# Tele-AI/MMPL

Hardware: AMD Instinct MI355X
Metric: video_latent_frames_per_sec (higher is better)
Workload: dtype bf16

## Files before the change

### include/mmpl_hip.h

```cpp
#ifndef MMPL_HIP_H
#define MMPL_HIP_H
#include <stddef.h>
#include <stdint.h>
#ifdef __cplusplus
extern "C" {
#endif

typedef void* mmpl_stream_t;

typedef struct MmplDitConfig {
  int dim, ffn_dim, num_heads, num_layers;
  int text_dim, freq_dim, in_dim, out_dim, text_len;
  float eps;
  int lat_h, lat_w;
  int max_frames;
} MmplDitConfig;

typedef struct MmplDit MmplDit;

int mmpl_dit_num_weights(const MmplDitConfig* cfg);
const char* mmpl_dit_weight_name(int slot_in_layer_or_global, int per_layer);

int mmpl_dit_create(const MmplDitConfig* cfg, MmplDit** out);
void mmpl_dit_destroy(MmplDit* h);
int mmpl_dit_bind_weights(MmplDit* h, const void* const* dev_ptrs, int n);

size_t mmpl_dit_workspace_bytes(const MmplDit* h, int n_frames);
size_t mmpl_dit_context_workspace_bytes(const MmplDit* h);

int mmpl_dit_precompute_context(MmplDit* h, const void* context, void* cross_k, void* cross_v, void* workspace,
                                size_t workspace_bytes, int* distinct_rows, mmpl_stream_t stream);

int mmpl_dit_set_image_kv(MmplDit* h, const void* img_k, const void* img_v, int n_img_tokens);

int mmpl_dit_set_attn_stats(MmplDit* h, void* stats_dev);

int mmpl_dit_forward(MmplDit* h, const void* x_in, const float* t_dev, int n_frames, const int* frame_ids,
                     const int* write_slots, const int* visible_slots, int n_visible, void* k_cache, void* v_cache,
                     int n_slots, const void* cross_k, const void* cross_v, int cross_rows, void* share_out, const void* share_in,
                     void* attn_history, void* out, void* workspace, size_t workspace_bytes, mmpl_stream_t stream);
size_t mmpl_dit_attn_history_bytes(const MmplDit* h, int n_frames);
int mmpl_dit_share_check_failures(MmplDit* h, long long* count, mmpl_stream_t stream);

int mmpl_attn_fwd(const void* q, int ldq, void* o, int ldo, const void* const* k_pages, const void* const* v_pages,
                  int ldk, int ldv, int n_pages, int page_rows, int Lq, int num_heads, float softmax_scale,
                  mmpl_stream_t stream);
size_t mmpl_attn_workspace_bytes(void);
int mmpl_attn_fwd_ws(const void* q, int ldq, void* o, int ldo, const void* const* k_pages, const void* const* v_pages,
                     int ldk, int ldv, int n_pages, int page_rows, int Lq, int num_heads, float softmax_scale,
                     void* workspace, size_t workspace_bytes, mmpl_stream_t stream);

int mmpl_attn_fwd_variant(const void* q, int ldq, void* o, int ldo, const void* const* k_pages, const void* const* v_pages,
                          int ldk, int ldv, int n_pages, int page_rows, int Lq, int num_heads, float softmax_scale,
                          void* workspace, size_t workspace_bytes, int variant, int cross, mmpl_stream_t stream);

size_t mmpl_attn_history_bytes(int Lq, int num_heads);
int mmpl_attn_fwd_history(const void* q, int ldq, void* o, int ldo, const void* const* k_pages, const void* const* v_pages,
                          int ldk, int ldv, int n_pages, int page_rows, int Lq, int num_heads, float softmax_scale,
                          void* workspace, size_t workspace_bytes, void* history, void* stats_dev, mmpl_stream_t stream);

int mmpl_gemm(const void* A, int lda, const void* W, int ldw, const void* bias, void* C, int ldc, int M, int N, int K,
              int epi, const void* res, int ldres, const void* gate, int gate_frame_stride, int rows_per_frame,
              mmpl_stream_t stream);
int mmpl_gemm_tickets(const void* A, int lda, const void* W, int ldw, const void* bias, void* C, int ldc, int M, int N, int K,
                      int epi, const void* res, int ldres, const void* gate, int gate_frame_stride, int rows_per_frame,
                      void* tile_counter, mmpl_stream_t stream);
size_t mmpl_gemm_scratch_bytes(void);
int mmpl_device_xcd_round_robin(void);
int mmpl_probe_mfma_tflops(int shape, double seconds, double* tflops);
int mmpl_gemm_scratch(const void* A, int lda, const void* W, int ldw, const void* bias, void* C, int ldc, int M, int N, int K,
                      int epi, const void* res, int ldres, const void* gate, int gate_frame_stride, int rows_per_frame,
                      void* scratch, size_t scratch_bytes, mmpl_stream_t stream);

int mmpl_layernorm(const void* x, int ldx, void* y, int ldy, int rows, int d, float eps, const void* scale,
                   const void* shift, int mod_frame_stride, int rows_per_frame, const void* w, const void* b,
                   mmpl_stream_t stream);

int mmpl_qknorm_rope(MmplDit* h, void* q, int ldq, const void* k, int ldk, const void* v, int ldv, const void* wq,
                     const void* wk, int n_frames, const int* frame_ids, void* const* k_dst, void* const* v_dst,
                     mmpl_stream_t stream);

typedef struct MmplUniPCStep {
  float guidance, sigma_cur;
  int use_corrector, corr_order;
  float c_c1, c_c2, c_c3, c_inv_rk, c_rho0, c_rho_last;
  int pred_order;
  float p_c1, p_c2, p_c3, p_inv_rk;
} MmplUniPCStep;
int mmpl_cfg_unipc_step(const void* flow_cond, const void* flow_uncond, void* x, void* m0, void* m1, void* last_sample,
                        size_t n, const MmplUniPCStep* s, mmpl_stream_t stream);
int mmpl_cfg_unipc_step_table(const void* flow_cond, const void* flow_uncond, void* x, void* m0, void* m1, void* last_sample,
                              size_t n, const MmplUniPCStep* table_dev, int* step_dev, float* timestep_dev,
                              const float* timestep_table_dev, int n_timestep, int n_steps, mmpl_stream_t stream);

int mmpl_fewstep_update(const void* flow, void* x, const void* noise, void* x0_out, size_t n, double sigma_t, float sigma_next,
                        mmpl_stream_t stream);

typedef struct MmplVae MmplVae;
int mmpl_vae_num_weights(void);
const char* mmpl_vae_weight_name(int i);
int mmpl_vae_create(int lat_h, int lat_w, MmplVae** out);
void mmpl_vae_destroy(MmplVae* v);
int mmpl_vae_bind_weights(MmplVae* v, const void* const* dev_ptrs, int n);
size_t mmpl_vae_workspace_bytes(MmplVae* v, int mode);
int mmpl_vae_decode(MmplVae* v, const void* z, int n_frames, const float* mean, const float* inv_std, void* out, void* workspace,
                    size_t workspace_bytes, mmpl_stream_t stream);
int mmpl_vae_encode(MmplVae* v, const void* px, int n_px_frames, const float* mean, const float* inv_std, void* out, void* workspace,
                    size_t workspace_bytes, mmpl_stream_t stream);

typedef struct MmplVaeStream MmplVaeStream;
int mmpl_vae_stream_create(MmplVae* v, MmplVaeStream** out);
void mmpl_vae_stream_destroy(MmplVaeStream* s);
int mmpl_vae_stream_reset(MmplVaeStream* s);
int mmpl_vae_stream_decode(MmplVaeStream* s, const void* z, int n_frames, const float* mean, const float* inv_std, void* out,
                           int out_format, int* n_px_frames_out, void* workspace, size_t workspace_bytes, mmpl_stream_t stream);

typedef struct MmplTaehv MmplTaehv;
int mmpl_taehv_num_weights(void);
const char* mmpl_taehv_weight_name(int i);
int mmpl_taehv_create(int lat_h, int lat_w, MmplTaehv** out);
void mmpl_taehv_destroy(MmplTaehv* v);
int mmpl_taehv_bind_weights(MmplTaehv* v, const void* const* dev_ptrs, int n);
size_t mmpl_taehv_workspace_bytes(MmplTaehv* v);
int mmpl_taehv_reset(MmplTaehv* v);
int mmpl_taehv_decode(MmplTaehv* v, const void* z, int n_frames, void* out, int out_format, int* n_px_frames_out, void* workspace,
                      size_t workspace_bytes, mmpl_stream_t stream);

typedef struct MmplT5Config {
  int vocab, dim, dim_attn, dim_ffn, num_heads, num_layers, num_buckets, text_len;
  float eps;
} MmplT5Config;
typedef struct MmplT5 MmplT5;
int mmpl_t5_num_weights(const MmplT5Config* cfg);
int mmpl_t5_create(const MmplT5Config* cfg, MmplT5** out);
void mmpl_t5_destroy(MmplT5* h);
int mmpl_t5_bind_weights(MmplT5* h, const void* const* dev_ptrs, int n);
size_t mmpl_t5_workspace_bytes(const MmplT5* h);
int mmpl_t5_encode(MmplT5* h, const int* ids, const int* mask, const int* bucket, void* out, void* workspace,
                   size_t workspace_bytes, mmpl_stream_t stream);

size_t mmpl_i2v_img_proj_workspace_bytes(int n_tok, int clip_dim, int dim);
int mmpl_i2v_img_proj(const void* clip_fea, int n_tok, int clip_dim, int dim, const void* const* w, void* out, void* workspace,
                      size_t workspace_bytes, mmpl_stream_t stream);
int mmpl_i2v_img_kv(const void* ctx_img, int n_tok, int dim, const void* wk, const void* bk, const void* wv, const void* bv,
                    const void* norm_k_img_w, float eps, void* k_out, void* v_out, mmpl_stream_t stream);
size_t mmpl_i2v_cross_attn_workspace_bytes(int Lq, int dim);
int mmpl_i2v_cross_attn(const void* x, int Lq, int dim, const void* wq, const void* bq, const void* norm_q_w, float eps,
                        const void* k_txt, const void* v_txt, int n_txt, const void* k_img, const void* v_img, int n_img,
                        const void* wo, const void* bo, void* out, void* workspace, size_t workspace_bytes, mmpl_stream_t stream);

size_t mmpl_clip_visual_workspace_bytes(int n_tok, int dim, int mlp_dim, int heads);
int mmpl_clip_visual(const void* patches, int n_patch, int pk, int dim, int mlp_dim, int heads, int head_dim, int n_blocks,
                     const void* const* gw, const void* const* lw, float eps, void* out, void* workspace, size_t workspace_bytes,
                     mmpl_stream_t stream);

int mmpl_profile_enable(int on);
int mmpl_profile_read(int n_kinds, double* ms, double* flops, long long* launches);

const char* mmpl_last_error(void);
const char* mmpl_version(void);

#ifdef __cplusplus
}
#endif
#endif
```

### mmpl_amd/_lib.py

```python
from __future__ import annotations

import ctypes as C
import os

_HERE = os.path.dirname(os.path.abspath(__file__))
LIB_PATH = os.path.join(_HERE, "lib", "libmmpl_hip.so")

SYMBOLS = [
    "mmpl_dit_num_weights", "mmpl_dit_weight_name", "mmpl_dit_create", "mmpl_dit_destroy", "mmpl_dit_bind_weights",
    "mmpl_dit_workspace_bytes", "mmpl_dit_context_workspace_bytes", "mmpl_dit_precompute_context", "mmpl_dit_forward", "mmpl_dit_attn_history_bytes", "mmpl_dit_share_check_failures", "mmpl_dit_set_attn_stats", "mmpl_dit_set_image_kv", "mmpl_clip_visual", "mmpl_clip_visual_workspace_bytes",
    "mmpl_attn_fwd", "mmpl_attn_fwd_ws", "mmpl_attn_fwd_variant", "mmpl_attn_fwd_history", "mmpl_attn_history_bytes", "mmpl_attn_workspace_bytes", "mmpl_gemm", "mmpl_gemm_tickets", "mmpl_gemm_scratch", "mmpl_gemm_scratch_bytes", "mmpl_device_xcd_round_robin", "mmpl_probe_mfma_tflops", "mmpl_layernorm", "mmpl_qknorm_rope", "mmpl_cfg_unipc_step", "mmpl_cfg_unipc_step_table", "mmpl_fewstep_update",
    "mmpl_vae_num_weights", "mmpl_vae_weight_name", "mmpl_vae_create", "mmpl_vae_destroy", "mmpl_vae_bind_weights",
    "mmpl_vae_workspace_bytes", "mmpl_vae_decode", "mmpl_vae_encode",
    "mmpl_vae_stream_create", "mmpl_vae_stream_destroy", "mmpl_vae_stream_reset", "mmpl_vae_stream_decode",
    "mmpl_taehv_num_weights", "mmpl_taehv_weight_name", "mmpl_taehv_create", "mmpl_taehv_destroy", "mmpl_taehv_bind_weights",
    "mmpl_taehv_workspace_bytes", "mmpl_taehv_reset", "mmpl_taehv_decode",
    "mmpl_t5_num_weights", "mmpl_t5_create", "mmpl_t5_destroy", "mmpl_t5_bind_weights", "mmpl_t5_workspace_bytes", "mmpl_t5_encode",
    "mmpl_i2v_img_proj_workspace_bytes", "mmpl_i2v_img_proj", "mmpl_i2v_img_kv", "mmpl_i2v_cross_attn_workspace_bytes", "mmpl_i2v_cross_attn",
    "mmpl_profile_enable", "mmpl_profile_read", "mmpl_last_error", "mmpl_version",
]


class MmplDitConfig(C.Structure):
    _fields_ = [(n, C.c_int) for n in ("dim", "ffn_dim", "num_heads", "num_layers", "text_dim", "freq_dim", "in_dim",
                                       "out_dim", "text_len")] + [("eps", C.c_float)] + \
               [(n, C.c_int) for n in ("lat_h", "lat_w", "max_frames")]


class MmplT5Config(C.Structure):
    _fields_ = [(n, C.c_int) for n in ("vocab", "dim", "dim_attn", "dim_ffn", "num_heads", "num_layers", "num_buckets", "text_len")] + \
               [("eps", C.c_float)]


class MmplUniPCStep(C.Structure):
    _fields_ = [("guidance", C.c_float), ("sigma_cur", C.c_float), ("use_corrector", C.c_int), ("corr_order", C.c_int),
                ("c_c1", C.c_float), ("c_c2", C.c_float), ("c_c3", C.c_float), ("c_inv_rk", C.c_float),
                ("c_rho0", C.c_float), ("c_rho_last", C.c_float), ("pred_order", C.c_int), ("p_c1", C.c_float),
                ("p_c2", C.c_float), ("p_c3", C.c_float), ("p_inv_rk", C.c_float)]


_lib = None


def load() -> C.CDLL:
    global _lib
    if _lib is not None:
        return _lib
    if not os.path.exists(LIB_PATH):
        raise RuntimeError(
            f"{LIB_PATH} not found: the MI355X HIP extension is not built. Run `python -m mmpl_amd.build` "
            "(or __graft_entry__.build()). mmpl_amd has no CPU/PyTorch fallback by design.")
    import torch
    lib = C.CDLL(LIB_PATH)
    vp, ci, cf, sz = C.c_void_p, C.c_int, C.c_float, C.c_size_t
    lib.mmpl_last_error.restype = C.c_char_p
    lib.mmpl_version.restype = C.c_char_p
    lib.mmpl_dit_num_weights.argtypes = [C.POINTER(MmplDitConfig)]
    lib.mmpl_dit_weight_name.argtypes = [ci, ci]
    lib.mmpl_dit_weight_name.restype = C.c_char_p
    lib.mmpl_dit_create.argtypes = [C.POINTER(MmplDitConfig), C.POINTER(vp)]
    lib.mmpl_dit_destroy.argtypes = [vp]
    lib.mmpl_dit_destroy.restype = None
    lib.mmpl_dit_bind_weights.argtypes = [vp, C.POINTER(vp), ci]
    lib.mmpl_dit_workspace_bytes.argtypes = [vp, ci]
    lib.mmpl_dit_workspace_bytes.restype = sz
    lib.mmpl_dit_context_workspace_bytes.argtypes = [vp]
    lib.mmpl_dit_context_workspace_bytes.restype = sz
    lib.mmpl_dit_precompute_context.argtypes = [vp, vp, vp, vp, vp, sz, C.POINTER(ci), vp]
    lib.mmpl_dit_forward.argtypes = [vp, vp, vp, ci, C.POINTER(ci), C.POINTER(ci), C.POINTER(ci), ci, vp, vp, ci, vp, vp,
                                     ci, vp, vp, vp, vp, vp, sz, vp]
    lib.mmpl_dit_attn_history_bytes.argtypes = [vp, ci]
    lib.mmpl_dit_attn_history_bytes.restype = sz
    lib.mmpl_dit_share_check_failures.argtypes = [vp, C.POINTER(C.c_longlong), vp]
    lib.mmpl_attn_history_bytes.argtypes = [ci, ci]
    lib.mmpl_attn_history_bytes.restype = sz
    lib.mmpl_attn_fwd_history.argtypes = [vp, ci, vp, ci, C.POINTER(vp), C.POINTER(vp), ci, ci, ci, ci, ci, ci, cf, vp, sz, vp, vp, vp]
    lib.mmpl_attn_fwd.argtypes = [vp, ci, vp, ci, C.POINTER(vp), C.POINTER(vp), ci, ci, ci, ci, ci, ci, cf, vp]
    lib.mmpl_attn_fwd_ws.argtypes = [vp, ci, vp, ci, C.POINTER(vp), C.POINTER(vp), ci, ci, ci, ci, ci, ci, cf, vp, sz, vp]
    lib.mmpl_attn_fwd_variant.argtypes = [vp, ci, vp, ci, C.POINTER(vp), C.POINTER(vp), ci, ci, ci, ci, ci, ci, cf, vp, sz, ci, ci, vp]
    lib.mmpl_cfg_unipc_step_table.argtypes = [vp, vp, vp, vp, vp, vp, sz, vp, vp, vp, vp, ci, ci, vp]
    lib.mmpl_attn_workspace_bytes.argtypes = []
    lib.mmpl_attn_workspace_bytes.restype = sz
    lib.mmpl_gemm.argtypes = [vp, ci, vp, ci, vp, vp, ci, ci, ci, ci, ci, vp, ci, vp, ci, ci, vp]
    lib.mmpl_gemm_tickets.argtypes = [vp, ci, vp, ci, vp, vp, ci, ci, ci, ci, ci, vp, ci, vp, ci, ci, vp, vp]
    lib.mmpl_gemm_scratch.argtypes = [vp, ci, vp, ci, vp, vp, ci, ci, ci, ci, ci, vp, ci, vp, ci, ci, vp, sz, vp]
    lib.mmpl_gemm_scratch_bytes.argtypes = []
    lib.mmpl_device_xcd_round_robin.argtypes = []
    lib.mmpl_probe_mfma_tflops.argtypes = [ci, C.c_double, C.POINTER(C.c_double)]
    lib.mmpl_gemm_scratch_bytes.restype = sz
    lib.mmpl_layernorm.argtypes = [vp, ci, vp, ci, ci, ci, cf, vp, vp, ci, ci, vp, vp, vp]
    lib.mmpl_qknorm_rope.argtypes = [vp, vp, ci, vp, ci, vp, ci, vp, vp, ci, C.POINTER(ci), C.POINTER(vp), C.POINTER(vp), vp]
    lib.mmpl_cfg_unipc_step.argtypes = [vp, vp, vp, vp, vp, vp, sz, C.POINTER(MmplUniPCStep), vp]
    lib.mmpl_fewstep_update.argtypes = [vp, vp, vp, vp, sz, C.c_double, cf, vp]
    lib.mmpl_profile_enable.argtypes = [ci]
    lib.mmpl_profile_read.argtypes = [ci, C.POINTER(C.c_double), C.POINTER(C.c_double), C.POINTER(C.c_longlong)]
    lib.mmpl_t5_num_weights.argtypes = [C.POINTER(MmplT5Config)]
    lib.mmpl_t5_create.argtypes = [C.POINTER(MmplT5Config), C.POINTER(vp)]
    lib.mmpl_t5_destroy.argtypes = [vp]
    lib.mmpl_t5_destroy.restype = None
    lib.mmpl_t5_bind_weights.argtypes = [vp, C.POINTER(vp), ci]
    lib.mmpl_t5_workspace_bytes.argtypes = [vp]
    lib.mmpl_t5_workspace_bytes.restype = sz
    lib.mmpl_t5_encode.argtypes = [vp, vp, vp, vp, vp, vp, sz, vp]
    cf = C.c_float
    lib.mmpl_i2v_img_proj_workspace_bytes.argtypes = [ci, ci, ci]
    lib.mmpl_i2v_img_proj_workspace_bytes.restype = sz
    lib.mmpl_dit_set_image_kv.argtypes = [vp, vp, vp, ci]
    lib.mmpl_dit_set_attn_stats.argtypes = [vp, vp]
    lib.mmpl_clip_visual_workspace_bytes.argtypes = [ci, ci, ci, ci]
    lib.mmpl_clip_visual_workspace_bytes.restype = sz
    lib.mmpl_clip_visual.argtypes = [vp, ci, ci, ci, ci, ci, ci, ci, C.POINTER(vp), C.POINTER(vp), cf, vp, vp, sz, vp]
    lib.mmpl_i2v_img_proj.argtypes = [vp, ci, ci, ci, C.POINTER(vp), vp, vp, sz, vp]
    lib.mmpl_i2v_img_kv.argtypes = [vp, ci, ci, vp, vp, vp, vp, vp, cf, vp, vp, vp]
    lib.mmpl_i2v_cross_attn_workspace_bytes.argtypes = [ci, ci]
    lib.mmpl_i2v_cross_attn_workspace_bytes.restype = sz
    lib.mmpl_i2v_cross_attn.argtypes = [vp, ci, ci, vp, vp, vp, cf, vp, vp, ci, vp, vp, ci, vp, vp, vp, vp, sz, vp]
    if hasattr(lib, "mmpl_vae_create"):
        _bind_vae(lib)
    _lib = lib
    return lib


def _bind_vae(lib):
    vp, ci, sz = C.c_void_p, C.c_int, C.c_size_t
    fp = C.POINTER(C.c_float)
    lib.mmpl_vae_weight_name.argtypes = [ci]
    lib.mmpl_vae_weight_name.restype = C.c_char_p
    lib.mmpl_vae_create.argtypes = [ci, ci, C.POINTER(vp)]
    lib.mmpl_vae_destroy.argtypes = [vp]
    lib.mmpl_vae_destroy.restype = None
    lib.mmpl_vae_bind_weights.argtypes = [vp, C.POINTER(vp), ci]
    lib.mmpl_vae_workspace_bytes.argtypes = [vp, ci]
    lib.mmpl_vae_workspace_bytes.restype = sz
    lib.mmpl_vae_decode.argtypes = [vp, vp, ci, fp, fp, vp, vp, sz, vp]
    lib.mmpl_vae_encode.argtypes = [vp, vp, ci, fp, fp, vp, vp, sz, vp]
    lib.mmpl_vae_stream_create.argtypes = [vp, C.POINTER(vp)]
    lib.mmpl_vae_stream_destroy.argtypes = [vp]
    lib.mmpl_vae_stream_destroy.restype = None
    lib.mmpl_vae_stream_reset.argtypes = [vp]
    lib.mmpl_vae_stream_decode.argtypes = [vp, vp, ci, fp, fp, vp, ci, C.POINTER(ci), vp, sz, vp]
    lib.mmpl_taehv_weight_name.argtypes = [ci]
    lib.mmpl_taehv_weight_name.restype = C.c_char_p
    lib.mmpl_taehv_create.argtypes = [ci, ci, C.POINTER(vp)]
    lib.mmpl_taehv_destroy.argtypes = [vp]
    lib.mmpl_taehv_destroy.restype = None
    lib.mmpl_taehv_bind_weights.argtypes = [vp, C.POINTER(vp), ci]
    lib.mmpl_taehv_workspace_bytes.argtypes = [vp]
    lib.mmpl_taehv_workspace_bytes.restype = sz
    lib.mmpl_taehv_reset.argtypes = [vp]
    lib.mmpl_taehv_decode.argtypes = [vp, vp, ci, vp, ci, C.POINTER(ci), vp, sz, vp]


def check(rc: int, what: str = "") -> None:
    if rc != 0:
        raise RuntimeError(f"libmmpl_hip {what}: {load().mmpl_last_error().decode()}")


def ptr(t) -> C.c_void_p:
    return C.c_void_p(0 if t is None else t.data_ptr())


def stream_ptr() -> C.c_void_p:
    import torch
    return C.c_void_p(torch.cuda.current_stream().cuda_stream)
```

### mmpl_amd/csrc/api.hip

```cpp
#include <math.h>
#include <stdio.h>
#include <stdlib.h>
#include <string.h>

#include <string>
#include <utility>
#include <vector>

#include "../../include/mmpl_hip.h"
#include "kernels.h"
#include "mmpl_config.h"

static thread_local std::string g_err;
static int fail(const char* where, const char* what) {
  g_err = std::string(where) + ": " + what;
  return 1;
}
int mmpl_set_error(const char* where, const char* what) { return fail(where, what); }
#define HIP_TRY(expr, where)                                     \
  do {                                                           \
    hipError_t e__ = (expr);                                     \
    if (e__ != hipSuccess) return fail(where, hipGetErrorString(e__)); \
  } while (0)

// ... 125 lines not shown
  for (int pos = 0; pos < 1024; ++pos) {
    int p = 0;
    for (int part = 0; part < 3; ++part)
      for (int j = 0; j < dims[part] / 2; ++j, ++p) {
        const double freq = 1.0 / pow(10000.0, (double)(2 * j) / (double)dims[part]);
        const double ang = (double)pos * freq;
        c[pos * 64 + p] = (float)cos(ang);
        s[pos * 64 + p] = (float)sin(ang);
      }
  }
  if (hipMalloc(&h->cos_tab, c.size() * 4) != hipSuccess || hipMalloc(&h->sin_tab, s.size() * 4) != hipSuccess) {
    delete h;
    return fail("mmpl_dit_create", "hipMalloc of RoPE tables failed (is a GPU present?)");
  }
  hipMemcpy(h->cos_tab, c.data(), c.size() * 4, hipMemcpyHostToDevice);
  hipMemcpy(h->sin_tab, s.data(), s.size() * 4, hipMemcpyHostToDevice);
  if (mmpl_config().check_share) {
    if (hipMalloc(&h->share_chk, 8 * sizeof(unsigned long long)) != hipSuccess || hipMemset(h->share_chk, 0, 8 * sizeof(unsigned long long)) != hipSuccess) {
      mmpl_dit_destroy(h);
      return fail("mmpl_dit_create", "hipMalloc of the share-check state failed");
    }
  }
  *out = h;
  return 0;
}

void mmpl_dit_destroy(MmplDit* h) {
  if (!h) return;
  if (h->cos_tab) hipFree(h->cos_tab);
  if (h->sin_tab) hipFree(h->sin_tab);
  if (h->share_chk) hipFree(h->share_chk);
  delete h;
}

int mmpl_dit_bind_weights(MmplDit* h, const void* const* ptrs, int n) {
  if (!h || !ptrs) return fail("mmpl_dit_bind_weights", "null argument");
  if (n != NG + h->cfg.num_layers * NL) return fail("mmpl_dit_bind_weights", "wrong pointer count");
  h->w.resize(n);
  for (int i = 0; i < n; ++i) {
    if (!ptrs[i]) return fail("mmpl_dit_bind_weights", "null weight pointer");
    h->w[i] = (const bf16_t*)ptrs[i];
  }
  return 0;
}

}

namespace {
struct Carver {
  char* base;
  size_t off = 0;
  explicit Carver(void* b) : base((char*)b) {}
  bf16_t* take(size_t elems) {
    bf16_t* p = (bf16_t*)(base + off);
    off += (elems * 2 + 255) & ~(size_t)255;
    return p;
  }
};
constexpr int kTicketInts = 64 + 256;
struct FwdWs {
  bf16_t *x, *xn, *big, *attn, *ksc, *vsc, *patch, *sinu, *t1, *e, *se, *e0, *emod, *emod_head, *yh;
  int* tile_counter;
  float* splitk;
  size_t bytes;
};
FwdWs carve_fwd(const MmplDit* h, int nF, void* base) {
  const MmplDitConfig& c = h->cfg;
  const size_t Lq = (size_t)nF * h->S, d = c.dim;
  const size_t bigw = (size_t)(3 * c.dim > c.ffn_dim ? 3 * c.dim : c.ffn_dim);
  Carver k(base);
  FwdWs w;
  static_assert(kTicketInts * sizeof(int) % sizeof(bf16_t) == 0, "ticket area");
  w.tile_counter = (int*)k.take(kTicketInts * sizeof(int) / sizeof(bf16_t));
  w.x = k.take(Lq * d);
  w.xn = k.take(Lq * d);
  w.big = k.take(Lq * bigw);
  w.attn = k.take(Lq * d);
  w.ksc = k.take(Lq * d);
  w.vsc = k.take(Lq * d);
  w.patch = k.take(Lq * (size_t)h->pe_k);
  w.sinu = k.take((size_t)nF * c.freq_dim);
  w.t1 = k.take((size_t)nF * d);
  w.e = k.take((size_t)nF * d);
  w.se = k.take((size_t)nF * d);
  w.e0 = k.take((size_t)nF * 6 * d);
  w.emod = k.take((size_t)c.num_layers * nF * 6 * d);
  w.emod_head = k.take((size_t)nF * 2 * d);
  w.yh = k.take(Lq * 64);
  w.splitk = (float*)k.take(mmpl_gemm_splitk_ws_bytes() / sizeof(bf16_t));
  w.bytes = k.off;
  return w;
}

int gemm(const bf16_t* A, int lda, const bf16_t* W, int ldw, const bf16_t* bias, bf16_t* C, int ldc, int M, int N, int K,
         int epi, const bf16_t* res, int ldres, const bf16_t* gate, int gfs, int rpf, hipStream_t s, int* tile_counter = nullptr,
         float* splitk_ws = nullptr) {
  GemmArgs g{A, lda, W, ldw, bias, C, ldc, M, N, K, epi, res, ldres, gate, gfs, rpf > 0 ? rpf : 1, 1.0f, 0, 0, 0, 0, 0};
  g.tile_counter = tile_counter;
  g.splitk_ws = splitk_ws;
  g.splitk_cnt = splitk_ws ? tile_counter + 64 : nullptr;
  ProfScope ps(K_GEMM, 2.0 * M * (double)N * K, s);
  hipError_t e = mmpl_launch_gemm(g, s);
  if (e != hipSuccess) return fail("gemm", hipGetErrorString(e));
  return 0;
}
#define TRY(x) do { if ((x) != 0) return 1; } while (0)
}

extern "C" {

size_t mmpl_dit_workspace_bytes(const MmplDit* h, int n_frames) { return carve_fwd(h, n_frames, nullptr).bytes; }
size_t mmpl_dit_context_workspace_bytes(const MmplDit* h) {
  return 2 * (((size_t)h->cfg.text_len * h->cfg.dim * 2 + 255) & ~(size_t)255) + (((size_t)h->cfg.text_len * sizeof(int) + 255) & ~(size_t)255);
}

int mmpl_dit_precompute_context(MmplDit* h, const void* context, void* cross_k, void* cross_v, void* workspace,
                                size_t workspace_bytes, int* distinct_rows, mmpl_stream_t stream) {
  if (!h || h->w.empty()) return fail("mmpl_dit_precompute_context", "weights not bound");
  if (workspace_bytes < mmpl_dit_context_workspace_bytes(h)) return fail("mmpl_dit_precompute_context", "workspace too small");
  const MmplDitConfig& c = h->cfg;
  hipStream_t s = (hipStream_t)stream;
  Carver k(workspace);
  bf16_t* t0 = k.take((size_t)c.text_len * c.dim);
  bf16_t* ctx = k.take((size_t)c.text_len * c.dim);
  const int T = c.text_len, d = c.dim;
  TRY(gemm((const bf16_t*)context, c.text_dim, h->G(G_TXT0_W), c.text_dim, h->G(G_TXT0_B), t0, d, T, d, c.text_dim,
           EPI_BIAS_GELU, nullptr, 0, nullptr, 0, 1, s));
  TRY(gemm(t0, d, h->G(G_TXT2_W), d, h->G(G_TXT2_B), ctx, d, T, d, d, EPI_BIAS, nullptr, 0, nullptr, 0, 1, s));
  if (distinct_rows) {
    *distinct_rows = T;
    hipStreamCaptureStatus cs = hipStreamCaptureStatusNone;
    (void)hipStreamIsCapturing(s, &cs);
    if (cs == hipStreamCaptureStatusNone && T >= 2) {
      int* flags = (int*)k.take(((size_t)T * sizeof(int) + 1) / sizeof(bf16_t));
      std::vector<int> hf(T);
      HIP_TRY(mmpl_launch_rows_equal_last(ctx, d, T, d, flags, s), "rows_equal_last");
      HIP_TRY(hipMemcpyAsync(hf.data(), flags, (size_t)T * sizeof(int), hipMemcpyDeviceToHost, s), "context flags");
      HIP_TRY(hipStreamSynchronize(s), "context flags");
      int n = T - 1;
      while (n > 0 && hf[n - 1]) --n;
      if (T - n >= 2) *distinct_rows = n;
    }
  }
  for (int l = 0; l < c.num_layers; ++l) {
    bf16_t* kl = (bf16_t*)cross_k + (size_t)l * T * d;
    bf16_t* vl = (bf16_t*)cross_v + (size_t)l * T * d;
    TRY(gemm(ctx, d, h->Lw(l, L_CK_W), d, h->Lw(l, L_CK_B), kl, d, T, d, d, EPI_BIAS, nullptr, 0, nullptr, 0, 1, s));
    HIP_TRY(mmpl_launch_rmsnorm(kl, d, h->Lw(l, L_CNK), T, d, c.eps, s), "rmsnorm(ctx k)");
    TRY(gemm(ctx, d, h->Lw(l, L_CV_W), d, h->Lw(l, L_CV_B), vl, d, T, d, d, EPI_BIAS, nullptr, 0, nullptr, 0, 1, s));
  }
  return 0;
}

int mmpl_dit_set_image_kv(MmplDit* h, const void* img_k, const void* img_v, int n_img_tokens) {
  if (!h) return fail("mmpl_dit_set_image_kv", "null handle");
  if ((img_k == nullptr) != (img_v == nullptr)) return fail("mmpl_dit_set_image_kv", "need both of img_k / img_v, or neither");
  if (img_k && (n_img_tokens < 1 || n_img_tokens > 4096)) return fail("mmpl_dit_set_image_kv", "n_img_tokens out of range");
  h->img_k = (const bf16_t*)img_k;
  h->img_v = (const bf16_t*)img_v;
  h->n_img = img_k ? n_img_tokens : 0;
  return 0;
}

int mmpl_dit_set_attn_stats(MmplDit* h, void* stats_dev) {
  if (!h) return fail("mmpl_dit_set_attn_stats", "null handle");
  if (reinterpret_cast<uintptr_t>(stats_dev) % 8) return fail("mmpl_dit_set_attn_stats", "stats must be 8-byte aligned");
  h->attn_stats = (unsigned long long*)stats_dev;
  return 0;
}

int mmpl_dit_forward(MmplDit* h, const void* x_in, const float* t_dev, int nF, const int* frame_ids,
                     const int* write_slots, const int* visible_slots, int n_visible, void* k_cache, void* v_cache,
                     int n_slots, const void* cross_k, const void* cross_v, int cross_rows, void* share_out, const void* share_in,
                     void* attn_history, void* out, void* workspace, size_t workspace_bytes, mmpl_stream_t stream) {
  if (!h || h->w.empty()) return fail("mmpl_dit_forward", "weights not bound");
  const MmplDitConfig& c = h->cfg;
  if (nF < 1 || nF > c.max_frames) return fail("mmpl_dit_forward", "n_frames out of range");
  int n_write = 0;
  for (int i = 0; i < nF; ++i) {
    if (write_slots[i] >= n_slots) return fail("mmpl_dit_forward", "write slot out of range");
    if (write_slots[i] >= 0) ++n_write;
  }
  if (n_write != 0 && n_write != nF) return fail("mmpl_dit_forward", "write_slots must be all >= 0 or all -1");
  if (share_out && share_in) return fail("mmpl_dit_forward", "share_out and share_in are exclusive (producer or consumer of block 0's self-attention)");
  const bool persist = n_write == nF;
  const int n_pages = n_visible + (persist ? 0 : nF);
  if (n_pages < 1 || n_pages > MMPL_MAX_PAGES) return fail("mmpl_dit_forward", "too many / no visible KV pages");
  for (int i = 0; i < n_visible; ++i)
    if (visible_slots[i] < 0 || visible_slots[i] >= n_slots) return fail("mmpl_dit_forward", "visible slot out of range");
  FwdWs w = carve_fwd(h, nF, workspace);
  if (workspace_bytes < w.bytes) return fail("mmpl_dit_forward", "workspace too small");
  hipStream_t s = (hipStream_t)stream;
  const int S = h->S, d = c.dim, f = c.ffn_dim, Lq = nF * S, H = c.num_heads, T = c.text_len;

  HIP_TRY(mmpl_launch_zero_ints(w.tile_counter, kTicketInts, s), "tile counter");
  int* const tc = w.tile_counter;
  HIP_TRY(mmpl_launch_patchify((const bf16_t*)x_in, w.patch, h->pe_k, nF, c.in_dim, c.lat_h, c.lat_w, s), "patchify");
  TRY(gemm(w.patch, h->pe_k, h->G(G_PE_W), h->pe_k, h->G(G_PE_B), w.x, d, Lq, d, h->pe_k, EPI_BIAS, nullptr, 0, nullptr, 0, 1, s));
  HIP_TRY(mmpl_launch_sinusoid(t_dev, w.sinu, nF, c.freq_dim, s), "sinusoid");
  TRY(gemm(w.sinu, c.freq_dim, h->G(G_TE0_W), c.freq_dim, h->G(G_TE0_B), w.t1, d, nF, d, c.freq_dim, EPI_BIAS_SILU, nullptr,
           0, nullptr, 0, 1, s));
  TRY(gemm(w.t1, d, h->G(G_TE2_W), d, h->G(G_TE2_B), w.e, d, nF, d, d, EPI_BIAS, nullptr, 0, nullptr, 0, 1, s));
  HIP_TRY(mmpl_launch_silu(w.e, w.se, (size_t)nF * d, s), "silu");
  TRY(gemm(w.se, d, h->G(G_TP_W), d, h->G(G_TP_B), w.e0, 6 * d, nF, 6 * d, d, EPI_BIAS, nullptr, 0, nullptr, 0, 1, s));
  HIP_TRY(mmpl_launch_modulation(h->G(G_BLOCK_MOD), (size_t)6 * d, w.e0, 6 * d, 0, w.emod, c.num_layers, nF, 6, d, s), "modulation");
  HIP_TRY(mmpl_launch_modulation(h->G(G_HEAD_MOD), 0, w.e, d, 1, w.emod_head, 1, nF, 2, d, s), "head modulation");

  const float scale = 1.0f / sqrtf(128.0f);
  const int self_variant = mmpl_attention_self_variant();
  const bool prescale_q = self_variant == ATTN_W64;
  const bool cross_w64_env = mmpl_config().cross_w64;
  const bool cross_w64 = cross_w64_env && prescale_q;
  const size_t layer_stride = (size_t)n_slots * S * d;
  const int ctx_n = (cross_rows >= 0 && cross_rows <= T - 2) ? cross_rows : -1;
  const size_t hist_layer = mmpl_attn_history_bytes(Lq, H);
  const bool check_share = h->share_chk != nullptr && (share_out || share_in);
  auto fingerprint_layer0 = [&](int which) -> int {
    PageList pk{}, pv{};
    for (int i = 0; i < n_visible; ++i) {
      pk.p[i] = (const bf16_t*)k_cache + (size_t)visible_slots[i] * S * d;
      pv.p[i] = (const bf16_t*)v_cache + (size_t)visible_slots[i] * S * d;
    }
    pk.n = pv.n = n_visible;
    if (n_visible < 1) return 0;
    HIP_TRY(mmpl_launch_share_check_zero(h->share_chk, which, s), "share check");
    HIP_TRY(mmpl_launch_pages_fingerprint(pk, (size_t)S * d * sizeof(bf16_t), h->share_chk, which, s), "share check (K)");
    HIP_TRY(mmpl_launch_pages_fingerprint(pv, (size_t)S * d * sizeof(bf16_t), h->share_chk, which, s), "share check (V)");
    if (which == 1) HIP_TRY(mmpl_launch_share_check_compare(h->share_chk, s), "share check (compare)");
    return 0;
  };
  for (int l = 0; l < c.num_layers; ++l) {
    const bf16_t* em = w.emod + (size_t)l * nF * 6 * d;
    bf16_t* kc = (bf16_t*)k_cache + (size_t)l * layer_stride;
    bf16_t* vc = (bf16_t*)v_cache + (size_t)l * layer_stride;
    const bool take_shared = l == 0 && share_in != nullptr;
    if (!take_shared || persist) {
      {
        LnArgs a{w.x, d, w.xn, d, Lq, d, c.eps, em + 1 * d, em + 0 * d, 6 * d, S, nullptr, nullptr};
        ProfScope ps(K_LAYERNORM, 0, s);
        HIP_TRY(mmpl_launch_layernorm(a, s), "norm1");
      }
      {
        GemmArgs g{w.xn, d, h->Lw(l, L_QKV_W), d, h->Lw(l, L_QKV_B), w.big, 3 * d, Lq, 3 * d, d, EPI_BIAS_VPAGES, nullptr, 0, nullptr, 0, S,
                   1.0f, 0, 0, 0, 0, 0};
        for (int i = 0; i < nF; ++i) g.v_dst[i] = persist ? vc + (size_t)write_slots[i] * S * d : w.vsc + (size_t)i * S * d;
        g.v_col0 = 2 * d;
        g.v_ld = d;
        g.tile_counter = tc;
        g.splitk_ws = w.splitk; g.splitk_cnt = tc + 64;
        ProfScope ps(K_GEMM, 2.0 * Lq * 3.0 * d * d, s);
        HIP_TRY(mmpl_launch_gemm(g, s), "qkv gemm");
      }
      {
        QkNormArgs a = {};
        a.q = w.big; a.ldq = 3 * d; a.k = w.big + d; a.ldk = 3 * d; a.v = nullptr; a.ldv = 3 * d;
        a.wq = h->Lw(l, L_NQ); a.wk = h->Lw(l, L_NK); a.rows = Lq; a.d = d; a.eps = c.eps; a.rope = 1;
        a.q_scale = prescale_q ? scale * 1.4426950408889634f : 0.f;
        a.cos_tab = h->cos_tab; a.sin_tab = h->sin_tab; a.rows_per_frame = S; a.grid_w = h->gw;
        for (int i = 0; i < nF; ++i) {
          a.frame_ids[i] = frame_ids[i];
          a.k_dst[i] = persist ? kc + (size_t)write_slots[i] * S * d : w.ksc + (size_t)i * S * d;
          a.v_dst[i] = persist ? vc + (size_t)write_slots[i] * S * d : w.vsc + (size_t)i * S * d;
        }
        ProfScope ps(K_QKNORM, 0, s);
        HIP_TRY(mmpl_launch_qknorm(a, s), "qk norm + rope + kv write");
      }
    }
    if (l == 0 && check_share) TRY(fingerprint_layer0(share_in ? 1 : 0));
    if (take_shared) {
      HIP_TRY(hipMemcpyAsync(w.x, share_in, (size_t)Lq * d * sizeof(bf16_t), hipMemcpyDeviceToDevice, s), "shared block-0 x");
    } else {
    {
        AttnArgs a = {};
        a.q = w.big; a.ldq = 3 * d; a.o = w.attn; a.ldo = d; a.ldk = d; a.ldv = d; a.page_rows = S; a.Lq = Lq; a.H = H; a.scale = scale;
        int np = 0;
        for (int i = 0; i < n_visible; ++i, ++np) {
          a.k_pages[np] = kc + (size_t)visible_slots[i] * S * d;
          a.v_pages[np] = vc + (size_t)visible_slots[i] * S * d;
        }
        if (!persist)
          for (int i = 0; i < nF; ++i, ++np) {
            a.k_pages[np] = w.ksc + (size_t)i * S * d;
            a.v_pages[np] = w.vsc + (size_t)i * S * d;
            a.page_group[np] = 1;
          }
        a.n_pages = np;
        a.variant = self_variant;
        a.q_prescaled = prescale_q;
        a.split_ws = (float*)w.xn;
        a.split_ws_bytes = (size_t)Lq * d * sizeof(bf16_t);
        a.redo_stats = h->attn_stats;
        a.history = attn_history ? (unsigned char*)attn_history + (size_t)l * hist_layer : nullptr;
        ProfScope ps(K_ATTN_SELF, 4.0 * Lq * (double)np * S * d, s);
        HIP_TRY(mmpl_launch_attention(a, s), "self attention");
      }
      TRY(gemm(w.attn, d, h->Lw(l, L_O_W), d, h->Lw(l, L_O_B), w.x, d, Lq, d, d, EPI_GATE_RES, w.x, d, em + 2 * d, 6 * d, S, s, tc, w.splitk));
      if (l == 0 && share_out) HIP_TRY(hipMemcpyAsync(share_out, w.x, (size_t)Lq * d * sizeof(bf16_t), hipMemcpyDeviceToDevice, s), "share block-0 x");
    }
    {
      LnArgs a{w.x, d, w.xn, d, Lq, d, c.eps, nullptr, nullptr, 0, S, h->Lw(l, L_N3_W), h->Lw(l, L_N3_B)};
      ProfScope ps(K_LAYERNORM, 0, s);
      HIP_TRY(mmpl_launch_layernorm(a, s), "norm3");
    }
    TRY(gemm(w.xn, d, h->Lw(l, L_CQ_W), d, h->Lw(l, L_CQ_B), w.big, d, Lq, d, d, EPI_BIAS, nullptr, 0, nullptr, 0, 1, s, tc, w.splitk));
    {
      ProfScope ps(K_QKNORM, 0, s);
      HIP_TRY(mmpl_launch_rmsnorm(w.big, d, h->Lw(l, L_CNQ), Lq, d, c.eps, s, cross_w64 ? scale * 1.4426950408889634f : 0.f), "cross q norm");
    }
    {
      AttnArgs a = {};
      a.q = w.big; a.ldq = d; a.o = w.attn; a.ldo = d; a.ldk = d; a.ldv = d; a.page_rows = T; a.Lq = Lq; a.H = H; a.scale = scale;
      a.n_pages = 1;
      a.cross = 1;
      if (cross_w64) { a.variant = ATTN_W64; a.q_prescaled = true; }
      else if (ctx_n >= 0) { a.page_rows = ctx_n + 1; a.last_row_copies = T - ctx_n; }
      a.k_pages[0] = (const bf16_t*)cross_k + (size_t)l * T * d;
      a.v_pages[0] = (const bf16_t*)cross_v + (size_t)l * T * d;
      ProfScope ps(K_ATTN_CROSS, 4.0 * Lq * (double)T * d, s);
      HIP_TRY(mmpl_launch_attention(a, s), "cross attention");
      if (h->img_k) {
        a.o = w.ksc;
        a.page_rows = h->n_img;
        a.last_row_copies = 0;
        a.k_pages[0] = h->img_k + (size_t)l * h->n_img * d;
        a.v_pages[0] = h->img_v + (size_t)l * h->n_img * d;
        ProfScope ps2(K_ATTN_CROSS, 4.0 * Lq * (double)h->n_img * d, s);
        HIP_TRY(mmpl_launch_attention(a, s), "image cross attention");
        HIP_TRY(mmpl_launch_add(w.attn, w.ksc, (size_t)Lq * d, s), "x + img_x");
      }
    }
    TRY(gemm(w.attn, d, h->Lw(l, L_CO_W), d, h->Lw(l, L_CO_B), w.x, d, Lq, d, d, EPI_RES, w.x, d, nullptr, 0, 1, s, tc, w.splitk));
    {
      LnArgs a{w.x, d, w.xn, d, Lq, d, c.eps, em + 4 * d, em + 3 * d, 6 * d, S, nullptr, nullptr};
      ProfScope ps(K_LAYERNORM, 0, s);
      HIP_TRY(mmpl_launch_layernorm(a, s), "norm2");
    }
    TRY(gemm(w.xn, d, h->Lw(l, L_F0_W), d, h->Lw(l, L_F0_B), w.big, f, Lq, f, d, EPI_BIAS_GELU, nullptr, 0, nullptr, 0, 1, s, tc, w.splitk));
    TRY(gemm(w.big, f, h->Lw(l, L_F2_W), f, h->Lw(l, L_F2_B), w.x, d, Lq, d, f, EPI_GATE_RES, w.x, d, em + 5 * d, 6 * d, S, s, tc, w.splitk));
  }
  {
    LnArgs a{w.x, d, w.xn, d, Lq, d, c.eps, w.emod_head + d, w.emod_head, 2 * d, S, nullptr, nullptr};
    HIP_TRY(mmpl_launch_layernorm(a, s), "head norm");
  }
  TRY(gemm(w.xn, d, h->G(G_HEAD_W), d, h->G(G_HEAD_B), w.yh, 64, Lq, 64, d, EPI_BIAS, nullptr, 0, nullptr, 0, 1, s));
  HIP_TRY(mmpl_launch_unpatchify(w.yh, 64, (bf16_t*)out, nF, c.out_dim, c.lat_h, c.lat_w, s), "unpatchify");
  if (check_share && share_in) {
    hipStreamCaptureStatus cs = hipStreamCaptureStatusNone;
    (void)hipStreamIsCapturing(s, &cs);
    if (cs == hipStreamCaptureStatusNone) {
      long long n = 0;
      TRY(mmpl_dit_share_check_failures(h, &n, stream));
      if (n) return fail("mmpl_dit_forward", "MMPL_CHECK_SHARE: share_in was given but the layer-0 K / V this forward attends to differ from "
                                             "the share_out forward's (the two CFG caches are out of step)");
    }
  }
  return 0;
}

int mmpl_dit_share_check_failures(MmplDit* h, long long* count, mmpl_stream_t stream) {
  if (!h || !count) return fail("mmpl_dit_share_check_failures", "null argument");
  *count = 0;
  if (!h->share_chk) return 0;
  unsigned long long n = 0;
  hipStream_t s = (hipStream_t)stream;
  HIP_TRY(hipMemcpyAsync(&n, h->share_chk + 4, sizeof(n), hipMemcpyDeviceToHost, s), "share check read");
  HIP_TRY(hipStreamSynchronize(s), "share check read");
  if (n) HIP_TRY(hipMemsetAsync(h->share_chk + 4, 0, sizeof(n), s), "share check reset");
  *count = (long long)n;
  return 0;
}

size_t mmpl_dit_attn_history_bytes(const MmplDit* h, int n_frames) {
  return h ? (size_t)h->cfg.num_layers * mmpl_attn_history_bytes(n_frames * h->S, h->cfg.num_heads) : 0;
}
size_t mmpl_attn_history_bytes(int Lq, int num_heads) { return mmpl_attention_history_bytes(Lq, num_heads); }

int mmpl_attn_fwd_history(const void* q, int ldq, void* o, int ldo, const void* const* k_pages, const void* const* v_pages,
                          int ldk, int ldv, int n_pages, int page_rows, int Lq, int num_heads, float softmax_scale,
                          void* workspace, size_t workspace_bytes, void* history, void* stats_dev, mmpl_stream_t stream) {
  if (n_pages < 1 || n_pages > MMPL_MAX_PAGES) return fail("mmpl_attn_fwd_history", "n_pages out of range");
  if (reinterpret_cast<uintptr_t>(stats_dev) % 8) return fail("mmpl_attn_fwd_history", "stats must be 8-byte aligned");
  AttnArgs a = {};
  a.variant = ATTN_W64;
  a.q_prescaled = 1;
  a.q = (const bf16_t*)q; a.ldq = ldq; a.o = (bf16_t*)o; a.ldo = ldo; a.ldk = ldk; a.ldv = ldv; a.n_pages = n_pages;
  a.page_rows = page_rows; a.Lq = Lq; a.H = num_heads; a.scale = softmax_scale;
  a.split_ws = (float*)workspace; a.split_ws_bytes = workspace ? workspace_bytes : 0;
  a.history = (unsigned char*)history;
  a.redo_stats = (unsigned long long*)stats_dev;
  for (int i = 0; i < n_pages; ++i) { a.k_pages[i] = (const bf16_t*)k_pages[i]; a.v_pages[i] = (const bf16_t*)v_pages[i]; }
  HIP_TRY(mmpl_launch_attention(a, (hipStream_t)stream), "mmpl_attn_fwd_history");
  return 0;
}

size_t mmpl_attn_workspace_bytes(void) { return mmpl_attention_split_ws_bytes(); }

int mmpl_attn_fwd_variant(const void* q, int ldq, void* o, int ldo, const void* const* k_pages, const void* const* v_pages,
                          int ldk, int ldv, int n_pages, int page_rows, int Lq, int num_heads, float softmax_scale,
                          void* workspace, size_t workspace_bytes, int variant, int cross, mmpl_stream_t stream) {
  if (n_pages < 1 || n_pages > MMPL_MAX_PAGES) return fail("mmpl_attn_fwd", "n_pages out of range");
  if (variant != ATTN_AUTO && variant != ATTN_LOCKSTEP && variant != ATTN_W64 && variant != ATTN_W64 + 1)
    return fail("mmpl_attn_fwd", "unknown kernel variant");
  AttnArgs a = {};
  a.variant = variant > ATTN_W64 ? ATTN_W64 : variant;
  a.q_prescaled = variant == ATTN_W64 + 1;
  a.cross = cross != 0;
  a.q = (const bf16_t*)q; a.ldq = ldq; a.o = (bf16_t*)o; a.ldo = ldo; a.ldk = ldk; a.ldv = ldv; a.n_pages = n_pages;
  a.page_rows = page_rows; a.Lq = Lq; a.H = num_heads; a.scale = softmax_scale;
  a.split_ws = (float*)workspace; a.split_ws_bytes = workspace ? workspace_bytes : 0;
  for (int i = 0; i < n_pages; ++i) { a.k_pages[i] = (const bf16_t*)k_pages[i]; a.v_pages[i] = (const bf16_t*)v_pages[i]; }
  HIP_TRY(mmpl_launch_attention(a, (hipStream_t)stream), "mmpl_attn_fwd");
  return 0;
}

int mmpl_attn_fwd_ws(const void* q, int ldq, void* o, int ldo, const void* const* k_pages, const void* const* v_pages,
                     int ldk, int ldv, int n_pages, int page_rows, int Lq, int num_heads, float softmax_scale,
                     void* workspace, size_t workspace_bytes, mmpl_stream_t stream) {
  return mmpl_attn_fwd_variant(q, ldq, o, ldo, k_pages, v_pages, ldk, ldv, n_pages, page_rows, Lq, num_heads, softmax_scale, workspace,
                               workspace_bytes, ATTN_AUTO, 0, stream);
}

int mmpl_attn_fwd(const void* q, int ldq, void* o, int ldo, const void* const* k_pages, const void* const* v_pages,
                  int ldk, int ldv, int n_pages, int page_rows, int Lq, int num_heads, float softmax_scale,
                  mmpl_stream_t stream) {
  return mmpl_attn_fwd_ws(q, ldq, o, ldo, k_pages, v_pages, ldk, ldv, n_pages, page_rows, Lq, num_heads, softmax_scale, nullptr, 0,
                          stream);
}

int mmpl_gemm(const void* A, int lda, const void* W, int ldw, const void* bias, void* C, int ldc, int M, int N, int K,
              int epi, const void* res, int ldres, const void* gate, int gate_frame_stride, int rows_per_frame,
              mmpl_stream_t stream) {
  if (epi < EPI_BIAS || epi > EPI_F32_SCALE) return fail("mmpl_gemm", "unknown epilogue");
  if ((epi == EPI_GATE_RES && (!res || !gate)) || (epi == EPI_RES && !res)) return fail("mmpl_gemm", "missing epilogue operand");
  return gemm((const bf16_t*)A, lda, (const bf16_t*)W, ldw, (const bf16_t*)bias, (bf16_t*)C, ldc, M, N, K, epi,
              (const bf16_t*)res, ldres, (const bf16_t*)gate, gate_frame_stride, rows_per_frame, (hipStream_t)stream);
}

int mmpl_gemm_tickets(const void* A, int lda, const void* W, int ldw, const void* bias, void* C, int ldc, int M, int N, int K,
                      int epi, const void* res, int ldres, const void* gate, int gate_frame_stride, int rows_per_frame,
                      void* tile_counter, mmpl_stream_t stream) {
  if (epi < EPI_BIAS || epi > EPI_F32_SCALE) return fail("mmpl_gemm", "unknown epilogue");
  if ((epi == EPI_GATE_RES && (!res || !gate)) || (epi == EPI_RES && !res)) return fail("mmpl_gemm", "missing epilogue operand");
  return gemm((const bf16_t*)A, lda, (const bf16_t*)W, ldw, (const bf16_t*)bias, (bf16_t*)C, ldc, M, N, K, epi,
              (const bf16_t*)res, ldres, (const bf16_t*)gate, gate_frame_stride, rows_per_frame, (hipStream_t)stream, (int*)tile_counter);
}

size_t mmpl_gemm_scratch_bytes(void) { return 2048 + mmpl_gemm_splitk_ws_bytes(); }
int mmpl_device_xcd_round_robin(void) { return mmpl_xcd_dispatch_ok(true) ? 1 : 0; }

int mmpl_gemm_scratch(const void* A, int lda, const void* W, int ldw, const void* bias, void* C, int ldc, int M, int N, int K,
                      int epi, const void* res, int ldres, const void* gate, int gate_frame_stride, int rows_per_frame,
                      void* scratch, size_t scratch_bytes, mmpl_stream_t stream) {
  if (epi < EPI_BIAS || epi > EPI_F32_SCALE) return fail("mmpl_gemm", "unknown epilogue");
  if ((epi == EPI_GATE_RES && (!res || !gate)) || (epi == EPI_RES && !res)) return fail("mmpl_gemm", "missing epilogue operand");
  if (!scratch || scratch_bytes < mmpl_gemm_scratch_bytes()) return fail("mmpl_gemm_scratch", "scratch missing or smaller than mmpl_gemm_scratch_bytes()");
  if (reinterpret_cast<uintptr_t>(scratch) % 256) return fail("mmpl_gemm_scratch", "scratch must be 256-byte aligned");
  return gemm((const bf16_t*)A, lda, (const bf16_t*)W, ldw, (const bf16_t*)bias, (bf16_t*)C, ldc, M, N, K, epi,
              (const bf16_t*)res, ldres, (const bf16_t*)gate, gate_frame_stride, rows_per_frame, (hipStream_t)stream, (int*)scratch,
              (float*)((char*)scratch + 2048));
}

int mmpl_layernorm(const void* x, int ldx, void* y, int ldy, int rows, int d, float eps, const void* scale,
                   const void* shift, int mod_frame_stride, int rows_per_frame, const void* w, const void* b,
                   mmpl_stream_t stream) {
  if (!w && (!scale || !shift)) return fail("mmpl_layernorm", "need (scale, shift) or (w, b)");
  LnArgs a{(const bf16_t*)x, ldx, (bf16_t*)y, ldy, rows, d, eps, (const bf16_t*)scale, (const bf16_t*)shift, mod_frame_stride,
           rows_per_frame > 0 ? rows_per_frame : 1, (const bf16_t*)w, (const bf16_t*)b};
  HIP_TRY(mmpl_launch_layernorm(a, (hipStream_t)stream), "mmpl_layernorm");
  return 0;
}

int mmpl_qknorm_rope(MmplDit* h, void* q, int ldq, const void* k, int ldk, const void* v, int ldv, const void* wq,
                     const void* wk, int n_frames, const int* frame_ids, void* const* k_dst, void* const* v_dst,
                     mmpl_stream_t stream) {
  if (!h) return fail("mmpl_qknorm_rope", "null handle");
  if (n_frames < 1 || n_frames > 8) return fail("mmpl_qknorm_rope", "n_frames out of range");
  QkNormArgs a = {};
  a.q = (bf16_t*)q; a.ldq = ldq; a.k = (const bf16_t*)k; a.ldk = ldk; a.v = (const bf16_t*)v; a.ldv = ldv;
  a.wq = (const bf16_t*)wq; a.wk = (const bf16_t*)wk; a.rows = n_frames * h->S; a.d = h->cfg.dim; a.eps = h->cfg.eps; a.rope = 1;
  a.cos_tab = h->cos_tab; a.sin_tab = h->sin_tab; a.rows_per_frame = h->S; a.grid_w = h->gw;
  for (int i = 0; i < n_frames; ++i) { a.frame_ids[i] = frame_ids[i]; a.k_dst[i] = (bf16_t*)k_dst[i]; a.v_dst[i] = (bf16_t*)v_dst[i]; }
  HIP_TRY(mmpl_launch_qknorm(a, (hipStream_t)stream), "mmpl_qknorm_rope");
  return 0;
}

int mmpl_cfg_unipc_step(const void* flow_cond, const void* flow_uncond, void* x, void* m0, void* m1, void* last_sample,
                        size_t n, const MmplUniPCStep* st, mmpl_stream_t stream) {
  if (!st) return fail("mmpl_cfg_unipc_step", "null step");
  UniPCArgs a = {};
  a.flow_c = (const bf16_t*)flow_cond; a.flow_u = (const bf16_t*)flow_uncond; a.guidance = st->guidance; a.x = (bf16_t*)x;
  a.m0 = (bf16_t*)m0; a.m1 = (bf16_t*)m1; a.last_sample = (bf16_t*)last_sample; a.n = n; a.sigma_cur = st->sigma_cur;
  a.use_corrector = st->use_corrector; a.corr_order = st->corr_order; a.c_c1 = st->c_c1; a.c_c2 = st->c_c2; a.c_c3 = st->c_c3;
  a.c_inv_rk = st->c_inv_rk; a.c_rho0 = st->c_rho0; a.c_rho_last = st->c_rho_last; a.pred_order = st->pred_order;
  a.p_c1 = st->p_c1; a.p_c2 = st->p_c2; a.p_c3 = st->p_c3; a.p_inv_rk = st->p_inv_rk;
  ProfScope ps(K_UNIPC, 0, (hipStream_t)stream);
  HIP_TRY(mmpl_launch_unipc(a, (hipStream_t)stream), "mmpl_cfg_unipc_step");
  return 0;
}

int mmpl_cfg_unipc_step_table(const void* flow_cond, const void* flow_uncond, void* x, void* m0, void* m1, void* last_sample,
                              size_t n, const MmplUniPCStep* table_dev, int* step_dev, float* timestep_dev,
                              const float* timestep_table_dev, int n_timestep, int n_steps, mmpl_stream_t stream) {
  if (!table_dev || !step_dev || !timestep_dev || !timestep_table_dev || n_steps < 1 || n_timestep < 1)
    return fail("mmpl_cfg_unipc_step_table", "bad arguments");
  static_assert(sizeof(MmplUniPCStep) == sizeof(UniPCStepDev), "table layout");
  UniPCArgs a = {};
  a.flow_c = (const bf16_t*)flow_cond; a.flow_u = (const bf16_t*)flow_uncond; a.x = (bf16_t*)x;
  a.m0 = (bf16_t*)m0; a.m1 = (bf16_t*)m1; a.last_sample = (bf16_t*)last_sample; a.n = n;
  HIP_TRY(mmpl_launch_unipc_table(a, (const UniPCStepDev*)table_dev, step_dev, timestep_dev, timestep_table_dev, n_timestep, n_steps,
                                  (hipStream_t)stream), "mmpl_cfg_unipc_step_table");
  return 0;
}

}
```

### mmpl_amd/csrc/attention.hip

```cpp
#include <stdlib.h>

#include <type_traits>

#include "common.h"
#include "kernels.h"
#include "mmpl_config.h"

namespace {

constexpr int NW = 8, QW = 32, QB = NW * QW, KVB = 64;
constexpr int K_STRIDE = 272;
constexpr int V_STRIDE = 320;
constexpr int K_TILE = KVB * K_STRIDE;
constexpr int V_TILE = KVB * V_STRIDE;
constexpr int BUF = K_TILE + V_TILE;
constexpr int SMEM = 2 * BUF;

typedef __attribute__((ext_vector_type(4))) short s16x4;

MMPL_DEV bf16x8 tr_pair(const char* p0, const char* p1) {
  s16x4 a = __builtin_amdgcn_ds_read_tr16_b64_v4i16((__attribute__((address_space(3))) s16x4*)(p0));
  s16x4 b = __builtin_amdgcn_ds_read_tr16_b64_v4i16((__attribute__((address_space(3))) s16x4*)(p1));
  return bf16x8{a[0], a[1], a[2], a[3], b[0], b[1], b[2], b[3]};
}

struct AttnState { f32x16 o[4]; float m_run, l_run; };
MMPL_DEV void attn_tile(const char* kb, const char* vb, const bf16x8 (&qf)[8], int valid, float last_bias, float c, int k_off, int v_off,
                        int hi, AttnState& st) {
#pragma clang fp contract(off)
  f32x16 (&o)[4] = st.o;
  float& m_run = st.m_run;
  float& l_run = st.l_run;
  f32x16 s0, s1;
#pragma unroll
  for (int r = 0; r < 16; ++r) { s0[r] = 0.f; s1[r] = 0.f; }
  {
    auto kfrag = [&](int i) {
      return *reinterpret_cast<const bf16x8*>(kb + k_off + (i >> 3) * (32 * K_STRIDE) + 32 * (i & 7));
    };
    bf16x8 w0 = kfrag(0), w1 = kfrag(1), w2 = kfrag(2), w3 = kfrag(3);
    __builtin_amdgcn_sched_barrier(0);
    __builtin_amdgcn_s_setprio(1);
#pragma unroll
    for (int i = 0; i < 16; i += 4) {
      if (i < 8) s0 = __builtin_amdgcn_mfma_f32_32x32x16_bf16(w0, qf[i & 7], s0, 0, 0, 0);
      else s1 = __builtin_amdgcn_mfma_f32_32x32x16_bf16(w0, qf[i & 7], s1, 0, 0, 0);
      if (i + 4 < 16) w0 = kfrag(i + 4);
      __builtin_amdgcn_sched_barrier(0);
      if (i < 8) s0 = __builtin_amdgcn_mfma_f32_32x32x16_bf16(w1, qf[(i + 1) & 7], s0, 0, 0, 0);
      else s1 = __builtin_amdgcn_mfma_f32_32x32x16_bf16(w1, qf[(i + 1) & 7], s1, 0, 0, 0);
      if (i + 5 < 16) w1 = kfrag(i + 5);
      __builtin_amdgcn_sched_barrier(0);
      if (i < 8) s0 = __builtin_amdgcn_mfma_f32_32x32x16_bf16(w2, qf[(i + 2) & 7], s0, 0, 0, 0);
      else s1 = __builtin_amdgcn_mfma_f32_32x32x16_bf16(w2, qf[(i + 2) & 7], s1, 0, 0, 0);
      if (i + 6 < 16) w2 = kfrag(i + 6);
      __builtin_amdgcn_sched_barrier(0);
      if (i < 8) s0 = __builtin_amdgcn_mfma_f32_32x32x16_bf16(w3, qf[(i + 3) & 7], s0, 0, 0, 0);
      else s1 = __builtin_amdgcn_mfma_f32_32x32x16_bf16(w3, qf[(i + 3) & 7], s1, 0, 0, 0);
      if (i + 7 < 16) w3 = kfrag(i + 7);
      __builtin_amdgcn_sched_barrier(0);
    }
    __builtin_amdgcn_s_setprio(0);
  }
  if (valid < KVB) {
#pragma unroll
    for (int r = 0; r < 16; ++r) {
      const int kv = 8 * (r >> 2) + 4 * hi + (r & 3);
      if (kv >= valid) s0[r] = -INFINITY;
      if (kv + 32 >= valid) s1[r] = -INFINITY;
    }
  }
  if (last_bias != 0.f && valid <= KVB) {
#pragma unroll
    for (int r = 0; r < 16; ++r) {
      const int kv = 8 * (r >> 2) + 4 * hi + (r & 3);
      if (kv == valid - 1) s0[r] += last_bias;
      if (kv + 32 == valid - 1) s1[r] += last_bias;
    }
  }
  float mx = s0[0];
#pragma unroll
  for (int r = 1; r < 16; ++r) mx = fmaxf(mx, s0[r]);
#pragma unroll
  for (int r = 0; r < 16; ++r) mx = fmaxf(mx, s1[r]);
  mx = fmaxf(mx, __shfl_xor(mx, 32, 64));
  const float m_new = fmaxf(m_run, mx);
  if (__any(m_new > m_run)) {
    const float alpha = __builtin_amdgcn_exp2f((m_run - m_new) * c);
    l_run *= alpha;
#pragma unroll
    for (int nb = 0; nb < 4; ++nb)
#pragma unroll
      for (int r = 0; r < 16; ++r) o[nb][r] *= alpha;
    m_run = m_new;
  }
  const float mc = m_run * c;
  float ls0 = 0.f, ls1 = 0.f;
  bf16x8 pb[2][2];
#pragma unroll
  for (int r = 0; r < 16; ++r) { s0[r] = __builtin_amdgcn_exp2f(__builtin_fmaf(s0[r], c, -mc)); ls0 += s0[r]; }
#pragma unroll
  for (int cc = 0; cc < 2; ++cc) {
    union { uint32_t u[4]; bf16x8 v; } x0;
#pragma unroll
    for (int j = 0; j < 4; ++j) x0.u[j] = pack2bf(s0[8 * cc + 2 * j], s0[8 * cc + 2 * j + 1]);
    pb[0][cc] = x0.v;
  }
#pragma unroll
  for (int cc = 0; cc < 2; ++cc)
#pragma unroll
    for (int nb = 0; nb < 4; ++nb) {
      const char* vp = vb + v_off + (16 * cc) * V_STRIDE + 64 * nb;
      const bf16x8 vf = tr_pair(vp, vp + 8 * V_STRIDE);
      o[nb] = __builtin_amdgcn_mfma_f32_32x32x16_bf16(vf, pb[0][cc], o[nb], 0, 0, 0);
    }
#pragma unroll
  for (int r = 0; r < 16; ++r) { s1[r] = __builtin_amdgcn_exp2f(__builtin_fmaf(s1[r], c, -mc)); ls1 += s1[r]; }
  l_run += ls0 + ls1;
#pragma unroll
  for (int cc = 0; cc < 2; ++cc) {
    union { uint32_t u[4]; bf16x8 v; } x1;
#pragma unroll
    for (int j = 0; j < 4; ++j) x1.u[j] = pack2bf(s1[8 * cc + 2 * j], s1[8 * cc + 2 * j + 1]);
    pb[1][cc] = x1.v;
  }
  __builtin_amdgcn_s_setprio(1);
#pragma unroll
  for (int cc = 0; cc < 2; ++cc)
#pragma unroll
    for (int nb = 0; nb < 4; ++nb) {
      const char* vp = vb + v_off + (32 + 16 * cc) * V_STRIDE + 64 * nb;
      const bf16x8 vf = tr_pair(vp, vp + 8 * V_STRIDE);
      o[nb] = __builtin_amdgcn_mfma_f32_32x32x16_bf16(vf, pb[1][cc], o[nb], 0, 0, 0);
    }
  __builtin_amdgcn_s_setprio(0);

}

template <int CROSS>
__global__ __launch_bounds__(512, 2) void attn_fwd_kernel(AttnArgs a) {
  extern __shared__ __attribute__((aligned(16))) char smem[];
  const int tid = threadIdx.x, lane = tid & 63, wave = tid >> 6;
  const int hi = lane >> 5, l31 = lane & 31;

  const int n_qb = (a.Lq + QB - 1) / QB;
  int head, qb;
  if ((a.H & 7) == 0) {
    const int xcd = blockIdx.x & 7, local = blockIdx.x >> 3;
    head = xcd + 8 * (local / n_qb);
    qb = local % n_qb;
  } else {
    head = blockIdx.x / n_qb;
    qb = blockIdx.x % n_qb;
  }

  const int qrow = min(qb * QB + wave * QW + l31, a.Lq - 1);
  bf16x8 qf[8];
  {
    const bf16_t* qp = a.q + (size_t)qrow * a.ldq + head * 128 + 8 * hi;
#pragma unroll
    for (int c = 0; c < 8; ++c) qf[c] = *reinterpret_cast<const bf16x8*>(qp + 16 * c);
  }

  const int tiles_pp = (a.page_rows + KVB - 1) / KVB;
  const int total = a.n_pages * tiles_pp;

  const int srow = tid >> 4, schunk = tid & 15;
  u32x4 rk[2], rv[2];
  auto stage_load = [&](int t) {
    const int p = t / tiles_pp, row0 = (t - p * tiles_pp) * KVB;
    const bf16_t* kp = a.k_pages[p] + head * 128 + schunk * 8;
    const bf16_t* vp = a.v_pages[p] + head * 128 + schunk * 8;
#pragma unroll
    for (int j = 0; j < 2; ++j) {
      const int r = min(row0 + srow + 32 * j, a.page_rows - 1);
      rk[j] = *reinterpret_cast<const u32x4*>(kp + (size_t)r * a.ldk);
      rv[j] = *reinterpret_cast<const u32x4*>(vp + (size_t)r * a.ldv);
    }
  };
  auto stage_write = [&](int buf) {
    char* kb = smem + buf * BUF;
    char* vb = kb + K_TILE;
#pragma unroll
    for (int j = 0; j < 2; ++j) {
      *reinterpret_cast<u32x4*>(kb + (srow + 32 * j) * K_STRIDE + schunk * 16) = rk[j];
      *reinterpret_cast<u32x4*>(vb + (srow + 32 * j) * V_STRIDE + schunk * 16) = rv[j];
    }
  };

  AttnState st;
#pragma unroll
  for (int nb = 0; nb < 4; ++nb)
#pragma unroll
    for (int r = 0; r < 16; ++r) st.o[nb][r] = 0.f;
  st.m_run = -INFINITY;
  st.l_run = 0.f;
  const float c = a.scale * 1.4426950408889634f;
  const float last_bias = a.last_row_copies > 1 ? __logf((float)a.last_row_copies) / a.scale : 0.f;

  const int k_off = l31 * K_STRIDE + 16 * hi;
  const int i16 = lane & 15, g16 = (lane >> 4) & 1;
  const int v_off = (4 * hi + (i16 >> 2)) * V_STRIDE + (16 * g16 + 4 * (i16 & 3)) * 2;

  stage_load(0);
  stage_write(0);
  __syncthreads();

  for (int t = 0; t < total; ++t) {
    const int cur = t & 1;
    if (t + 1 < total) stage_load(t + 1);
    const char* kb = smem + cur * BUF;
    const char* vb = kb + K_TILE;

    const int pg = t / tiles_pp, row0 = (t - pg * tiles_pp) * KVB;
    attn_tile(kb, vb, qf, a.page_rows - row0, last_bias, c, k_off, v_off, hi, st);

    if (t + 1 < total) stage_write(cur ^ 1);
    __syncthreads();
  }

  const float l_tot = st.l_run + __shfl_xor(st.l_run, 32, 64);
  const float inv = 1.0f / l_tot;
  constexpr int O_PITCH = 264;
  static_assert(NW * QW * O_PITCH <= SMEM, "output staging fits the K/V buffers");
  char* ob = smem + wave * (QW * O_PITCH);
#pragma unroll
  for (int nb = 0; nb < 4; ++nb)
#pragma unroll
    for (int g = 0; g < 4; ++g) {
      uint2 w;
      w.x = pack2bf(st.o[nb][4 * g] * inv, st.o[nb][4 * g + 1] * inv);
      w.y = pack2bf(st.o[nb][4 * g + 2] * inv, st.o[nb][4 * g + 3] * inv);
      *reinterpret_cast<uint2*>(ob + l31 * O_PITCH + (32 * nb + 8 * g + 4 * hi) * 2) = w;
    }
  const int orow = lane >> 4, ochunk = lane & 15;
#pragma unroll
  for (int k = 0; k < 8; ++k) {
    const int r = orow + 4 * k, q_out = qb * QB + wave * QW + r;
    const uint2 lo = *reinterpret_cast<const uint2*>(ob + r * O_PITCH + ochunk * 16);
    const uint2 hi2 = *reinterpret_cast<const uint2*>(ob + r * O_PITCH + ochunk * 16 + 8);
    if (q_out < a.Lq) *reinterpret_cast<uint4*>(a.o + (size_t)q_out * a.ldo + head * 128 + ochunk * 8) = uint4{lo.x, lo.y, hi2.x, hi2.y};
  }
}


constexpr int O_PITCH_X = 264;
constexpr int SMEM_X = 2 * BUF + NW * QW * O_PITCH_X;

template <int NT>
__global__ __launch_bounds__(512, 2) void attn_cross_kernel(AttnArgs a, int qb_per_block, int blocks_per_head) {
  extern __shared__ __attribute__((aligned(16))) char smem[];
  const int tid = threadIdx.x, lane = tid & 63, wave = __builtin_amdgcn_readfirstlane(tid >> 6);
  const int hi = lane >> 5, l31 = lane & 31;
  const int n_qb = (a.Lq + QB - 1) / QB;
  int head, part;
  if ((a.H & 7) == 0) {
    const int xcd = blockIdx.x & 7, local = blockIdx.x >> 3;
    head = xcd + 8 * (local / blocks_per_head);
    part = local % blocks_per_head;
  } else {
    head = blockIdx.x / blocks_per_head;
    part = blockIdx.x % blocks_per_head;
  }
  int qb = part * qb_per_block;
  const int qb_end = min(qb + qb_per_block, n_qb);
  if (qb >= qb_end) return;

  auto load_q = [&](bf16x8 (&f)[8], int qblock) {
    const int qrow = min(qblock * QB + wave * QW + l31, a.Lq - 1);
    const bf16_t* qp = a.q + (size_t)qrow * a.ldq + head * 128 + 8 * hi;
#pragma unroll
    for (int c = 0; c < 8; ++c) f[c] = *reinterpret_cast<const bf16x8*>(qp + 16 * c);
  };
  bf16x8 qf[8], qn[8];
  load_q(qf, qb);
  {
    const int srow = tid >> 4, schunk = tid & 15;
    const bf16_t* kp = a.k_pages[0] + head * 128 + schunk * 8;
    const bf16_t* vp = a.v_pages[0] + head * 128 + schunk * 8;
#pragma unroll
    for (int t = 0; t < NT; ++t)
#pragma unroll
      for (int j = 0; j < 2; ++j) {
        const int r = min(t * KVB + srow + 32 * j, a.page_rows - 1);
        const u32x4 rk = *reinterpret_cast<const u32x4*>(kp + (size_t)r * a.ldk);
        const u32x4 rv = *reinterpret_cast<const u32x4*>(vp + (size_t)r * a.ldv);
        *reinterpret_cast<u32x4*>(smem + t * BUF + (srow + 32 * j) * K_STRIDE + schunk * 16) = rk;
        *reinterpret_cast<u32x4*>(smem + t * BUF + K_TILE + (srow + 32 * j) * V_STRIDE + schunk * 16) = rv;
      }
  }
  __syncthreads();
  const float c = a.scale * 1.4426950408889634f;
  const float last_bias = a.last_row_copies > 1 ? __logf((float)a.last_row_copies) / a.scale : 0.f;
  const int k_off = l31 * K_STRIDE + 16 * hi;
  const int i16 = lane & 15, g16 = (lane >> 4) & 1;
  const int v_off = (4 * hi + (i16 >> 2)) * V_STRIDE + (16 * g16 + 4 * (i16 & 3)) * 2;
  char* ob = smem + 2 * BUF + wave * (QW * O_PITCH_X);
  const int orow = lane >> 4, ochunk = lane & 15;

  for (;; ++qb) {
    const bool more = qb + 1 < qb_end;
    if (more) load_q(qn, qb + 1);
    asm volatile("" ::: "memory");
    AttnState st;
#pragma unroll
    for (int nb = 0; nb < 4; ++nb)
#pragma unroll
      for (int r = 0; r < 16; ++r) st.o[nb][r] = 0.f;
    st.m_run = -INFINITY;
    st.l_run = 0.f;
#pragma unroll
    for (int t = 0; t < NT; ++t)
      attn_tile(smem + t * BUF, smem + t * BUF + K_TILE, qf, a.page_rows - t * KVB, last_bias, c, k_off, v_off, hi, st);
    const float l_tot = st.l_run + __shfl_xor(st.l_run, 32, 64);
    const float inv = 1.0f / l_tot;
#pragma unroll
    for (int nb = 0; nb < 4; ++nb)
#pragma unroll
      for (int g = 0; g < 4; ++g) {
        uint2 w;
        w.x = pack2bf(st.o[nb][4 * g] * inv, st.o[nb][4 * g + 1] * inv);
        w.y = pack2bf(st.o[nb][4 * g + 2] * inv, st.o[nb][4 * g + 3] * inv);
        *reinterpret_cast<uint2*>(ob + l31 * O_PITCH_X + (32 * nb + 8 * g + 4 * hi) * 2) = w;
      }
#pragma unroll
    for (int k = 0; k < 8; ++k) {
      const int r = orow + 4 * k, q_out = qb * QB + wave * QW + r;
      const uint2 lo = *reinterpret_cast<const uint2*>(ob + r * O_PITCH_X + ochunk * 16);
      const uint2 hi2 = *reinterpret_cast<const uint2*>(ob + r * O_PITCH_X + ochunk * 16 + 8);
      if (q_out < a.Lq) *reinterpret_cast<uint4*>(a.o + (size_t)q_out * a.ldo + head * 128 + ochunk * 8) = uint4{lo.x, lo.y, hi2.x, hi2.y};
    }
    if (!more) break;
#pragma unroll
    for (int i = 0; i < 8; ++i) {
      qf[i] = qn[i];
      asm volatile("" : "+v"(qf[i]));
    }
  }
}


__global__ __launch_bounds__(256) void attn_merge_kernel(AttnArgs a, int local_base, int sp, int tb) {
  __shared__ float wgt[QB][4];
  const int xcd = blockIdx.x & 7, k = blockIdx.x >> 3;
  const int n_qb = (a.Lq + QB - 1) / QB;
  int head, qb;
  if (!mmpl_attn_item(a.H, n_qb, xcd, local_base + k, head, qb)) return;
  const float* base = a.split_ws + (size_t)(xcd * tb + k) * sp * (QB * 130);
  const float c = a.scale * 1.4426950408889634f;
  {
    const int r = threadIdx.x;
    float m = -INFINITY;
    for (int p = 0; p < sp; ++p) m = fmaxf(m, base[(size_t)p * (QB * 130) + QB * 128 + r]);
    float l = 0.f, w[4] = {0.f, 0.f, 0.f, 0.f};
    for (int p = 0; p < sp; ++p) {
      w[p] = __builtin_amdgcn_exp2f((base[(size_t)p * (QB * 130) + QB * 128 + r] - m) * c);
      l += w[p] * base[(size_t)p * (QB * 130) + QB * 129 + r];
    }
    const float inv = 1.0f / l;
    for (int p = 0; p < 4; ++p) wgt[r][p] = w[p] * inv;
  }
  __syncthreads();
  for (int i = threadIdx.x; i < QB * 32; i += 256) {
    const int r = i >> 5, ch = i & 31, q_out = qb * QB + r;
    f32x4 acc = {0.f, 0.f, 0.f, 0.f};
    for (int p = 0; p < sp; ++p) {
      const f32x4 v = *reinterpret_cast<const f32x4*>(base + (size_t)p * (QB * 130) + (size_t)r * 128 + ch * 4);
      const float w = wgt[r][p];
      acc[0] += w * v[0]; acc[1] += w * v[1]; acc[2] += w * v[2]; acc[3] += w * v[3];
    }
    if (q_out < a.Lq) {
      uint2 o2;
      o2.x = pack2bf(acc[0], acc[1]);
      o2.y = pack2bf(acc[2], acc[3]);
      *reinterpret_cast<uint2*>(a.o + (size_t)q_out * a.ldo + head * 128 + ch * 4) = o2;
    }
  }
}

}

size_t mmpl_attention_split_ws_bytes() { return (size_t)256 * QB * 130 * sizeof(float); }

int mmpl_attention_self_variant() { return mmpl_config().attn_v1 ? ATTN_LOCKSTEP : ATTN_W64; }

namespace {
AttnArgs merge_contiguous_pages(const AttnArgs& a) {
  int order[MMPL_MAX_PAGES];
  for (int i = 0; i < a.n_pages; ++i) order[i] = i;
  auto before = [&a](int x, int y) {
    return a.page_group[x] != a.page_group[y] ? a.page_group[x] < a.page_group[y] : a.k_pages[x] < a.k_pages[y];
  };
  for (int i = 1; i < a.n_pages; ++i)
    for (int j = i; j > 0 && before(order[j], order[j - 1]); --j) { const int t = order[j]; order[j] = order[j - 1]; order[j - 1] = t; }
  const size_t kstride = (size_t)a.page_rows * a.ldk, vstride = (size_t)a.page_rows * a.ldv;
  const size_t per_page = 2 * (kstride > vstride ? kstride : vstride);
  const int max_run = per_page ? (int)(((1ull << 31) - 1) / per_page) : 1;
  AttnArgs m = a;
  m.n_pages = 0;
  for (int i = 0; i < a.n_pages;) {
    int r = 1;
    while (i + r < a.n_pages && r < max_run && a.page_group[order[i + r]] == a.page_group[order[i]] &&
           a.k_pages[order[i + r]] == a.k_pages[order[i + r - 1]] + kstride && a.v_pages[order[i + r]] == a.v_pages[order[i + r - 1]] + vstride)
      ++r;
    m.k_pages[m.n_pages] = a.k_pages[order[i]];
    m.v_pages[m.n_pages] = a.v_pages[order[i]];
    m.page_rows_each[m.n_pages++] = r * a.page_rows;
    i += r;
  }
  return m;
}
}

hipError_t mmpl_launch_attention(const AttnArgs& a_in, hipStream_t s) {
  if (a_in.Lq <= 0) return hipSuccess;
  if (a_in.n_pages <= 0 || a_in.n_pages > MMPL_MAX_PAGES) return hipErrorInvalidValue;
  const bool no_merge = mmpl_config().attn_no_merge;
  const bool w64_bound = a_in.variant == ATTN_W64 || (a_in.variant == ATTN_AUTO && !a_in.cross && a_in.q_prescaled && mmpl_attention_self_variant() == ATTN_W64);
  AttnArgs a = a_in;
  for (int p = 0; p < a.n_pages; ++p) a.page_rows_each[p] = a.page_rows;
  if (!no_merge && w64_bound && a.n_pages > 1) a = merge_contiguous_pages(a);
  if (a.n_pages <= 0 || a.n_pages > MMPL_MAX_PAGES || a.page_rows <= 0 || (a.ldq % 8) || (a.ldk % 8) || (a.ldv % 8) ||
      (a.ldo % 8) || ((uintptr_t)a.o & 15) || (a.variant != ATTN_AUTO && a.variant != ATTN_LOCKSTEP && a.variant != ATTN_W64))
    return hipErrorInvalidValue;
  const bool no_split = mmpl_config().attn_nosplit;
  int variant = a.variant;
  if (variant == ATTN_AUTO) {
    variant = a.cross ? ATTN_LOCKSTEP : mmpl_attention_self_variant();
    if (variant == ATTN_W64 && !a.q_prescaled) variant = ATTN_LOCKSTEP;
  }
  if (a.q_prescaled && variant != ATTN_W64) return hipErrorInvalidValue;
  if (a.last_row_copies > 1 && (variant != ATTN_LOCKSTEP || a.n_pages != 1)) return hipErrorInvalidValue;
  const int n_qb = (a.Lq + QB - 1) / QB;
  if (variant == ATTN_LOCKSTEP && a.cross && a.n_pages == 1 && a.page_rows <= 2 * KVB) {
    const int nt = (a.page_rows + KVB - 1) / KVB;
    const void* f = nt == 1 ? reinterpret_cast<const void*>(attn_cross_kernel<1>) : reinterpret_cast<const void*>(attn_cross_kernel<2>);
    if (hipError_t e = mmpl_dyn_smem_once(f, SMEM_X); e != hipSuccess) return e;
    const int cus = 8 * mmpl_cus_per_xcd();
    int bph = cus / a.H < 1 ? 1 : cus / a.H;
    if (bph > n_qb) bph = n_qb;
    const int qpb = (n_qb + bph - 1) / bph;
    bph = (n_qb + qpb - 1) / qpb;
    if (nt == 1) hipLaunchKernelGGL(attn_cross_kernel<1>, dim3(bph * a.H), dim3(512), SMEM_X, s, a, qpb, bph);
    else hipLaunchKernelGGL(attn_cross_kernel<2>, dim3(bph * a.H), dim3(512), SMEM_X, s, a, qpb, bph);
    return hipGetLastError();
  }
  if (variant == ATTN_LOCKSTEP) {
    const void* f = a.cross ? reinterpret_cast<const void*>(attn_fwd_kernel<1>) : reinterpret_cast<const void*>(attn_fwd_kernel<0>);
    if (hipError_t e = mmpl_dyn_smem_once(f, SMEM); e != hipSuccess) return e;
    if (a.cross) hipLaunchKernelGGL(attn_fwd_kernel<1>, dim3(n_qb * a.H), dim3(512), SMEM, s, a);
    else hipLaunchKernelGGL(attn_fwd_kernel<0>, dim3(n_qb * a.H), dim3(512), SMEM, s, a);
    return hipGetLastError();
  }
  if (a.history) a.history_mem = reinterpret_cast<short*>(a.history + mmpl_attention_history_state_bytes(a.Lq, a.H));
  if (hipError_t e = mmpl_dyn_smem_once(mmpl_attention_w64_symbol(0), mmpl_attention_w64_smem()); e != hipSuccess) return e;
  if (hipError_t e = mmpl_dyn_smem_once(mmpl_attention_w64_symbol(1), mmpl_attention_w64_smem()); e != hipSuccess) return e;
  auto run = [&](int blocks, int local_base, int sp, bool split) { mmpl_launch_attention_w64(a, blocks, local_base, sp, split, s); };
  const int per_xcd = mmpl_cus_per_xcd();
  int tiles = 0;
  for (int p = 0; p < a.n_pages; ++p) tiles += (a.page_rows_each[p] + KVB - 1) / KVB;
  const int total = n_qb * a.H;
  const int b = (a.H & 7) == 0 ? total / 8 : (total + 7) / 8, tb = b % per_xcd;
  int sp = 1;
  if (!no_split && a.split_ws && b > per_xcd && tb > 0 && per_xcd / tb >= 2) {
    sp = per_xcd / tb > 4 ? 4 : per_xcd / tb;
    if (tiles / sp < 8 || (size_t)8 * tb * sp * QB * 130 * sizeof(float) > a.split_ws_bytes) sp = 1;
  }
  if (sp == 1) {
    run(8 * b, 0, 1, false);
  } else {
    run(8 * (b - tb), 0, 1, false);
    run(8 * tb * sp, b - tb, sp, true);
    hipLaunchKernelGGL(attn_merge_kernel, dim3(8 * tb), dim3(256), 0, s, a, b - tb, sp, tb);
  }
  return hipGetLastError();
}
```

### mmpl_amd/csrc/device_state.hip

```cpp
#include <mutex>
#include <set>
#include <utility>

#include "kernels.h"

namespace {
std::mutex g_mu;
std::set<std::pair<int, const void*>> g_attr_done;
int g_per_xcd[64];
int g_xcd_dispatch[64];

__global__ void xcc_probe_kernel(int* out) {
  if (threadIdx.x == 0) {
    int x;
    asm volatile("s_getreg_b32 %0, hwreg(HW_REG_XCC_ID, 0, 4)" : "=s"(x));
    out[blockIdx.x] = x;
  }
}
}

bool mmpl_xcd_dispatch_ok(bool may_probe) {
  int dev = 0;
  if (hipGetDevice(&dev) != hipSuccess || dev < 0 || dev >= 64) return false;
  std::lock_guard<std::mutex> lk(g_mu);
  if (g_xcd_dispatch[dev] == 0 && may_probe) {
    constexpr int n = 2048;
    int* d = nullptr;
    int h[n];
    bool ok = hipMalloc(&d, n * sizeof(int)) == hipSuccess;
    if (ok) {
      ok = hipMemset(d, 0xff, n * sizeof(int)) == hipSuccess;
      hipLaunchKernelGGL(xcc_probe_kernel, dim3(n), dim3(64), 0, 0, d);
      ok = ok && hipGetLastError() == hipSuccess;
      ok = hipMemcpy(h, d, n * sizeof(int), hipMemcpyDeviceToHost) == hipSuccess && ok;
      (void)hipFree(d);
    }
    unsigned seen = 0;
    for (int x = 0; ok && x < 8; ++x) {
      ok = h[x] >= 0 && h[x] < 8 && !(seen & (1u << h[x]));
      if (ok) seen |= 1u << h[x];
    }
    for (int b = 8; ok && b < n; ++b) ok = h[b] == h[b & 7];
    g_xcd_dispatch[dev] = ok ? 1 : -1;
  }
  return g_xcd_dispatch[dev] == 1;
}

hipError_t mmpl_dyn_smem_once(const void* func, int bytes) {
  int dev = 0;
  hipError_t e = hipGetDevice(&dev);
  if (e != hipSuccess) return e;
  std::lock_guard<std::mutex> lk(g_mu);
  if (g_attr_done.count({dev, func})) return hipSuccess;
  e = hipFuncSetAttribute(func, hipFuncAttributeMaxDynamicSharedMemorySize, bytes);
  if (e == hipSuccess) g_attr_done.insert({dev, func});
  return e;
}

int mmpl_cus_per_xcd() {
  int dev = 0;
  if (hipGetDevice(&dev) != hipSuccess || dev < 0 || dev >= 64) return 32;
  std::lock_guard<std::mutex> lk(g_mu);
  if (!g_per_xcd[dev]) {
    hipDeviceProp_t prop;
    g_per_xcd[dev] = hipGetDeviceProperties(&prop, dev) == hipSuccess && prop.multiProcessorCount >= 8 ? prop.multiProcessorCount / 8 : 32;
  }
  return g_per_xcd[dev];
}


#include <stdlib.h>

#include "mmpl_config.h"
const MmplRuntimeConfig& mmpl_config() {
  static const MmplRuntimeConfig cfg = [] {
    auto flag = [](const char* n) { const char* v = getenv(n); return v != nullptr && atoi(v) != 0; };
    auto num = [](const char* n, int dflt) { const char* v = getenv(n); return v ? atoi(v) : dflt; };
    MmplRuntimeConfig c{};
    c.attn_v1 = flag("MMPL_ATTN_V1"); c.attn_nosplit = flag("MMPL_ATTN_NOSPLIT"); c.attn_no_merge = flag("MMPL_ATTN_NO_MERGE");
    c.cross_w64 = flag("MMPL_CROSS_W64");
    c.gemm_v1 = flag("MMPL_GEMM_V1"); c.gemm_v2 = flag("MMPL_GEMM_V2");
    c.gemm_no_splitk = flag("MMPL_GEMM_NO_SPLITK"); c.gemm_no_subtile = flag("MMPL_GEMM_NO_SUBTILE");
    c.gemm_group = num("MMPL_GEMM_GROUP", 0);
    c.gemm_pf = num("MMPL_GEMM_PF", 2);
    c.gemm_v8 = num("MMPL_GEMM_V8", -1);
    c.vae_no_fuse_norm = flag("MMPL_VAE_NO_FUSE_NORM");
    c.ln_pipeline_min_rows = num("MMPL_LN_PIPELINE_MIN_ROWS", 16384);
    c.check_share = flag("MMPL_CHECK_SHARE");
    return c;
  }();
  return cfg;
}
```

### mmpl_amd/csrc/elementwise.hip

```cpp
#include "common.h"
#include "kernels.h"
#include "mmpl_config.h"

namespace {

MMPL_DEV void unpack8(const uint4& u, float (&f)[8]) {
  f[0] = bf2f(u.x & 0xffff); f[1] = bf2f(u.x >> 16); f[2] = bf2f(u.y & 0xffff); f[3] = bf2f(u.y >> 16);
  f[4] = bf2f(u.z & 0xffff); f[5] = bf2f(u.z >> 16); f[6] = bf2f(u.w & 0xffff); f[7] = bf2f(u.w >> 16);
}
MMPL_DEV uint4 pack8(const float (&f)[8]) {
  uint4 u;
  u.x = pack2bf(f[0], f[1]); u.y = pack2bf(f[2], f[3]); u.z = pack2bf(f[4], f[5]); u.w = pack2bf(f[6], f[7]);
  return u;
}

template <int NIT>
__global__ __launch_bounds__(256) void layernorm_kernel(LnArgs a) {
#pragma clang fp contract(off)
  const int row = blockIdx.x * 4 + (threadIdx.x >> 6);
  if (row >= a.rows) return;
  const int lane = threadIdx.x & 63;
  const int nchunk = a.d >> 3;
  const bf16_t* xp = a.x + (size_t)row * a.ldx;
  float v[NIT][8];
// ... 138 lines not shown
      __syncthreads();
      const bf16_t* p0 = a.w ? a.w : a.scale + (size_t)gframe * a.mod_frame_stride;
      const bf16_t* p1 = a.w ? a.b : a.shift + (size_t)gframe * a.mod_frame_stride;
      for (int i = threadIdx.x; i < nchunk; i += 256) {
        sm[0][i] = *reinterpret_cast<const uint4*>(p0 + i * 8);
        sm[1][i] = *reinterpret_cast<const uint4*>(p1 + i * 8);
      }
      __syncthreads();
      staged = gframe;
    }
    if (more) load_row<NIT, FULL>(nxt, a.x + (size_t)(row + 4) * a.ldx, lane, nchunk, row + 4 < a.rows);
    asm volatile("" ::: "memory");
    if (FULL || row < a.rows) layernorm_row<NIT, FULL>(a, cur, sm, staged, row, lane, nchunk);
    if (!more) break;
#pragma unroll
    for (int it = 0; it < NIT; ++it) { cur[it] = nxt[it]; keep_packed(cur[it]); }
  }
}

struct RopeRow { float cs[4], sn[4]; int lf, tok; };
MMPL_DEV void rope_row(const QkNormArgs& a, int row, int lane, bool live, RopeRow& r) {
  r.lf = a.rope ? row / a.rows_per_frame : 0;
  r.tok = a.rope ? row - r.lf * a.rows_per_frame : row;
  if (a.rope && live) {
    const int gy = r.tok / a.grid_w, gx = r.tok - gy * a.grid_w, ft = a.frame_ids[r.lf];
#pragma unroll
    for (int j = 0; j < 4; ++j) {
      const int p = 4 * (lane & 15) + j;
      const int pos = p < 22 ? ft : (p < 43 ? gy : gx);
      r.cs[j] = a.cos_tab[pos * 64 + p];
      r.sn[j] = a.sin_tab[pos * 64 + p];
    }
  }
}

template <int NIT, bool FULL>
MMPL_DEV void qknorm_row(const QkNormArgs& a, uint4 (&cur)[NIT], const uint4* sg, const RopeRow& rc, bf16_t* dst, float qs, int lane, int nchunk) {
#pragma clang fp contract(off)
  float sq = 0.f;
#pragma unroll
  for (int it = 0; it < NIT; ++it) {
    float v[8];
    unpack8(cur[it], v);
#pragma unroll
    for (int j = 0; j < 8; ++j) sq += v[j] * v[j];
  }
  const float rr = rsqrtf(wave_sum(sq) / (float)a.d + a.eps);
#pragma unroll
  for (int it = 0; it < NIT; ++it) {
    const int ch = lane + 64 * it;
    if (!FULL && ch >= nchunk) continue;
    keep_packed(cur[it]);
    float v[8], w[8], o[8];
    unpack8(cur[it], v);
    unpack8(sg[ch], w);
#pragma unroll
    for (int j = 0; j < 8; ++j) o[j] = rbf(rbf(v[j] * rr) * w[j]);
    if (a.rope) {
#pragma unroll
      for (int j = 0; j < 4; ++j) {
        const float re = o[2 * j], im = o[2 * j + 1], cs = rc.cs[j], sn = rc.sn[j];
        o[2 * j] = j == 0 ? re * cs - im * sn : __builtin_fmaf(re, cs, -(im * sn));
        o[2 * j + 1] = j == 3 ? __builtin_fmaf(re, sn, im * cs) : __builtin_fmaf(im, cs, re * sn);
      }
    }
#pragma unroll
    for (int j = 0; j < 8; ++j) o[j] *= qs;
    *reinterpret_cast<uint4*>(dst + ch * 8) = pack8(o);
  }
}

template <int NIT, bool FULL>
__global__ __launch_bounds__(256) void qknorm_kernel(QkNormArgs a, int groups_per_block) {
  __shared__ uint4 sg[NIT * 64];
  const int wv = __builtin_amdgcn_readfirstlane(threadIdx.x >> 6), lane = threadIdx.x & 63;
  const int nchunk = a.d >> 3;
  const int which = blockIdx.y;
  const int ngroups = (a.rows + 3) >> 2;
  int g = blockIdx.x * groups_per_block;
  const int g_end = min(g + groups_per_block, ngroups);
  if (g >= g_end) return;
  if (which == 2) {
    for (; g < g_end; ++g) {
      const int row = 4 * g + wv;
      if (row >= a.rows) break;
      const int lf = a.rope ? row / a.rows_per_frame : 0, tok = a.rope ? row - lf * a.rows_per_frame : row;
      const bf16_t* src = a.v + (size_t)row * a.ldv;
      bf16_t* dst = a.v_dst[lf] + (size_t)tok * a.d;
      for (int ch = lane; ch < nchunk; ch += 64)
        *reinterpret_cast<uint4*>(dst + ch * 8) = *reinterpret_cast<const uint4*>(src + ch * 8);
    }
    return;
  }
  const bf16_t* gain = which == 0 ? a.wq : a.wk;
  for (int i = threadIdx.x; i < nchunk; i += 256) sg[i] = *reinterpret_cast<const uint4*>(gain + i * 8);
  const bf16_t* base = which == 0 ? a.q : a.k;
  const int ld = which == 0 ? a.ldq : a.ldk;
  const float qs = (which == 0 && a.q_scale != 0.f) ? a.q_scale : 1.0f;
  uint4 cur[NIT], nxt[NIT];
  RopeRow rc, rn;
  rope_row(a, 4 * g + wv, lane, FULL || 4 * g + wv < a.rows, rc);
  load_row<NIT, FULL>(cur, base + (size_t)(4 * g + wv) * ld, lane, nchunk, 4 * g + wv < a.rows);
  __syncthreads();
  for (;; ++g) {
    const int row = 4 * g + wv;
    const bool more = g + 1 < g_end;
    if (more) {
      rope_row(a, row + 4, lane, FULL || row + 4 < a.rows, rn);
      load_row<NIT, FULL>(nxt, base + (size_t)(row + 4) * ld, lane, nchunk, row + 4 < a.rows);
    }
    asm volatile("" ::: "memory");
    if (FULL || row < a.rows)
      qknorm_row<NIT, FULL>(a, cur, sg, rc, which == 0 ? a.q + (size_t)row * a.ldq : (a.k_dst[rc.lf] + (size_t)rc.tok * a.d), qs, lane, nchunk);
    if (!more) break;
#pragma unroll
    for (int it = 0; it < NIT; ++it) { cur[it] = nxt[it]; keep_packed(cur[it]); }
    rc = rn;
  }
}

__global__ void modulation_kernel(const bf16_t* mod, size_t mod_layer_stride, const bf16_t* e, int e_frame_stride, int bcast,
                                  bf16_t* emod, int n_layers, int n_frames, int nmod, int d) {
  const size_t per_frame = (size_t)nmod * d;
  const size_t total = (size_t)n_layers * n_frames * per_frame;
  for (size_t i = (size_t)blockIdx.x * blockDim.x + threadIdx.x; i < total; i += (size_t)gridDim.x * blockDim.x) {
    const size_t within = i % per_frame;
    const size_t lf = i / per_frame;
    const int f = (int)(lf % n_frames), l = (int)(lf / n_frames);
    const size_t ei = (size_t)f * e_frame_stride + (bcast ? within % d : within);
    emod[i] = f2bf(bf2f(mod[(size_t)l * mod_layer_stride + within]) + bf2f(e[ei]));
  }
}

__global__ void patchify_kernel(const bf16_t* x, bf16_t* a, int lda, int F, int C, int h, int w) {
  const int gh = h >> 1, gw = w >> 1;
  const size_t total = (size_t)F * gh * gw * lda;
  for (size_t i = (size_t)blockIdx.x * blockDim.x + threadIdx.x; i < total; i += (size_t)gridDim.x * blockDim.x) {
    const int col = (int)(i % lda);
    const size_t tokg = i / lda;
    const int c = col >> 2, ph = (col >> 1) & 1, pw = col & 1;
    const int gx = (int)(tokg % gw), gy = (int)((tokg / gw) % gh), f = (int)(tokg / ((size_t)gw * gh));
    a[i] = c < C ? x[(((size_t)f * C + c) * h + (2 * gy + ph)) * w + 2 * gx + pw] : (bf16_t)0;
  }
}

__global__ void unpatchify_kernel(const bf16_t* y, int ldy, bf16_t* out, int F, int C, int h, int w) {
  const int gh = h >> 1, gw = w >> 1;
  const size_t total = (size_t)F * C * h * w;
  for (size_t i = (size_t)blockIdx.x * blockDim.x + threadIdx.x; i < total; i += (size_t)gridDim.x * blockDim.x) {
    const int xx = (int)(i % w), yy = (int)((i / w) % h), c = (int)((i / ((size_t)w * h)) % C),
              f = (int)(i / ((size_t)w * h * C));
    const size_t tok = ((size_t)f * gh + (yy >> 1)) * gw + (xx >> 1);
    out[i] = y[tok * ldy + ((yy & 1) * 2 + (xx & 1)) * C + c];
  }
}

__global__ void sinusoid_kernel(const float* t, bf16_t* out, int F, int freq_dim) {
  const int half = freq_dim >> 1;
  const int i = blockIdx.x * blockDim.x + threadIdx.x;
  if (i >= F * half) return;
  const int f = i / half, k = i - f * half;
  const double ang = (double)t[f] * pow(10000.0, -(double)k / (double)half);
  out[(size_t)f * freq_dim + k] = f2bf((float)cos(ang));
  out[(size_t)f * freq_dim + half + k] = f2bf((float)sin(ang));
}

__global__ void silu_kernel(const bf16_t* x, bf16_t* y, size_t n) {
  for (size_t i = (size_t)blockIdx.x * blockDim.x + threadIdx.x; i < n; i += (size_t)gridDim.x * blockDim.x)
    y[i] = f2bf(silu(bf2f(x[i])));
}

MMPL_DEV void unipc_body(const UniPCArgs& a) {
  for (size_t i = (size_t)blockIdx.x * blockDim.x + threadIdx.x; i < a.n; i += (size_t)gridDim.x * blockDim.x) {
    float flow = bf2f(a.flow_c[i]);
    if (a.flow_u) {
      const float fu = bf2f(a.flow_u[i]);
      flow = rbf(fu + rbf(a.guidance * rbf(flow - fu)));
    }
    float x = bf2f(a.x[i]);
    const float m_conv = rbf(x - rbf(a.sigma_cur * flow));
    float m0 = bf2f(a.m0[i]), m1 = bf2f(a.m1[i]);
    if (a.use_corrector) {
      const float ls = bf2f(a.last_sample[i]);
      const float xt_ = rbf(rbf(a.c_c1 * ls) - rbf(a.c_c2 * m0));
      const float d1t = rbf(m_conv - m0);
      float acc = rbf(a.c_rho_last * d1t);
      if (a.corr_order == 2) {
        const float d1 = rbf(rbf(m1 - m0) * a.c_inv_rk);
        acc = rbf(rbf(a.c_rho0 * d1) + acc);
      }
      x = rbf(xt_ - rbf(a.c_c3 * acc));
    }
    m1 = m0;
    m0 = m_conv;
    a.m1[i] = f2bf(m1);
    a.m0[i] = f2bf(m0);
    a.last_sample[i] = f2bf(x);
    float xt = rbf(rbf(a.p_c1 * x) - rbf(a.p_c2 * m0));
    if (a.pred_order == 2) {
      const float d1 = rbf(rbf(m1 - m0) * a.p_inv_rk);
      xt = rbf(xt - rbf(a.p_c3 * rbf(0.5f * d1)));
    }
    a.x[i] = f2bf(xt);
  }
}
__global__ void unipc_kernel(UniPCArgs a) { unipc_body(a); }
__global__ void unipc_table_kernel(UniPCArgs a, const UniPCStepDev* table, const int* step, int n_steps) {
  if (*step >= n_steps) return;
  const UniPCStepDev st = table[*step];
  a.guidance = st.guidance; a.sigma_cur = st.sigma_cur; a.use_corrector = st.use_corrector; a.corr_order = st.corr_order;
  a.c_c1 = st.c_c1; a.c_c2 = st.c_c2; a.c_c3 = st.c_c3; a.c_inv_rk = st.c_inv_rk; a.c_rho0 = st.c_rho0; a.c_rho_last = st.c_rho_last;
  a.pred_order = st.pred_order; a.p_c1 = st.p_c1; a.p_c2 = st.p_c2; a.p_c3 = st.p_c3; a.p_inv_rk = st.p_inv_rk;
  unipc_body(a);
}
__global__ void unipc_advance_kernel(int* step, float* t_out, const float* t_tab, int n_t, int n_steps) {
  if (*step >= n_steps) return;
  const int nxt = *step + 1;
  __syncthreads();
  if (threadIdx.x == 0) *step = nxt;
  const float t = t_tab[nxt < n_steps ? nxt : n_steps - 1];
  for (int i = threadIdx.x; i < n_t; i += blockDim.x) t_out[i] = t;
}

inline int grid_for(size_t n, int block = 256) {
  size_t g = (n + block - 1) / block;
  return (int)(g > 2048 * 4 ? 2048 * 4 : (g == 0 ? 1 : g));
}

}

#define DISPATCH_NIT(NITV, KERNEL, ARGS, ROWS, STREAM)                                                     \
  switch (NITV) {                                                                                          \
    case 1: hipLaunchKernelGGL(KERNEL<1>, dim3(((ROWS) + 3) / 4), dim3(256), 0, STREAM, ARGS); break;      \
    case 2: hipLaunchKernelGGL(KERNEL<2>, dim3(((ROWS) + 3) / 4), dim3(256), 0, STREAM, ARGS); break;      \
    case 3: hipLaunchKernelGGL(KERNEL<3>, dim3(((ROWS) + 3) / 4), dim3(256), 0, STREAM, ARGS); break;      \
    case 4: hipLaunchKernelGGL(KERNEL<4>, dim3(((ROWS) + 3) / 4), dim3(256), 0, STREAM, ARGS); break;      \
    case 5: case 6: hipLaunchKernelGGL(KERNEL<6>, dim3(((ROWS) + 3) / 4), dim3(256), 0, STREAM, ARGS); break; \
    case 7: case 8: hipLaunchKernelGGL(KERNEL<8>, dim3(((ROWS) + 3) / 4), dim3(256), 0, STREAM, ARGS); break; \
    case 9: case 10: hipLaunchKernelGGL(KERNEL<10>, dim3(((ROWS) + 3) / 4), dim3(256), 0, STREAM, ARGS); break; \
    default: return hipErrorInvalidValue;                                                                  \
  }
template <typename K>
static int resident_blocks(K kernel, int* cache) {
  if (!*cache) {
    int per_cu = 0;
    if (hipOccupancyMaxActiveBlocksPerMultiprocessor(&per_cu, kernel, 256, 0) != hipSuccess || per_cu < 1) per_cu = 2;
    *cache = per_cu * 8 * mmpl_cus_per_xcd();
  }
  return *cache;
}
template <typename A>
static void launch_pipelined(void (*kernel)(A, int), int* cache, const A& a, int rows, int ny, hipStream_t s) {
  const int ngroups = (rows + 3) / 4, resident = resident_blocks(kernel, cache);
  int gpb = (ngroups + resident - 1) / resident;
  hipLaunchKernelGGL(kernel, dim3((ngroups + gpb - 1) / gpb, ny), dim3(256), 0, s, a, gpb);
}
#define PIPELINED_CASE(N, KERNEL, ARGS, ROWS, NY, STREAM, FULLV)                                           \
  { static int c0 = 0, c1 = 0;                                                                             \
    if (FULLV) launch_pipelined(KERNEL<N, true>, &c1, ARGS, ROWS, NY, STREAM);                             \
    else launch_pipelined(KERNEL<N, false>, &c0, ARGS, ROWS, NY, STREAM); }
#define DISPATCH_PIPELINED(NITV, KERNEL, ARGS, ROWS, NY, STREAM, FULLV)                                    \
  switch (NITV) {                                                                                          \
    case 1: PIPELINED_CASE(1, KERNEL, ARGS, ROWS, NY, STREAM, FULLV) break;                                \
    case 2: PIPELINED_CASE(2, KERNEL, ARGS, ROWS, NY, STREAM, FULLV) break;                                \
    case 3: PIPELINED_CASE(3, KERNEL, ARGS, ROWS, NY, STREAM, FULLV) break;                                \
    case 4: PIPELINED_CASE(4, KERNEL, ARGS, ROWS, NY, STREAM, FULLV) break;                                \
    case 5: case 6: PIPELINED_CASE(6, KERNEL, ARGS, ROWS, NY, STREAM, (FULLV) && (NITV) == 6) break;       \
    case 7: case 8: PIPELINED_CASE(8, KERNEL, ARGS, ROWS, NY, STREAM, (FULLV) && (NITV) == 8) break;       \
    case 9: case 10: PIPELINED_CASE(10, KERNEL, ARGS, ROWS, NY, STREAM, (FULLV) && (NITV) == 10) break;    \
    default: return hipErrorInvalidValue;                                                                  \
  }

hipError_t mmpl_launch_layernorm(const LnArgs& a, hipStream_t s) {
  if (a.rows <= 0) return hipSuccess;
  if (a.d % 8 || a.d > 5120 || a.ldx % 8 || a.ldy % 8) return hipErrorInvalidValue;
  const int nit = (a.d / 8 + 63) / 64;
  if (nit >= 6 && a.rows >= mmpl_config().ln_pipeline_min_rows) {
    const bool full = a.d == 512 * nit && a.rows % 4 == 0 && (a.w || a.rows_per_frame % 4 == 0);
    DISPATCH_PIPELINED(nit, layernorm_pipelined_kernel, a, a.rows, 1, s, full);
  } else {
    DISPATCH_NIT(nit, layernorm_kernel, a, a.rows, s);
  }
  return hipGetLastError();
}

hipError_t mmpl_launch_qknorm(const QkNormArgs& a, hipStream_t s) {
  if (a.rows <= 0) return hipSuccess;
  if (a.d % 128 || a.d > 5120 || a.ldq % 8 || a.ldk % 8 || a.ldv % 8) return hipErrorInvalidValue;
  if (a.v && !a.k) return hipErrorInvalidValue;
  const int nit = (a.d / 8 + 63) / 64;
  const bool full = a.d == 512 * nit && a.rows % 4 == 0;
  DISPATCH_PIPELINED(nit, qknorm_kernel, a, a.rows, 1 + (a.k ? 1 : 0) + (a.v ? 1 : 0), s, full);
  return hipGetLastError();
}

hipError_t mmpl_launch_rmsnorm(bf16_t* x, int ldx, const bf16_t* w, int rows, int d, float eps, hipStream_t s, float out_scale) {
  QkNormArgs a = {};
  a.q = x; a.ldq = ldx; a.wq = w; a.rows = rows; a.d = d; a.eps = eps; a.rope = 0; a.rows_per_frame = rows > 0 ? rows : 1;
  a.q_scale = out_scale;
  a.grid_w = 1;
  return mmpl_launch_qknorm(a, s);
}

hipError_t mmpl_launch_modulation(const bf16_t* mod, size_t mod_layer_stride, const bf16_t* e, int e_frame_stride, int bcast,
                                  bf16_t* emod, int n_layers, int n_frames, int nmod, int d, hipStream_t s) {
  const size_t n = (size_t)n_layers * n_frames * nmod * d;
  hipLaunchKernelGGL(modulation_kernel, dim3(grid_for(n)), dim3(256), 0, s, mod, mod_layer_stride, e, e_frame_stride, bcast, emod,
                     n_layers, n_frames, nmod, d);
  return hipGetLastError();
}
hipError_t mmpl_launch_patchify(const bf16_t* x, bf16_t* a, int lda, int F, int C, int h, int w, hipStream_t s) {
  const size_t n = (size_t)F * (h / 2) * (w / 2) * lda;
  hipLaunchKernelGGL(patchify_kernel, dim3(grid_for(n)), dim3(256), 0, s, x, a, lda, F, C, h, w);
  return hipGetLastError();
}
hipError_t mmpl_launch_unpatchify(const bf16_t* y, int ldy, bf16_t* out, int F, int C, int h, int w, hipStream_t s) {
  const size_t n = (size_t)F * C * h * w;
  hipLaunchKernelGGL(unpatchify_kernel, dim3(grid_for(n)), dim3(256), 0, s, y, ldy, out, F, C, h, w);
  return hipGetLastError();
}
__global__ __launch_bounds__(64) void rows_equal_last_kernel(const bf16_t* x, int ld, int rows, int d, int* flags) {
  const int r = blockIdx.x;
  const u32x4* a = reinterpret_cast<const u32x4*>(x + (size_t)r * ld);
  const u32x4* b = reinterpret_cast<const u32x4*>(x + (size_t)(rows - 1) * ld);
  bool same = true;
  for (int i = threadIdx.x; i < d / 8; i += 64) {
    const u32x4 u = a[i], v = b[i];
    same = same && u[0] == v[0] && u[1] == v[1] && u[2] == v[2] && u[3] == v[3];
  }
  const bool all = __all(same);
  if (threadIdx.x == 0) flags[r] = all ? 1 : 0;
}
hipError_t mmpl_launch_rows_equal_last(const bf16_t* x, int ld, int rows, int d, int* flags, hipStream_t s) {
  if (d % 8 || ld % 8) return hipErrorInvalidValue;
  hipLaunchKernelGGL(rows_equal_last_kernel, dim3(rows), dim3(64), 0, s, x, ld, rows, d, flags);
  return hipGetLastError();
}
__global__ __launch_bounds__(256) void pages_fingerprint_kernel(PageList pl, size_t words_per_page, unsigned long long* fp) {
  const size_t total = (size_t)pl.n * words_per_page;
  unsigned long long s1 = 0, s2 = 0;
  for (size_t i = (size_t)blockIdx.x * 256 + threadIdx.x; i < total; i += (size_t)gridDim.x * 256) {
    const size_t pg = i / words_per_page, off = i - pg * words_per_page;
    const unsigned long long w = reinterpret_cast<const uint32_t*>(pl.p[pg])[off];
    s1 += w;
    s2 += w * (unsigned long long)(i + 1);
  }
#pragma unroll
  for (int m = 32; m >= 1; m >>= 1) {
    s1 += __shfl_xor(s1, m, 64);
    s2 += __shfl_xor(s2, m, 64);
  }
  if ((threadIdx.x & 63) == 0) {
    atomicAdd(fp, s1);
    atomicAdd(fp + 1, s2);
  }
}
__global__ void share_check_zero_kernel(unsigned long long* chk, int which) {
  if (threadIdx.x < 2) chk[2 * which + threadIdx.x] = 0;
}
__global__ void share_check_compare_kernel(unsigned long long* chk) {
  if (threadIdx.x == 0 && (chk[0] != chk[2] || chk[1] != chk[3])) chk[4] += 1;
}
hipError_t mmpl_launch_pages_fingerprint(const PageList& pl, size_t bytes_per_page, unsigned long long* chk, int which, hipStream_t s) {
  if (pl.n < 1 || pl.n > MMPL_MAX_PAGES || bytes_per_page % 4) return hipErrorInvalidValue;
  hipLaunchKernelGGL(pages_fingerprint_kernel, dim3(2048), dim3(256), 0, s, pl, bytes_per_page / 4, chk + 2 * which);
  return hipGetLastError();
}
hipError_t mmpl_launch_share_check_zero(unsigned long long* chk, int which, hipStream_t s) {
  hipLaunchKernelGGL(share_check_zero_kernel, dim3(1), dim3(64), 0, s, chk, which);
  return hipGetLastError();
}
hipError_t mmpl_launch_share_check_compare(unsigned long long* chk, hipStream_t s) {
  hipLaunchKernelGGL(share_check_compare_kernel, dim3(1), dim3(64), 0, s, chk);
  return hipGetLastError();
}
__global__ void zero_ints_kernel(int* p, int n) {
  for (int i = threadIdx.x; i < n; i += blockDim.x) p[i] = 0;
}
hipError_t mmpl_launch_zero_ints(int* p, int n, hipStream_t s) {
  hipLaunchKernelGGL(zero_ints_kernel, dim3(1), dim3(64), 0, s, p, n);
  return hipGetLastError();
}
hipError_t mmpl_launch_sinusoid(const float* t, bf16_t* out, int F, int freq_dim, hipStream_t s) {
  const int n = F * (freq_dim / 2);
  hipLaunchKernelGGL(sinusoid_kernel, dim3((n + 255) / 256), dim3(256), 0, s, t, out, F, freq_dim);
  return hipGetLastError();
}
hipError_t mmpl_launch_silu(const bf16_t* x, bf16_t* y, size_t n, hipStream_t s) {
  hipLaunchKernelGGL(silu_kernel, dim3(grid_for(n)), dim3(256), 0, s, x, y, n);
  return hipGetLastError();
}
hipError_t mmpl_launch_unipc(const UniPCArgs& a, hipStream_t s) {
  hipLaunchKernelGGL(unipc_kernel, dim3(grid_for(a.n)), dim3(256), 0, s, a);
  return hipGetLastError();
}
hipError_t mmpl_launch_unipc_table(const UniPCArgs& a, const UniPCStepDev* table, int* step, float* t_out, const float* t_tab,
                                   int n_t, int n_steps, hipStream_t s) {
  hipLaunchKernelGGL(unipc_table_kernel, dim3(grid_for(a.n)), dim3(256), 0, s, a, table, step, n_steps);
  hipLaunchKernelGGL(unipc_advance_kernel, dim3(1), dim3(64), 0, s, step, t_out, t_tab, n_t, n_steps);
  return hipGetLastError();
}
```

### mmpl_amd/csrc/gemm.hip

```cpp
#include <stdlib.h>

#include "common.h"
#include "dev_knobs.h"
#include "kernels.h"
#include "w64_util.h"
#include "mmpl_config.h"

#ifdef MMPL_DEV_ABLATIONS
#define GEMM_DEV_TICKS [[maybe_unused]] unsigned long long tk0 = 0, tk1 = 0, tk2 = 0, tk3 = 0
#define GEMM_DEV_TICK(x) do { if constexpr (GEMM6_TIMING) x = __builtin_readcyclecounter(); } while (0)
#else
#define GEMM_DEV_TICKS do { } while (0)
#define GEMM_DEV_TICK(x) do { } while (0)
#endif

namespace {
using w64::sfor;

constexpr int BM = 128, BN = 128, BK = 64;
constexpr int TILE_BYTES = BM * BK * 2;

template <int EPI>
MMPL_DEV void gemm_epilogue(const GemmArgs& g, const f32x4 (&acc)[4][4], int mw, int nw, int frow, int fchunk) {
  const int m0 = 0, n0 = 0, wm = 0, wn = 0;
  (void)m0; (void)n0; (void)wm; (void)wn;
  uint2 bias4[4], res4[4][4], gate4[4][4];
#pragma unroll
  for (int j = 0; j < 4; ++j) {
    const int n = nw + 16 * j + 4 * fchunk;
    bias4[j] = (EPI != EPI_F32_SCALE && g.bias && n < g.N) ? *reinterpret_cast<const uint2*>(g.bias + n) : uint2{0u, 0u};
  }
  if (EPI == EPI_GATE_RES || EPI == EPI_RES) {
#pragma unroll
    for (int i = 0; i < 4; ++i) {
      const int m = mw + 16 * i + frow;
      const int frame = (EPI == EPI_GATE_RES && m < g.M) ? (m / g.rows_per_frame) : 0;
#pragma unroll
      for (int j = 0; j < 4; ++j) {
        const int n = nw + 16 * j + 4 * fchunk;
        const bool ok = m < g.M && n < g.N;
        res4[i][j] = ok ? *reinterpret_cast<const uint2*>(g.res + (size_t)m * g.ldres + n) : uint2{0u, 0u};
        if (EPI == EPI_GATE_RES)
          gate4[i][j] = ok ? *reinterpret_cast<const uint2*>(g.gate + (size_t)frame * g.gate_frame_stride + n) : uint2{0u, 0u};
      }
    }
  }
#pragma unroll
  for (int i = 0; i < 4; ++i) {
    const int m = mw + 16 * i + frow;
    if (m >= g.M) continue;
#pragma unroll
    for (int j = 0; j < 4; ++j) {
      const int n = nw + 16 * j + 4 * fchunk;
      if (n >= g.N) continue;
      if (EPI == EPI_F32_SCALE) {
        f32x4 o4;
#pragma unroll
        for (int r = 0; r < 4; ++r) o4[r] = acc[i][j][r] * g.alpha;
        *reinterpret_cast<f32x4*>(reinterpret_cast<float*>(g.C) + (size_t)m * g.ldc + n) = o4;
        continue;
      }
      float v[4];
      {
        const uint2 bb = bias4[j];
        const float b[4] = {bf2f(bb.x & 0xffff), bf2f(bb.x >> 16), bf2f(bb.y & 0xffff), bf2f(bb.y >> 16)};
#pragma unroll
        for (int r = 0; r < 4; ++r) v[r] = rbf(acc[i][j][r] + b[r]);
      }
      if (EPI == EPI_BIAS_GELU) {
#pragma unroll
        for (int r = 0; r < 4; ++r) v[r] = gelu_tanh(v[r]);
      } else if (EPI == EPI_BIAS_SILU) {
#pragma unroll
        for (int r = 0; r < 4; ++r) v[r] = silu(v[r]);
      } else if (EPI == EPI_GATE_RES || EPI == EPI_RES) {
        const uint2 xx = res4[i][j];
        float x[4] = {bf2f(xx.x & 0xffff), bf2f(xx.x >> 16), bf2f(xx.y & 0xffff), bf2f(xx.y >> 16)};
        if (EPI == EPI_GATE_RES) {
          const uint2 ee = gate4[i][j];
          float e[4] = {bf2f(ee.x & 0xffff), bf2f(ee.x >> 16), bf2f(ee.y & 0xffff), bf2f(ee.y >> 16)};
#pragma unroll
          for (int r = 0; r < 4; ++r) v[r] = rbf(v[r] * e[r]);
        }
#pragma unroll
        for (int r = 0; r < 4; ++r) v[r] = x[r] + v[r];
      }
      uint2 o;
      o.x = pack2bf(v[0], v[1]);
      o.y = pack2bf(v[2], v[3]);
      if (EPI == EPI_BIAS_VPAGES && n >= g.v_col0) {
        const int fr = m / g.rows_per_frame;
        *reinterpret_cast<uint2*>(g.v_dst[fr] + (size_t)(m - fr * g.rows_per_frame) * g.v_ld + (n - g.v_col0)) = o;
      } else {
        *reinterpret_cast<uint2*>(g.C + (size_t)m * g.ldc + n) = o;
      }
    }
  }
}

template <int EPI>
MMPL_DEV void gemm128_tile(const GemmArgs& g, char* smem, int m0, int n0) {
  char* As = smem;
  char* Ws = smem + 2 * TILE_BYTES;
  const int tid = threadIdx.x, lane = tid & 63, wave = tid >> 6;
  const int wm = wave >> 1, wn = wave & 1;

  const int srow = tid >> 3, schunk = tid & 7;
  const bf16_t* a_ptr[4];
  const bf16_t* w_ptr[4];
  int lds_off[4];
#pragma unroll
  for (int j = 0; j < 4; ++j) {
    const int row = srow + 32 * j;
    a_ptr[j] = g.A + (size_t)min(m0 + row, g.M - 1) * g.lda + schunk * 8;
    w_ptr[j] = g.W + (size_t)min(n0 + row, g.N - 1) * g.ldw + schunk * 8;
    lds_off[j] = row * 128 + ((schunk ^ (row & 7)) << 4);
  }
  u32x4 ra[4], rw[4];
  const int nt = g.K / BK;
#pragma unroll
  for (int j = 0; j < 4; ++j) {
    ra[j] = *reinterpret_cast<const u32x4*>(a_ptr[j]);
    rw[j] = *reinterpret_cast<const u32x4*>(w_ptr[j]);
  }
#pragma unroll
  for (int j = 0; j < 4; ++j) {
    *reinterpret_cast<u32x4*>(As + lds_off[j]) = ra[j];
    *reinterpret_cast<u32x4*>(Ws + lds_off[j]) = rw[j];
  }
  __syncthreads();

  f32x4 acc[4][4];
#pragma unroll
  for (int i = 0; i < 4; ++i)
#pragma unroll
    for (int j = 0; j < 4; ++j) acc[i][j] = f32x4{0.f, 0.f, 0.f, 0.f};

  const int frow = lane & 15, fchunk = lane >> 4;
  int a_off[4], w_off[4];
#pragma unroll
  for (int i = 0; i < 4; ++i) {
    const int ar = 64 * wm + 16 * i + frow, wr = 64 * wn + 16 * i + frow;
    a_off[i] = ar * 128 + ((fchunk ^ (ar & 7)) << 4);
    w_off[i] = wr * 128 + ((fchunk ^ (wr & 7)) << 4);
  }

  for (int t = 0; t < nt; ++t) {
    const int cur = t & 1;
    if (t + 1 < nt) {
      const int koff = (t + 1) * BK;
#pragma unroll
      for (int j = 0; j < 4; ++j) {
        ra[j] = *reinterpret_cast<const u32x4*>(a_ptr[j] + koff);
        rw[j] = *reinterpret_cast<const u32x4*>(w_ptr[j] + koff);
      }
    }
    const char* Ac = As + cur * TILE_BYTES;
    const char* Wc = Ws + cur * TILE_BYTES;
#pragma unroll
    for (int ks = 0; ks < 2; ++ks) {
      bf16x8 af[4], wf[4];
#pragma unroll
      for (int i = 0; i < 4; ++i) {
        af[i] = *reinterpret_cast<const bf16x8*>(Ac + (a_off[i] ^ (ks << 6)));
        wf[i] = *reinterpret_cast<const bf16x8*>(Wc + (w_off[i] ^ (ks << 6)));
      }
#pragma unroll
      for (int i = 0; i < 4; ++i)
#pragma unroll
        for (int j = 0; j < 4; ++j)
          acc[i][j] = __builtin_amdgcn_mfma_f32_16x16x32_bf16(wf[j], af[i], acc[i][j], 0, 0, 0);
    }
    if (t + 1 < nt) {
      char* An = As + (cur ^ 1) * TILE_BYTES;
      char* Wn = Ws + (cur ^ 1) * TILE_BYTES;
#pragma unroll
      for (int j = 0; j < 4; ++j) {
        *reinterpret_cast<u32x4*>(An + lds_off[j]) = ra[j];
        *reinterpret_cast<u32x4*>(Wn + lds_off[j]) = rw[j];
      }
    }
    __syncthreads();
  }

  gemm_epilogue<EPI>(g, acc, m0 + 64 * wm, n0 + 64 * wn, frow, fchunk);
}

template <int EPI>
__global__ __launch_bounds__(256) __attribute__((amdgpu_waves_per_eu(2, 2))) void gemm_bf16_kernel(GemmArgs g) {
  if (g.batch > 1) {
    g.A += (size_t)blockIdx.y * g.sA;
    g.W += (size_t)blockIdx.y * g.sW;
    g.C = (bf16_t*)((char*)g.C + (size_t)blockIdx.y * g.sC * (g.epi == EPI_F32_SCALE ? 4 : 2));
  }
  extern __shared__ __attribute__((aligned(16))) char smem[];
  const int tiles_m = (g.M + BM - 1) / BM, tiles_n = (g.N + BN - 1) / BN;
  const int nwg = tiles_m * tiles_n;
  int bid = blockIdx.x;
  {
    const int q = nwg >> 3, r = nwg & 7, xcd = bid & 7, idx = bid >> 3;
    bid = (xcd < r ? xcd * (q + 1) : r * (q + 1) + (xcd - r) * q) + idx;
  }
  constexpr int GROUP = 8;
  const int per_group = GROUP * tiles_n;
  const int gid = bid / per_group;
  const int first_m = gid * GROUP;
  const int gsz = min(tiles_m - first_m, GROUP);
  const int tm = first_m + (bid % per_group) % gsz;
  const int tn = (bid % per_group) / gsz;
  gemm128_tile<EPI>(g, smem, tm * BM, tn * BN);
}

constexpr int BM2 = 256, BN2 = 128;
constexpr int A2_BYTES = BM2 * BK * 2, W2_BYTES = BN2 * BK * 2, STAGE2 = A2_BYTES + W2_BYTES, NSTAGE2 = 3;

MMPL_DEV void glds16(const void* g, char* lds) {
  __builtin_amdgcn_global_load_lds((const __attribute__((address_space(1))) void*)g,
                                   (__attribute__((address_space(3))) void*)lds, 16, 0, 0);
}

template <int EPI>
__global__ __launch_bounds__(512) __attribute__((amdgpu_waves_per_eu(2, 2))) void gemm_bf16_v2_kernel(GemmArgs g) {
  extern __shared__ __attribute__((aligned(16))) char smem[];
  const int tiles_m = (g.M + BM2 - 1) / BM2, tiles_n = (g.N + BN2 - 1) / BN2;
  const int nwg = tiles_m * tiles_n;
  int bid = blockIdx.x;
  {
    const int q = nwg >> 3, r = nwg & 7, xcd = bid & 7, idx = bid >> 3;
    bid = (xcd < r ? xcd * (q + 1) : r * (q + 1) + (xcd - r) * q) + idx;
  }
  constexpr int GROUP = 4;
  const int per_group = GROUP * tiles_n;
  const int gid = bid / per_group;
  const int first_m = gid * GROUP;
  const int gsz = min(tiles_m - first_m, GROUP);
  const int tm = first_m + (bid % per_group) % gsz;
  const int tn = (bid % per_group) / gsz;
  const int m0 = tm * BM2, n0 = tn * BN2;

  const int tid = threadIdx.x, lane = tid & 63;
  const int wave = __builtin_amdgcn_readfirstlane(tid >> 6);
  const int wm = wave >> 1, wn = wave & 1;

  const bf16_t* a_src[4];
  const bf16_t* w_src[2];
#pragma unroll
  for (int j = 0; j < 4; ++j) {
    const int p = (j * 8 + wave) * 64 + lane, row = p >> 3, c = (p & 7) ^ (row & 7);
    a_src[j] = g.A + (size_t)min(m0 + row, g.M - 1) * g.lda + c * 8;
  }
#pragma unroll
  for (int j = 0; j < 2; ++j) {
    const int p = (j * 8 + wave) * 64 + lane, row = p >> 3, c = (p & 7) ^ (row & 7);
    w_src[j] = g.W + (size_t)min(n0 + row, g.N - 1) * g.ldw + c * 8;
  }
  auto issue = [&](int t) {
    char* st = smem + (t % NSTAGE2) * STAGE2;
    const int koff = t * BK;
#pragma unroll
    for (int j = 0; j < 4; ++j) glds16(a_src[j] + koff, st + (j * 8 + wave) * 1024);
#pragma unroll
    for (int j = 0; j < 2; ++j) glds16(w_src[j] + koff, st + A2_BYTES + (j * 8 + wave) * 1024);
  };

  f32x4 acc[4][4];
#pragma unroll
  for (int i = 0; i < 4; ++i)
#pragma unroll
    for (int j = 0; j < 4; ++j) acc[i][j] = f32x4{0.f, 0.f, 0.f, 0.f};
  const int frow = lane & 15, fchunk = lane >> 4;
  int a_off[4], w_off[4];
#pragma unroll
  for (int i = 0; i < 4; ++i) {
    const int ar = 64 * wm + 16 * i + frow, wr = 64 * wn + 16 * i + frow;
    a_off[i] = ar * 128 + ((fchunk ^ (ar & 7)) << 4);
    w_off[i] = A2_BYTES + wr * 128 + ((fchunk ^ (wr & 7)) << 4);
  }

  const int nt = g.K / BK;
  issue(0);
  if (nt > 1) {
    issue(1);
    asm volatile("s_waitcnt vmcnt(6)" ::: "memory");
  } else {
    asm volatile("s_waitcnt vmcnt(0)" ::: "memory");
  }
  __builtin_amdgcn_s_barrier();

  for (int t = 0; t < nt; ++t) {
    if (t + 2 < nt) issue(t + 2);
    const char* st = smem + (t % NSTAGE2) * STAGE2;
#pragma unroll
    for (int ks = 0; ks < 2; ++ks) {
      bf16x8 af[4], wf[4];
#pragma unroll
      for (int i = 0; i < 4; ++i) {
        af[i] = *reinterpret_cast<const bf16x8*>(st + (a_off[i] ^ (ks << 6)));
        wf[i] = *reinterpret_cast<const bf16x8*>(st + (w_off[i] ^ (ks << 6)));
      }
#pragma unroll
      for (int i = 0; i < 4; ++i)
#pragma unroll
        for (int j = 0; j < 4; ++j)
          acc[i][j] = __builtin_amdgcn_mfma_f32_16x16x32_bf16(wf[j], af[i], acc[i][j], 0, 0, 0);
    }
    if (t + 2 < nt) asm volatile("s_waitcnt vmcnt(6)" ::: "memory");
    else asm volatile("s_waitcnt vmcnt(0)" ::: "memory");
    __builtin_amdgcn_s_barrier();
  }
  gemm_epilogue<EPI>(g, acc, m0 + 64 * wm, n0 + 64 * wn, frow, fchunk);
}

constexpr int BM3 = 256, BN3 = 256;

constexpr int BK4 = 64, A4_BYTES = BM3 * BK4 * 2, STAGE4 = 2 * A4_BYTES;
MMPL_DEV int swz64(int r, int c) { return r * 128 + ((c ^ (r & 7)) << 4); }

#define GEMM_POL_STR_0 ""
#define GEMM_POL_STR_1 " nt"
#define GEMM_POL_STR_2 " sc1"
#define GEMM_POL_STR_3 " sc0 sc1"
#define GEMM_POL_CAT(n) GEMM_POL_STR_##n
#define GEMM_POL_STR(n) GEMM_POL_CAT(n)
#define GEMM_POL_A GEMM_POL_STR(GEMM_POLICY_A)
#define GEMM_POL_W GEMM_POL_STR(GEMM_POLICY_W)
MMPL_DEV void glds16s(const void* base, uint32_t voff, char* lds) {
  const uint32_t dst = (uint32_t)(size_t)((__attribute__((address_space(3))) char*)lds);
  asm volatile("s_mov_b32 m0, %2\n\ts_nop 0\n\tglobal_load_lds_dwordx4 %0, %1" ::"v"(voff), "s"(base), "s"(dst) : "memory");
}
MMPL_DEV void glds16s_a(const void* base, uint32_t voff, char* lds) {
  const uint32_t dst = (uint32_t)(size_t)((__attribute__((address_space(3))) char*)lds);
  asm volatile("s_mov_b32 m0, %2\n\ts_nop 0\n\tglobal_load_lds_dwordx4 %0, %1" GEMM_POL_A ::"v"(voff), "s"(base), "s"(dst) : "memory");
}
MMPL_DEV void glds16s_w(const void* base, uint32_t voff, char* lds) {
  const uint32_t dst = (uint32_t)(size_t)((__attribute__((address_space(3))) char*)lds);
  asm volatile("s_mov_b32 m0, %2\n\ts_nop 0\n\tglobal_load_lds_dwordx4 %0, %1" GEMM_POL_W ::"v"(voff), "s"(base), "s"(dst) : "memory");
}

MMPL_DEV void store16_c(void* p, const uint4& v) {
  const u32x4 w = {v.x, v.y, v.z, v.w};
#if GEMM6_STORE == 1
  asm volatile("global_store_dwordx4 %0, %1, off nt\n\ts_nop 1" ::"v"(p), "v"(w) : "memory");
#elif GEMM6_STORE == 2
  asm volatile("global_store_dwordx4 %0, %1, off sc1\n\ts_nop 1" ::"v"(p), "v"(w) : "memory");
#elif GEMM6_STORE == 3
  asm volatile("global_store_dwordx4 %0, %1, off sc0 sc1\n\ts_nop 1" ::"v"(p), "v"(w) : "memory");
#else
  *reinterpret_cast<u32x4*>(p) = w;
#endif
}
MMPL_DEV void glds4s(const void* base, uint32_t voff, char* lds) {
  const uint32_t dst = (uint32_t)(size_t)((__attribute__((address_space(3))) char*)lds);
  asm volatile("s_mov_b32 m0, %2\n\ts_nop 0\n\tglobal_load_lds_dword %0, %1" ::"v"(voff), "s"(base), "s"(dst) : "memory");
}

struct EpiIn {
  uint2 bias4[4];
  uint4 res8[16];
  uint4 gate_lo, gate_hi;
  int m_split;
};
template <int EPI>
MMPL_DEV void epi_load_bias(const GemmArgs& g, EpiIn& in, int nw, int lane) {
  const int fchunk = lane >> 4;
#pragma unroll
  for (int j = 0; j < 4; ++j) {
    const int nb = nw + 16 * j + 4 * fchunk;
    in.bias4[j] = (g.bias && nb < g.N) ? *reinterpret_cast<const uint2*>(g.bias + nb) : uint2{0u, 0u};
  }
  asm volatile("" ::"v"(in.bias4[0].x), "v"(in.bias4[1].x), "v"(in.bias4[2].x), "v"(in.bias4[3].x));
}
template <int EPI, int U0 = 0, int U1 = 16>
MMPL_DEV void epi_load_res(const GemmArgs& g, EpiIn& in, int mw, int nw, int lane) {
  constexpr bool HAS_RES = EPI == EPI_GATE_RES || EPI == EPI_RES;
  const int erow = lane >> 3, ec = lane & 7, n = nw + 8 * ec;
  const bool n_ok = n < g.N;
  if (HAS_RES) {
#pragma unroll
    for (int u = U0; u < U1; ++u) {
      const int m = mw + 8 * u + erow;
      if ((GEMM6_ABL & 16) && g.M >= 0) {
        in.res8[u] = uint4{0x3f803f80u, 0x3f803f80u, 0x3f803f80u, 0x3f803f80u};
      } else if (n_ok && m < g.M) {
        const u32x4* rp = reinterpret_cast<const u32x4*>(g.res + (size_t)m * g.ldres + n);
        const u32x4 rv = GEMM6_RESLD ? __builtin_nontemporal_load(rp) : *rp;
        in.res8[u] = uint4{rv[0], rv[1], rv[2], rv[3]};
      } else {
        in.res8[u] = uint4{0u, 0u, 0u, 0u};
      }
    }
  }
  if (U0 != 0) return;
  in.gate_lo = uint4{0u, 0u, 0u, 0u};
  in.gate_hi = in.gate_lo;
  in.m_split = 0;
  if (EPI == EPI_GATE_RES && n_ok) {
    const int f_lo = min(mw, g.M - 1) / g.rows_per_frame;
    const int f_hi = min(mw + 127, g.M - 1) / g.rows_per_frame;
    in.m_split = (f_lo + 1) * g.rows_per_frame;
    in.gate_lo = *reinterpret_cast<const uint4*>(g.gate + (size_t)f_lo * g.gate_frame_stride + n);
    in.gate_hi = *reinterpret_cast<const uint4*>(g.gate + (size_t)f_hi * g.gate_frame_stride + n);
  }
}
template <int EPI>
MMPL_DEV void epi_stage(const f32x4 (&acc)[2][4][4], const EpiIn& in, char* stg, int lane) {
  const int frow = lane & 15, fchunk = lane >> 4;
#pragma unroll
  for (int h = 0; h < 2; ++h)
#pragma unroll
    for (int i = 0; i < 4; ++i) {
      const int row = 64 * h + 16 * i + frow;
#pragma unroll
      for (int j = 0; j < 4; ++j) {
        const float b[4] = {__uint_as_float(in.bias4[j].x << 16), __uint_as_float(in.bias4[j].x & 0xffff0000u),
                            __uint_as_float(in.bias4[j].y << 16), __uint_as_float(in.bias4[j].y & 0xffff0000u)};
        float v[4];
#pragma unroll
        for (int r = 0; r < 4; ++r) {
          v[r] = rbf(acc[h][i][j][r] + b[r]);
          if (EPI == EPI_BIAS_GELU) v[r] = gelu_tanh(v[r]);
          if (EPI == EPI_BIAS_SILU) v[r] = silu(v[r]);
        }
        const int c = 2 * j + (fchunk >> 1);
        *reinterpret_cast<uint2*>(stg + row * 128 + ((c ^ (row & 7)) << 4) + 8 * (fchunk & 1)) = uint2{pack2bf(v[0], v[1]), pack2bf(v[2], v[3])};
      }
    }
  __builtin_amdgcn_fence(__ATOMIC_RELEASE, "wavefront");
  __builtin_amdgcn_wave_barrier();
  __builtin_amdgcn_fence(__ATOMIC_ACQUIRE, "wavefront");
}
template <int EPI>
MMPL_DEV void epi_finish(const GemmArgs& g, const EpiIn& in, const char* stg, int mw, int nw, int lane) {
  constexpr bool HAS_RES = EPI == EPI_GATE_RES || EPI == EPI_RES;
  const int erow = lane >> 3, ec = lane & 7, n = nw + 8 * ec;
  const bool n_ok = n < g.N;
#pragma unroll
  for (int u = 0; u < 16; ++u) {
    const int row = 8 * u + erow, m = mw + row;
    const uint4 yv = *reinterpret_cast<const uint4*>(stg + row * 128 + ((ec ^ (row & 7)) << 4));
    if (m >= g.M || !n_ok) continue;
    uint4 ov = yv;
    if (HAS_RES) {
      uint4 ev = uint4{0u, 0u, 0u, 0u};
      if (EPI == EPI_GATE_RES) ev = (m < in.m_split) ? in.gate_lo : in.gate_hi;
      const uint32_t yw[4] = {yv.x, yv.y, yv.z, yv.w}, xw[4] = {in.res8[u].x, in.res8[u].y, in.res8[u].z, in.res8[u].w}, ew[4] = {ev.x, ev.y, ev.z, ev.w};
      float v[8];
#pragma unroll
      for (int e = 0; e < 8; ++e) {
        float y = __uint_as_float((e & 1) ? (yw[e >> 1] & 0xffff0000u) : (yw[e >> 1] << 16));
        const float x = __uint_as_float((e & 1) ? (xw[e >> 1] & 0xffff0000u) : (xw[e >> 1] << 16));
        if (EPI == EPI_GATE_RES) y = rbf(y * __uint_as_float((e & 1) ? (ew[e >> 1] & 0xffff0000u) : (ew[e >> 1] << 16)));
        v[e] = x + y;
      }
      ov.x = pack2bf(v[0], v[1]); ov.y = pack2bf(v[2], v[3]); ov.z = pack2bf(v[4], v[5]); ov.w = pack2bf(v[6], v[7]);
    }
    if ((GEMM6_ABL & 8) && g.M >= 0) { asm volatile("" ::"v"(ov.x), "v"(ov.y), "v"(ov.z), "v"(ov.w)); continue; }
    if (EPI == EPI_BIAS_VPAGES && n >= g.v_col0) {
      const int fr = m / g.rows_per_frame;
      store16_c(g.v_dst[fr] + (size_t)(m - fr * g.rows_per_frame) * g.v_ld + (n - g.v_col0), ov);
    } else {
      store16_c(g.C + (size_t)m * g.ldc + n, ov);
    }
  }
}
template <int EPI>
MMPL_DEV void gemm_epilogue_staged(const GemmArgs& g, const f32x4 (&acc)[2][4][4], char* stg, int mw, int nw, int lane) {
  EpiIn in;
  epi_load_bias<EPI>(g, in, nw, lane);
  epi_load_res<EPI>(g, in, mw, nw, lane);
  epi_stage<EPI>(acc, in, stg, lane);
  epi_finish<EPI>(g, in, stg, mw, nw, lane);
}

MMPL_DEV void store16_sys(f32x4* p, const f32x4& v) {
  asm volatile("global_store_dwordx4 %0, %1, off sc0 sc1\n\ts_nop 1" ::"v"(p), "v"(v) : "memory");
}
MMPL_DEV void load16x8_sys(const f32x4* p, f32x4 (&v)[8]) {
  asm volatile("global_load_dwordx4 %0, %8, off sc0 sc1\n\t"
               "global_load_dwordx4 %1, %8, off offset:1024 sc0 sc1\n\t"
               "global_load_dwordx4 %2, %8, off offset:2048 sc0 sc1\n\t"
               "global_load_dwordx4 %3, %8, off offset:3072 sc0 sc1\n\t"
               "global_load_dwordx4 %4, %9, off sc0 sc1\n\t"
               "global_load_dwordx4 %5, %9, off offset:1024 sc0 sc1\n\t"
               "global_load_dwordx4 %6, %9, off offset:2048 sc0 sc1\n\t"
               "global_load_dwordx4 %7, %9, off offset:3072 sc0 sc1\n\t"
               "s_waitcnt vmcnt(0)"
               : "=&v"(v[0]), "=&v"(v[1]), "=&v"(v[2]), "=&v"(v[3]), "=&v"(v[4]), "=&v"(v[5]), "=&v"(v[6]), "=&v"(v[7])
               : "v"(p), "v"(p + 256)
               : "memory");
}

template <int EPI, bool SPLITK = false>
__global__ __launch_bounds__(512) __attribute__((amdgpu_waves_per_eu(2, 2))) void gemm_bf16_v6_kernel(GemmArgs g) {
  extern __shared__ __attribute__((aligned(16))) char smem[];
  GEMM_DEV_TICKS;
  GEMM_DEV_TICK(tk0);
  const int tiles_m = (g.M + BM3 - 1) / BM3, tiles_n = (g.N + BN3 - 1) / BN3;
  const int nwg = tiles_m * tiles_n;
  __shared__ int s_ticket;
  const bool persistent = !SPLITK && g.tile_counter != nullptr;
  const int my_xcd = blockIdx.x & 7;
  const int GROUP = g.group;
  const int per_group = GROUP * tiles_n;
  const int full_groups = tiles_m / GROUP;
  const int rounds = g.sync_sweeps ? full_groups >> 3 : 0;
  const int dealt = rounds * per_group;
  const int left = nwg - 8 * dealt;
  const int lq = left >> 3, lr = left & 7;
  const int chunk_all = dealt + lq + (my_xcd < lr ? 1 : 0);
  const int chunk_main = g.splitk_s > 1 ? chunk_all - chunk_all % g.splitk_per : chunk_all;
  const int chunk = SPLITK ? chunk_all : chunk_main;
  [[maybe_unused]] int part = 0, slot = 0;
  const int blocks_x = (int)(gridDim.x >> 3) + (my_xcd < (int)(gridDim.x & 7) ? 1 : 0);
  for (;;) {
  int idx = blockIdx.x >> 3;
  if constexpr (SPLITK) {
    const int t_local = idx / g.splitk_s;
    part = idx - t_local * g.splitk_s;
    slot = my_xcd * g.splitk_tb + t_local;
    idx = chunk_main + t_local;
    if (idx >= chunk) return;
  }
  if (persistent) {
    if (threadIdx.x == 0) s_ticket = atomicAdd(g.tile_counter + my_xcd, 1);
    __syncthreads();
    const int ticket = s_ticket;
    if (ticket >= chunk) {
      if (ticket == chunk + blocks_x - 1 && threadIdx.x == 0) g.tile_counter[my_xcd] = 0;
      return;
    }
    idx = ticket;
  }
  int bid;
  if (idx < dealt) {
    bid = ((idx / per_group) * 8 + my_xcd) * per_group + idx % per_group;
  } else {
    bid = 8 * dealt + (my_xcd < lr ? my_xcd * (lq + 1) : lr * (lq + 1) + (my_xcd - lr) * lq) + (idx - dealt);
  }
  const int gid = bid / per_group;
  const int first_m = gid * GROUP;
  const int gsz = min(tiles_m - first_m, GROUP);
  const int tm = first_m + (bid % per_group) % gsz;
  const int tn = (bid % per_group) / gsz;
  const int m0 = tm * BM3, n0 = tn * BN3;
  const int tid = threadIdx.x, lane = tid & 63;
  const int wave = __builtin_amdgcn_readfirstlane(tid >> 6);
  const int wm = wave >> 2, wn = wave & 3, grp = wave >> 2;

  const int prow = lane >> 3, lc = ((lane & 7) ^ (prow & 7)) << 3;
  const int nt_all = g.K / BK4;
  const int kt0 = SPLITK ? part * nt_all / g.splitk_s : 0;
  const int nt = SPLITK ? (part + 1) * nt_all / g.splitk_s - kt0 : nt_all;
  const bf16_t* const A_k0 = g.A + (size_t)kt0 * BK4;
  const bf16_t* const W_k0 = g.W + (size_t)kt0 * BK4;
  const bf16_t* a_k = A_k0;
  const bf16_t* w_k = W_k0;
  auto issue_piece = [&](int q, char* st) {
    const bool isw = q >= 8;
    const int p = 4 * (q & 7) + wave;
    int row = isw ? min(n0 + 8 * p + prow, g.N - 1) : min(m0 + 8 * p + prow, g.M - 1);
    if constexpr (GEMM6_ABL & 1) row = 8 * p + prow;
    const uint32_t voff = (uint32_t)(row * (isw ? g.ldw : g.lda) + lc) * 2u;
    if (isw) glds16s_w(w_k, voff, st + A4_BYTES + p * 1024);
    else glds16s_a(a_k, voff, st + p * 1024);
  };

  f32x4 acc[2][4][4];
#pragma unroll
  for (int h = 0; h < 2; ++h)
#pragma unroll
    for (int i = 0; i < 4; ++i)
#pragma unroll
      for (int j = 0; j < 4; ++j) acc[h][i][j] = f32x4{0.f, 0.f, 0.f, 0.f};
  const int frow = lane & 15, fchunk = lane >> 4;
  int a_off[8], w_off[4];
#pragma unroll
  for (int i = 0; i < 8; ++i) a_off[i] = swz64(128 * wm + 16 * i + frow, fchunk);
#pragma unroll
  for (int i = 0; i < 4; ++i) w_off[i] = A4_BYTES + swz64(64 * wn + 16 * i + frow, fchunk);
  const bool pf_on = g.pf_dist > 0 && grp == 1 && gsz >= 2;
  const int pf_P = 32 / gsz;
  const int pf_nw = __builtin_amdgcn_readfirstlane(2 * (256 / gsz)), pf_na = __builtin_amdgcn_readfirstlane(2 * (256 / pf_P));
  const int pf_wrow0 = __builtin_amdgcn_readfirstlane(n0 + ((bid % per_group) % gsz) * (256 / gsz));
  const int pf_arow0 = __builtin_amdgcn_readfirstlane(m0 + (tn % pf_P) * (256 / pf_P));

  if (grp == 0) {
#pragma unroll
    for (int q = 0; q < 16; ++q) issue_piece(q, smem);
    a_k += BK4;
    w_k += BK4;
    asm volatile("s_waitcnt vmcnt(0)" ::: "memory");
  }
  __builtin_amdgcn_s_barrier();
  if (grp == 1) __builtin_amdgcn_s_barrier();
  GEMM_DEV_TICK(tk1);

  for (int t = 0; t < nt; ++t) {
    if (pf_on && t + g.pf_dist < nt) {
      const int l = (wave - 4) * 64 + lane;
      char* dump = smem + 2 * STAGE4 + (wave - 4) * 256;
      const size_t koff = (size_t)(t + g.pf_dist) * BK4;
      if (l < pf_nw) glds4s(W_k0 + koff, (uint32_t)(min(pf_wrow0 + (l >> 1), g.N - 1) * g.ldw + (l & 1) * 32) * 2u, dump);
      if (l < pf_na) glds4s(A_k0 + koff, (uint32_t)(min(pf_arow0 + (l >> 1), g.M - 1) * g.lda + (l & 1) * 32) * 2u, dump);
    }
    const char* st = smem + (t & 1) * STAGE4;
    char* nx = smem + ((t + 1) & 1) * STAGE4;
    const bool do_issue = grp == 0 && t + 1 < nt && !(GEMM6_ABL & 4);
    bf16x8 af[2][8], wf[2][4];
#pragma unroll
    for (int ks = 0; ks < 2; ++ks) {
#pragma unroll
      for (int i = 0; i < 4; ++i) {
        wf[ks][i] = *reinterpret_cast<const bf16x8*>(st + (w_off[i] ^ (ks << 6)));
        if (do_issue) issue_piece(ks * 8 + i, nx);
      }
#pragma unroll
      for (int i = 0; i < 8; ++i) {
        af[ks][i] = *reinterpret_cast<const bf16x8*>(st + (a_off[i] ^ (ks << 6)));
        if ((i & 1) && do_issue) issue_piece(ks * 8 + 4 + (i >> 1), nx);
      }
    }
    if (do_issue) { a_k += BK4; w_k += BK4; }
    asm volatile("s_waitcnt lgkmcnt(0)" ::: "memory");
#pragma unroll
    for (int ks = 0; ks < 2; ++ks) {
      asm volatile("" : "+v"(af[ks][0]), "+v"(af[ks][1]), "+v"(af[ks][2]), "+v"(af[ks][3]), "+v"(af[ks][4]), "+v"(af[ks][5]),
                        "+v"(af[ks][6]), "+v"(af[ks][7]), "+v"(wf[ks][0]), "+v"(wf[ks][1]), "+v"(wf[ks][2]), "+v"(wf[ks][3]));
    }
    __builtin_amdgcn_s_barrier();
    __builtin_amdgcn_s_setprio(1);
#pragma unroll
    for (int ks = 0; ks < 2; ++ks)
#pragma unroll
      for (int i = 0; i < 8; ++i)
#pragma unroll
        for (int j = 0; j < 4; ++j)
          acc[i >> 2][i & 3][j] = __builtin_amdgcn_mfma_f32_16x16x32_bf16(wf[ks][j], af[ks][i], acc[i >> 2][i & 3][j], 0, 0, 0);
    __builtin_amdgcn_s_setprio(0);
    if (grp == 0) asm volatile("s_waitcnt vmcnt(0)" ::: "memory");
    if (grp == 0 || t + 1 < nt) __builtin_amdgcn_s_barrier();
  }
  GEMM_DEV_TICK(tk2);
  if constexpr (SPLITK) {
    const size_t part_floats = (size_t)8 * 32 * 64 * 4;
    f32x4* wsp = reinterpret_cast<f32x4*>(g.splitk_ws + ((size_t)slot * g.splitk_s + part) * part_floats) + (size_t)wave * 32 * 64 + lane;
#pragma unroll
    for (int r = 0; r < 32; ++r) store16_sys(wsp + r * 64, acc[r >> 4][(r >> 2) & 3][r & 3]);
    asm volatile("s_waitcnt vmcnt(0)" ::: "memory");
    __syncthreads();
    if (threadIdx.x == 0) s_ticket = __hip_atomic_fetch_add(g.splitk_cnt + slot, 1, __ATOMIC_RELAXED, __HIP_MEMORY_SCOPE_AGENT);
    __syncthreads();
    if (s_ticket != g.splitk_s - 1) return;
    if (threadIdx.x == 0) g.splitk_cnt[slot] = 0;
    const f32x4* rsp = reinterpret_cast<const f32x4*>(g.splitk_ws + (size_t)slot * g.splitk_s * part_floats) + (size_t)wave * 32 * 64 + lane;
    for (int p = 0; p < g.splitk_s; ++p) {
#pragma unroll
      for (int r0 = 0; r0 < 32; r0 += 8) {
        f32x4 v[8];
        load16x8_sys(rsp + r0 * 64, v);
#pragma unroll
        for (int i = 0; i < 8; ++i) {
          const int r = r0 + i;
          f32x4& a = acc[r >> 4][(r >> 2) & 3][r & 3];
          if (p == 0) a = v[i];
          else { a[0] += v[i][0]; a[1] += v[i][1]; a[2] += v[i][2]; a[3] += v[i][3]; }
        }
      }
      rsp += part_floats / 4;
    }
  }
  if constexpr (GEMM6_ABL & 2) {
    if (g.M < 0) gemm_epilogue<EPI>(g, acc[0], m0 + 128 * wm, n0 + 64 * wn, frow, fchunk);
  } else if (EPI != EPI_F32_SCALE && g.staged_epilogue) {
    gemm_epilogue_staged<EPI>(g, acc, smem + wave * (128 * 128), m0 + 128 * wm, n0 + 64 * wn, lane);
  } else {
    gemm_epilogue<EPI>(g, acc[0], m0 + 128 * wm, n0 + 64 * wn, frow, fchunk);
    gemm_epilogue<EPI>(g, acc[1], m0 + 128 * wm + 64, n0 + 64 * wn, frow, fchunk);
  }
#ifdef MMPL_DEV_ABLATIONS
  if constexpr (GEMM6_TIMING) {
    asm volatile("s_waitcnt vmcnt(0)" ::: "memory");
    tk3 = __builtin_readcyclecounter();
    __syncthreads();
    if (lane == 0 && (wave & 1) == 0) {
      float* tp = reinterpret_cast<float*>(g.C) + (blockIdx.x * 4 + (wave >> 1)) * 4;
      tp[0] = (float)(tk1 - tk0);
      tp[1] = (float)(tk2 - tk1);
      tp[2] = (float)(tk3 - tk2);
      tp[3] = (float)(2 * nt);
    }
  }
#endif
  if (g.pf_dist > 0 && grp == 1) asm volatile("s_waitcnt vmcnt(0)" ::: "memory");
  if (!persistent) return;
  __syncthreads();
  }
}

template <int EPI>
MMPL_DEV void gemm128_ring_tile(const GemmArgs& g, char* smem, int m0, int n0) {
  constexpr int NST = 4, STG = 2 * TILE_BYTES;
  const int tid = threadIdx.x, lane = tid & 63;
  const int wave = __builtin_amdgcn_readfirstlane(tid >> 6);
  const int wm = wave >> 1, wn = wave & 1;
  const int prow = lane >> 3, lc = ((lane & 7) ^ (prow & 7)) << 3;
  uint32_t a_vo[4], w_vo[4];
#pragma unroll
  for (int q = 0; q < 4; ++q) {
    const int p = 4 * q + wave;
    a_vo[q] = (uint32_t)(min(m0 + 8 * p + prow, g.M - 1) * g.lda + lc) * 2u;
    w_vo[q] = (uint32_t)(min(n0 + 8 * p + prow, g.N - 1) * g.ldw + lc) * 2u;
  }
  const int nt = g.K / BK;
  auto issue = [&](int t) {
    char* st = smem + (t & (NST - 1)) * STG;
    const bf16_t* ak = g.A + (size_t)t * BK;
    const bf16_t* wk = g.W + (size_t)t * BK;
#pragma unroll
    for (int q = 0; q < 4; ++q) glds16s(ak, a_vo[q], st + (4 * q + wave) * 1024);
#pragma unroll
    for (int q = 0; q < 4; ++q) glds16s(wk, w_vo[q], st + TILE_BYTES + (4 * q + wave) * 1024);
  };
  f32x4 acc[4][4];
#pragma unroll
  for (int i = 0; i < 4; ++i)
#pragma unroll
    for (int j = 0; j < 4; ++j) acc[i][j] = f32x4{0.f, 0.f, 0.f, 0.f};
  const int frow = lane & 15, fchunk = lane >> 4;
  int a_off[4], w_off[4];
#pragma unroll
  for (int i = 0; i < 4; ++i) {
    const int ar = 64 * wm + 16 * i + frow, wr = 64 * wn + 16 * i + frow;
    a_off[i] = ar * 128 + ((fchunk ^ (ar & 7)) << 4);
    w_off[i] = TILE_BYTES + wr * 128 + ((fchunk ^ (wr & 7)) << 4);
  }
  const int pre = nt < NST - 1 ? nt : NST - 1;
  for (int t = 0; t < pre; ++t) issue(t);
  if (pre >= 3) asm volatile("s_waitcnt vmcnt(16)" ::: "memory");
  else if (pre == 2) asm volatile("s_waitcnt vmcnt(8)" ::: "memory");
  else asm volatile("s_waitcnt vmcnt(0)" ::: "memory");
  __syncthreads();
#pragma unroll 1
  for (int t = 0; t < nt; ++t) {
    if (t + NST - 1 < nt) issue(t + NST - 1);
    const char* st = smem + (t & (NST - 1)) * STG;
#pragma unroll
    for (int ks = 0; ks < 2; ++ks) {
      bf16x8 af[4], wf[4];
#pragma unroll
      for (int i = 0; i < 4; ++i) {
        af[i] = *reinterpret_cast<const bf16x8*>(st + (a_off[i] ^ (ks << 6)));
        wf[i] = *reinterpret_cast<const bf16x8*>(st + (w_off[i] ^ (ks << 6)));
      }
#pragma unroll
      for (int i = 0; i < 4; ++i)
#pragma unroll
        for (int j = 0; j < 4; ++j) acc[i][j] = __builtin_amdgcn_mfma_f32_16x16x32_bf16(wf[j], af[i], acc[i][j], 0, 0, 0);
    }
    const int later = (t + 3 < nt ? 1 : 0) + (t + 2 < nt ? 1 : 0);
    if (later == 2) asm volatile("s_waitcnt vmcnt(16)" ::: "memory");
    else if (later == 1) asm volatile("s_waitcnt vmcnt(8)" ::: "memory");
    else asm volatile("s_waitcnt vmcnt(0)" ::: "memory");
    __syncthreads();
  }
  gemm_epilogue<EPI>(g, acc, m0 + 64 * wm, n0 + 64 * wn, frow, fchunk);
}

template <int EPI, bool RING>
__global__ __launch_bounds__(256) __attribute__((amdgpu_waves_per_eu(2, 2))) void gemm_tail128_kernel(GemmArgs g) {
  extern __shared__ __attribute__((aligned(16))) char smem[];
  const int tiles_m = (g.M + BM3 - 1) / BM3, tiles_n = (g.N + BN3 - 1) / BN3;
  const int nwg = tiles_m * tiles_n;
  const int my_xcd = blockIdx.x & 7, r = blockIdx.x >> 3, t_local = r >> 2, quad = r & 3;
  const int GROUP = g.group, per_group = GROUP * tiles_n;
  const int rounds = g.sync_sweeps ? (tiles_m / GROUP) >> 3 : 0;
  const int dealt = rounds * per_group, left = nwg - 8 * dealt, lq = left >> 3, lr = left & 7;
  const int chunk_all = dealt + lq + (my_xcd < lr ? 1 : 0);
  const int idx = chunk_all - chunk_all % g.splitk_per + t_local;
  if (idx >= chunk_all) return;
  int bid;
  if (idx < dealt) bid = ((idx / per_group) * 8 + my_xcd) * per_group + idx % per_group;
  else bid = 8 * dealt + (my_xcd < lr ? my_xcd * (lq + 1) : lr * (lq + 1) + (my_xcd - lr) * lq) + (idx - dealt);
  const int first_m = (bid / per_group) * GROUP;
  const int gsz = min(tiles_m - first_m, GROUP);
  const int tm = first_m + (bid % per_group) % gsz, tn = (bid % per_group) / gsz;
  const int m0 = tm * BM3 + 128 * (quad >> 1), n0 = tn * BN3 + 128 * (quad & 1);
  if (m0 >= g.M || n0 >= g.N) return;
  if constexpr (RING) gemm128_ring_tile<EPI>(g, smem, m0, n0);
  else gemm128_tile<EPI>(g, smem, m0, n0);
}

struct G8 {
  bf16x8 af[2][8], wf[2][8];
  uint32_t ra[2][2], rw[2][2];
  uint32_t a_vo[8], w_vo[8];
  const bf16_t* a_k; const bf16_t* w_k;
  const bf16_t* a_last; const bf16_t* w_last;
  uint32_t dst0;
  uint32_t pf_wo, pf_ao, pf_dump;

  template <int KS, int I, int J, bool ZERO = false> MMPL_DEV void mfma() {
    constexpr int c = 4 * (8 * I + J);
    if constexpr (ZERO) asm volatile("v_mfma_f32_16x16x32_bf16 a[%c0:%c1], %2, %3, 0" ::"i"(c), "i"(c + 3), "v"(wf[KS][J]), "v"(af[KS][I]));
    else asm volatile("v_mfma_f32_16x16x32_bf16 a[%c0:%c1], %2, %3, a[%c0:%c1]" ::"i"(c), "i"(c + 3), "v"(wf[KS][J]), "v"(af[KS][I]));
  }
  template <int S, int KS, int R> MMPL_DEV void lds() {
    if constexpr (GEMM8_ABL & 4) return;
    if constexpr (R < 8) asm volatile("ds_read_b128 %0, %1 offset:%c2" : "=v"(wf[KS][R]) : "v"(rw[S][KS]), "i"(2048 * R));
    else asm volatile("ds_read_b128 %0, %1 offset:%c2" : "=v"(af[KS][R - 8]) : "v"(ra[S][KS]), "i"(2048 * (R - 8)));
  }
  template <int S, int Q> MMPL_DEV void dma() {
    if constexpr (GEMM8_ABL & 1) return;
    constexpr int q = Q & 7;
    const uint32_t m = dst0 + S * STAGE4 + (Q < 8 ? 0 : A4_BYTES) + 4096 * q;
    if constexpr (Q < 8) asm volatile("s_mov_b32 m0, %2\n\ts_nop 0\n\tglobal_load_lds_dwordx4 %0, %1" GEMM_POL_A ::"v"(a_vo[q]), "s"(a_k), "s"(m) : "memory");
    else asm volatile("s_mov_b32 m0, %2\n\ts_nop 0\n\tglobal_load_lds_dwordx4 %0, %1" GEMM_POL_W ::"v"(w_vo[q]), "s"(w_k), "s"(m) : "memory");
  }
  MMPL_DEV void prefetch() {
    if constexpr (GEMM8_ABL & 1) return;
    const bf16_t* pw = w_k + BK4 <= w_last ? w_k + BK4 : w_last;
    const bf16_t* pa = a_k + BK4 <= a_last ? a_k + BK4 : a_last;
    asm volatile("s_mov_b32 m0, %2\n\ts_nop 0\n\tglobal_load_lds_dword %0, %1" ::"v"(pf_wo), "s"(pw), "s"(pf_dump) : "memory");
    asm volatile("s_mov_b32 m0, %2\n\ts_nop 0\n\tglobal_load_lds_dword %0, %1" ::"v"(pf_ao), "s"(pa), "s"(pf_dump + 256u) : "memory");
  }
};

template <int S, bool ISSUE, bool NEXT, bool FIRST = false> MMPL_DEV void gemm8_tile(G8& k) {
  constexpr int D1 = GEMM8_BAR1 + 2;
  constexpr int N1 = (64 - D1 + GEMM8_DMAS - 1) / GEMM8_DMAS;
  static_assert(N1 >= 0 && N1 <= 16 && (16 - N1) * GEMM8_DMAS + 1 < GEMM8_BAR2 && GEMM8_BAR2 + GEMM8_RD * 16 < 64 && GEMM8_RD * 15 < GEMM8_BAR1, "placement");
  if constexpr (GEMM8_FINEWAIT) asm volatile("s_waitcnt lgkmcnt(7)" ::: "memory");
  else asm volatile("s_waitcnt lgkmcnt(0)" ::: "memory");
  sfor<64>([&k](auto gi) {
    constexpr int g = decltype(gi)::value;
    if constexpr (GEMM8_FINEWAIT && g % 8 == 0 && g > 0) {
      constexpr int i = g / 8, n_new = (g + GEMM8_RD - 1) / GEMM8_RD < 16 ? (g + GEMM8_RD - 1) / GEMM8_RD : 16;
      constexpr int n = 7 - i + n_new < 15 ? 7 - i + n_new : 15;
      asm volatile("s_waitcnt lgkmcnt(%c0)" ::"i"(n) : "memory");
    }
    k.template mfma<0, g / 8, g % 8, FIRST>();
    if constexpr (g % GEMM8_RD == 0 && g / GEMM8_RD < 16) k.template lds<S, 1, g / GEMM8_RD>();
    if constexpr (g == GEMM8_BAR1 && !(GEMM8_ABL & 8)) asm volatile("s_waitcnt lgkmcnt(0)\n\ts_barrier" ::: "memory");
    if constexpr (ISSUE && g >= D1 && (g - D1) % GEMM8_DMAS == 0) k.template dma<S, (g - D1) / GEMM8_DMAS>();
  });
  sfor<64>([&k](auto gi) {
    constexpr int g = decltype(gi)::value;
    k.template mfma<1, g / 8, g % 8>();
    if constexpr (ISSUE && g % GEMM8_DMAS == 0 && N1 + g / GEMM8_DMAS < 16) k.template dma<S, N1 + g / GEMM8_DMAS>();
    if constexpr (ISSUE && GEMM8_PF && g == (16 - N1) * GEMM8_DMAS) k.prefetch();
    if constexpr (NEXT && g == GEMM8_BAR2 && !(GEMM8_ABL & 8)) {
      if constexpr (ISSUE) asm volatile("s_waitcnt vmcnt(%c0)\n\ts_barrier" ::"i"(GEMM8_PF ? 20 : 16) : "memory");
      else asm volatile("s_waitcnt vmcnt(0)\n\ts_barrier" ::: "memory");
    }
    if constexpr (NEXT && g > GEMM8_BAR2 && (g - GEMM8_BAR2) % GEMM8_RD == 0 && (g - GEMM8_BAR2) / GEMM8_RD <= 16)
      k.template lds<S ^ 1, 0, (g - GEMM8_BAR2) / GEMM8_RD - 1>();
  });
  if constexpr (ISSUE) { k.a_k += BK4; k.w_k += BK4; }
}

template <int EPI>
__global__ __launch_bounds__(256) __attribute__((amdgpu_waves_per_eu(1, 1))) void gemm_bf16_v8_kernel(GemmArgs g) {
  extern __shared__ __attribute__((aligned(16))) char smem[];
  __shared__ int s_ticket;
  const int tiles_m = (g.M + BM3 - 1) / BM3, tiles_n = (g.N + BN3 - 1) / BN3;
  const int nwg = tiles_m * tiles_n;
  const bool persistent = g.tile_counter != nullptr;
  const int my_xcd = blockIdx.x & 7;
  const int GROUP = g.group;
  const int per_group = GROUP * tiles_n;
  const int full_groups = tiles_m / GROUP;
  const int rounds = g.sync_sweeps ? full_groups >> 3 : 0;
  const int dealt = rounds * per_group;
  const int left = nwg - 8 * dealt;
  const int lq = left >> 3, lr = left & 7;
  const int chunk_all = dealt + lq + (my_xcd < lr ? 1 : 0);
  const int chunk = g.splitk_s > 1 ? chunk_all - chunk_all % g.splitk_per : chunk_all;
  const int blocks_x = (int)(gridDim.x >> 3) + (my_xcd < (int)(gridDim.x & 7) ? 1 : 0);
  const int tid = threadIdx.x, lane = tid & 63;
  const int wave = __builtin_amdgcn_readfirstlane(tid >> 6);
  const int wm = wave >> 1, wn = wave & 1;
  const int frow = lane & 15, fchunk = lane >> 4;
  GEMM_DEV_TICKS;
  GEMM_DEV_TICK(tk0);
  asm volatile("s_nop 0" ::: MMPL_ALL_AGPRS);

  G8 k;
  {
    const uint32_t ring = (uint32_t)(size_t)((__attribute__((address_space(3))) char*)smem);
#pragma unroll
    for (int s = 0; s < 2; ++s)
#pragma unroll
      for (int ks = 0; ks < 2; ++ks) {
        k.ra[s][ks] = ring + s * STAGE4 + (swz64(128 * wm + frow, fchunk) ^ (ks << 6));
        k.rw[s][ks] = ring + s * STAGE4 + A4_BYTES + (swz64(128 * wn + frow, fchunk) ^ (ks << 6));
      }
    k.dst0 = ring + 1024 * wave;
    k.pf_dump = ring + 2 * STAGE4 + 512 * wave;
  }
  const int prow = lane >> 3, lc = ((lane & 7) ^ (prow & 7)) << 3;
  const int nt = g.K / BK4;

  for (;;) {
    int idx = blockIdx.x >> 3;
    if (persistent) {
      if (threadIdx.x == 0) s_ticket = atomicAdd(g.tile_counter + my_xcd, 1);
      __syncthreads();
      const int ticket = s_ticket;
      if (ticket >= chunk) {
        if (ticket == chunk + blocks_x - 1 && threadIdx.x == 0) g.tile_counter[my_xcd] = 0;
        return;
      }
      idx = ticket;
    } else if (idx >= chunk) {
      return;
    }
    int bid;
    if (idx < dealt) bid = ((idx / per_group) * 8 + my_xcd) * per_group + idx % per_group;
    else bid = 8 * dealt + (my_xcd < lr ? my_xcd * (lq + 1) : lr * (lq + 1) + (my_xcd - lr) * lq) + (idx - dealt);
    const int gid = bid / per_group;
    const int first_m = gid * GROUP;
    const int gsz = min(tiles_m - first_m, GROUP);
    const int tm = first_m + (bid % per_group) % gsz;
    const int tn = (bid % per_group) / gsz;
    const int m0 = tm * BM3, n0 = tn * BN3;

#pragma unroll
    for (int q = 0; q < 8; ++q) {
      const int p = 4 * q + wave;
      k.a_vo[q] = (uint32_t)(min(m0 + 8 * p + prow, g.M - 1) * g.lda + lc) * 2u;
      k.w_vo[q] = (uint32_t)(min(n0 + 8 * p + prow, g.N - 1) * g.ldw + lc) * 2u;
    }
    k.a_k = g.A; k.w_k = g.W;
    k.a_last = g.A + (size_t)(nt - 1) * BK4; k.w_last = g.W + (size_t)(nt - 1) * BK4;
    if constexpr (GEMM8_PF) {
      const int P = 32 / gsz, nw = 2 * (256 / gsz), na = 2 * (256 / P);
      const int l = wave * 64 + lane;
      const int wrow0 = n0 + ((bid % per_group) % gsz) * (256 / gsz), arow0 = m0 + (tn % P) * (256 / P);
      const int lw = (g.pf_dist > 0 && l < nw) ? l : 0, la = (g.pf_dist > 0 && l < na) ? l : 0;
      k.pf_wo = (uint32_t)(min(wrow0 + (lw >> 1), g.N - 1) * g.ldw + (lw & 1) * 32) * 2u;
      k.pf_ao = (uint32_t)(min(arow0 + (la >> 1), g.M - 1) * g.lda + (la & 1) * 32) * 2u;
    }
    if (nt < 4) sfor<256>([](auto ii) { asm volatile("v_accvgpr_write_b32 a[%c0], 0" ::"i"(decltype(ii)::value)); });

    sfor<16>([&k](auto q) { k.template dma<0, decltype(q)::value>(); });
    k.a_k += BK4; k.w_k += BK4;
    if (nt > 1) {
      sfor<16>([&k](auto q) { k.template dma<1, decltype(q)::value>(); });
      if constexpr (GEMM8_PF) k.prefetch();
      k.a_k += BK4; k.w_k += BK4;
      asm volatile("s_waitcnt vmcnt(%c0)\n\ts_barrier" ::"i"(GEMM8_PF ? 18 : 16) : "memory");
    } else {
      asm volatile("s_waitcnt vmcnt(0)\n\ts_barrier" ::: "memory");
    }
    sfor<16>([&k](auto r) { k.template lds<0, 0, decltype(r)::value>(); });

    GEMM_DEV_TICK(tk1);
    int t = 0;
    if (nt >= 4) {
      gemm8_tile<0, true, true, true>(k);
      gemm8_tile<1, true, true>(k);
      t = 2;
    }
#pragma unroll 1
    for (; t + 3 < nt; t += 2) {
      gemm8_tile<0, true, true>(k);
      gemm8_tile<1, true, true>(k);
    }
    if (nt - t == 3) {
      gemm8_tile<0, true, true>(k);
      gemm8_tile<1, false, true>(k);
      gemm8_tile<0, false, false>(k);
    } else if (nt - t == 2) {
      gemm8_tile<0, false, true>(k);
      gemm8_tile<1, false, false>(k);
    } else {
      gemm8_tile<0, false, false>(k);
    }
    asm volatile("s_waitcnt vmcnt(0) lgkmcnt(0)\n\ts_nop 15\n\ts_nop 15" ::: "memory");
    GEMM_DEV_TICK(tk2);

    int lane_e = lane;
    asm volatile("" : "+v"(lane_e));
    const int frow_e = lane_e & 15, fchunk_e = lane_e >> 4;
    const int mw = m0 + 128 * wm, nw0 = n0 + 128 * wn;
    auto read_half = [](auto nhi, f32x4 (&acc)[2][4][4]) {
      constexpr int nh = decltype(nhi)::value;
      sfor<128>([&acc](auto ii) {
        constexpr int x = decltype(ii)::value, i8 = x >> 4, j = (x >> 2) & 3, r = x & 3;
        float v;
        asm volatile("v_accvgpr_read_b32 %0, a[%c1]" : "=v"(v) : "i"(4 * (8 * i8 + 4 * nh + j) + r));
        acc[i8 >> 2][i8 & 3][j][r] = v;
      });
    };
    if (EPI != EPI_F32_SCALE && g.staged_epilogue) {
      char* stg0 = smem + wave * 32768;
      EpiIn in0, in1;
      epi_load_bias<EPI>(g, in0, nw0, lane_e);
      epi_load_res<EPI>(g, in0, mw, nw0, lane_e);
      {
        f32x4 acc[2][4][4];
        read_half(w64::ic<0>{}, acc);
        epi_stage<EPI>(acc, in0, stg0, lane_e);
      }
      epi_load_bias<EPI>(g, in1, nw0 + 64, lane_e);
      constexpr int NPRE = 8;
      epi_load_res<EPI, 0, NPRE>(g, in1, mw, nw0 + 64, lane_e);
      epi_finish<EPI>(g, in0, stg0, mw, nw0, lane_e);
      {
        f32x4 acc[2][4][4];
        read_half(w64::ic<1>{}, acc);
        epi_stage<EPI>(acc, in1, stg0 + 16384, lane_e);
      }
      epi_load_res<EPI, NPRE, 16>(g, in1, mw, nw0 + 64, lane_e);
      epi_finish<EPI>(g, in1, stg0 + 16384, mw, nw0 + 64, lane_e);
    } else {
      sfor<2>([&](auto nhi) {
        constexpr int nh = decltype(nhi)::value;
        f32x4 acc[2][4][4];
        read_half(nhi, acc);
        gemm_epilogue<EPI>(g, acc[0], mw, nw0 + 64 * nh, frow_e, fchunk_e);
        gemm_epilogue<EPI>(g, acc[1], mw + 64, nw0 + 64 * nh, frow_e, fchunk_e);
      });
    }
#ifdef MMPL_DEV_ABLATIONS
    if constexpr (GEMM6_TIMING) {
      asm volatile("s_waitcnt vmcnt(0)" ::: "memory");
      tk3 = __builtin_readcyclecounter();
      __syncthreads();
      if (lane == 0) {
        float* tp = reinterpret_cast<float*>(g.C) + (blockIdx.x * 4 + wave) * 4;
        tp[0] = (float)(tk1 - tk0);
        tp[1] = (float)(tk2 - tk1);
        tp[2] = (float)(tk3 - tk2);
        tp[3] = (float)(2 * nt);
      }
    }
#endif
    if (!persistent) return;
    __syncthreads();
  }
}

template <int EPI>
hipError_t launch_v6(const GemmArgs& g, hipStream_t s) {
  constexpr int smem = 2 * STAGE4 + 1024;
  if (hipError_t e = mmpl_dyn_smem_once(reinterpret_cast<const void*>(gemm_bf16_v6_kernel<EPI>), smem); e != hipSuccess) return e;
  if (hipError_t e = mmpl_dyn_smem_once(reinterpret_cast<const void*>(gemm_bf16_v6_kernel<EPI, true>), smem); e != hipSuccess) return e;
  if (hipError_t e = mmpl_dyn_smem_once(reinterpret_cast<const void*>(gemm_bf16_v8_kernel<EPI>), 2 * STAGE4 + 2048); e != hipSuccess) return e;
  if (hipError_t e = mmpl_dyn_smem_once(reinterpret_cast<const void*>(gemm_tail128_kernel<EPI, true>), 8 * TILE_BYTES); e != hipSuccess) return e;
  if (hipError_t e = mmpl_dyn_smem_once(reinterpret_cast<const void*>(gemm_tail128_kernel<EPI, false>), 4 * TILE_BYTES); e != hipSuccess) return e;
  const int env_v8 = mmpl_config().gemm_v8;
  const bool use_v8 = env_v8 >= 0 ? env_v8 != 0 : g.N >= 8192;
  const int tiles = ((g.M + BM3 - 1) / BM3) * ((g.N + BN3 - 1) / BN3);
  GemmArgs g2 = g;
  const MmplRuntimeConfig& rc = mmpl_config();
  const int env_group = rc.gemm_group;
  const int tiles_m_ = (g.M + BM3 - 1) / BM3;
  g2.group = env_group > 0 ? env_group : ((tiles_m_ >= 96 && g.N < 8192 && g.K < 8192) ? 8 : 4);
  auto al = [](const void* p, uintptr_t a) { return p == nullptr || reinterpret_cast<uintptr_t>(p) % a == 0; };
  bool ptrs_ok = al(g.C, 16) && al(g.bias, 8);
  if (g.epi == EPI_GATE_RES || g.epi == EPI_RES) ptrs_ok = ptrs_ok && al(g.res, 16);
  if (g.epi == EPI_GATE_RES) ptrs_ok = ptrs_ok && al(g.gate, 16);
  if (g.epi == EPI_BIAS_VPAGES)
    for (int i = 0; i < 8; ++i) ptrs_ok = ptrs_ok && al(g.v_dst[i], 16);
  g2.staged_epilogue = ptrs_ok && g.N % 8 == 0 && g.ldc % 8 == 0 &&
                       (g.epi != EPI_GATE_RES || (g.gate_frame_stride % 8 == 0 && g.rows_per_frame >= 128)) &&
                       ((g.epi != EPI_GATE_RES && g.epi != EPI_RES) || g.ldres % 8 == 0) &&
                       (g.epi != EPI_BIAS_VPAGES || (g.v_col0 % 8 == 0 && g.v_ld % 8 == 0));
  g2.pf_dist = rc.gemm_pf;
  g2.sync_sweeps = 1;
  const int per = mmpl_cus_per_xcd(), n_cu = 8 * per;
  g2.splitk_s = 1; g2.splitk_tb = 0; g2.splitk_per = per;
  if (g2.tile_counter && g.splitk_ws && g.splitk_cnt && !rc.gemm_no_splitk && EPI != EPI_F32_SCALE && g.K / BK4 >= 64) {
    const int tiles_n_ = (g.N + BN3 - 1) / BN3, per_group = g2.group * tiles_n_;
    const int dealt = g2.sync_sweeps ? ((tiles_m_ / g2.group) >> 3) * per_group : 0, left = tiles - 8 * dealt;
    int tb = 0, main_tiles = 0;
    for (int x = 0; x < 8; ++x) {
      const int chunk = dealt + (left >> 3) + (x < (left & 7) ? 1 : 0);
      tb = chunk % per > tb ? chunk % per : tb;
      main_tiles += chunk - chunk % per;
    }
    int sp = tb > 0 ? per / tb : 1;
    sp = sp > 4 ? 4 : sp;
    if (sp >= 2 && (size_t)8 * tb * sp * (BM3 * BN3 * sizeof(float)) <= mmpl_gemm_splitk_ws_bytes()) {
      g2.splitk_s = sp; g2.splitk_tb = tb;
      if (main_tiles > 0) {
        if (use_v8) hipLaunchKernelGGL(gemm_bf16_v8_kernel<EPI>, dim3(main_tiles < n_cu ? main_tiles : n_cu), dim3(256), 2 * STAGE4 + 2048, s, g2);
        else hipLaunchKernelGGL(gemm_bf16_v6_kernel<EPI>, dim3(main_tiles < n_cu ? main_tiles : n_cu), dim3(512), smem, s, g2);
      }
      hipLaunchKernelGGL((gemm_bf16_v6_kernel<EPI, true>), dim3(8 * tb * sp), dim3(512), smem, s, g2);
      return hipGetLastError();
    }
  }
  if (g2.tile_counter && !rc.gemm_no_splitk && !rc.gemm_no_subtile && EPI != EPI_F32_SCALE && g.K / BK4 < 64) {
    const int tiles_n_ = (g.N + BN3 - 1) / BN3, per_group = g2.group * tiles_n_;
    const int dealt = g2.sync_sweeps ? ((tiles_m_ / g2.group) >> 3) * per_group : 0, left = tiles - 8 * dealt;
    int tb = 0, main_tiles = 0;
    for (int x = 0; x < 8; ++x) {
      const int chunk = dealt + (left >> 3) + (x < (left & 7) ? 1 : 0);
      tb = chunk % per > tb ? chunk % per : tb;
      main_tiles += chunk - chunk % per;
    }
    if (tb > 0 && 2 * tb <= per) {
      g2.splitk_s = 4; g2.splitk_tb = tb;
      if (main_tiles > 0) {
        if (use_v8) hipLaunchKernelGGL(gemm_bf16_v8_kernel<EPI>, dim3(main_tiles < n_cu ? main_tiles : n_cu), dim3(256), 2 * STAGE4 + 2048, s, g2);
        else hipLaunchKernelGGL(gemm_bf16_v6_kernel<EPI>, dim3(main_tiles < n_cu ? main_tiles : n_cu), dim3(512), smem, s, g2);
      }
      if (4 * tb <= per) hipLaunchKernelGGL((gemm_tail128_kernel<EPI, true>), dim3(8 * tb * 4), dim3(256), 8 * TILE_BYTES, s, g2);
      else hipLaunchKernelGGL((gemm_tail128_kernel<EPI, false>), dim3(8 * tb * 4), dim3(256), 4 * TILE_BYTES, s, g2);
      return hipGetLastError();
    }
  }
  const int blocks = g2.tile_counter && tiles > n_cu ? n_cu : tiles;
  if (blocks == tiles) g2.tile_counter = nullptr;
  if (use_v8) hipLaunchKernelGGL(gemm_bf16_v8_kernel<EPI>, dim3(blocks), dim3(256), 2 * STAGE4 + 2048, s, g2);
  else hipLaunchKernelGGL(gemm_bf16_v6_kernel<EPI>, dim3(blocks), dim3(512), smem, s, g2);
  return hipGetLastError();
}

template <int EPI>
hipError_t launch_v2(const GemmArgs& g, hipStream_t s) {
  constexpr int smem = NSTAGE2 * STAGE2;
  if (hipError_t e = mmpl_dyn_smem_once(reinterpret_cast<const void*>(gemm_bf16_v2_kernel<EPI>), smem); e != hipSuccess) return e;
  const int tiles = ((g.M + BM2 - 1) / BM2) * ((g.N + BN2 - 1) / BN2);
  hipLaunchKernelGGL(gemm_bf16_v2_kernel<EPI>, dim3(tiles), dim3(512), smem, s, g);
  return hipGetLastError();
}

template <int EPI>
hipError_t launch(const GemmArgs& g, hipStream_t s) {
  const bool env_v1 = mmpl_config().gemm_v1, env_v2 = mmpl_config().gemm_v2;
  const bool big = g.batch <= 1 && g.M >= 1024 && g.N >= 256 && g.K >= 128 && !env_v1 && !env_v2;
  if (big && (long long)g.M * g.lda < (1ll << 31) && (long long)g.N * g.ldw < (1ll << 31)) return launch_v6<EPI>(g, s);
  if (g.batch <= 1 && g.M >= 1024 && g.N >= 128 && g.K >= 128 && !env_v1) return launch_v2<EPI>(g, s);
  constexpr int smem = 4 * TILE_BYTES;
  if (hipError_t e = mmpl_dyn_smem_once(reinterpret_cast<const void*>(gemm_bf16_kernel<EPI>), smem); e != hipSuccess) return e;
  const int tiles = ((g.M + BM - 1) / BM) * ((g.N + BN - 1) / BN);
  hipLaunchKernelGGL(gemm_bf16_kernel<EPI>, dim3(tiles, g.batch > 1 ? g.batch : 1), dim3(256), smem, s, g);
  return hipGetLastError();
}

}

size_t mmpl_gemm_splitk_ws_bytes() { return (size_t)256 * BM3 * BN3 * sizeof(float); }

hipError_t mmpl_launch_gemm(const GemmArgs& g, hipStream_t s) {
  if (g.M <= 0 || g.N <= 0) return hipSuccess;
  if (g.K % BK != 0 || g.N % 4 != 0 || g.lda % 8 != 0 || g.ldw % 8 != 0 || g.ldc % 4 != 0) return hipErrorInvalidValue;
  switch (g.epi) {
    case EPI_BIAS: return launch<EPI_BIAS>(g, s);
    case EPI_BIAS_GELU: return launch<EPI_BIAS_GELU>(g, s);
    case EPI_BIAS_SILU: return launch<EPI_BIAS_SILU>(g, s);
    case EPI_GATE_RES: return launch<EPI_GATE_RES>(g, s);
    case EPI_RES: return launch<EPI_RES>(g, s);
    case EPI_F32_SCALE: return launch<EPI_F32_SCALE>(g, s);
    case EPI_BIAS_VPAGES: return launch<EPI_BIAS_VPAGES>(g, s);
  }
  return hipErrorInvalidValue;
}
```

### mmpl_amd/csrc/kernels.h

```cpp
#pragma once
#include <hip/hip_runtime.h>
#include <stdint.h>
#include "common.h"

hipError_t mmpl_dyn_smem_once(const void* func, int bytes);
int mmpl_cus_per_xcd();

enum GemmEpi { EPI_BIAS = 0, EPI_BIAS_GELU = 1, EPI_BIAS_SILU = 2, EPI_GATE_RES = 3, EPI_RES = 4, EPI_F32_SCALE = 5,
               EPI_BIAS_VPAGES = 6 };
struct GemmArgs {
  const bf16_t* A; int lda;
  const bf16_t* W; int ldw;
  const bf16_t* bias;
  bf16_t* C; int ldc;
  int M, N, K;
  int epi;
  const bf16_t* res; int ldres;
  const bf16_t* gate;
  int gate_frame_stride;
  int rows_per_frame;
  float alpha;
  int group;
  int batch;
  long sA, sW, sC;
  bf16_t* v_dst[8]; int v_col0, v_ld;
  int staged_epilogue;
  int* tile_counter;
  int pf_dist;
  int sync_sweeps;
  float* splitk_ws; int* splitk_cnt;
  int splitk_s, splitk_tb, splitk_per;
};
size_t mmpl_gemm_splitk_ws_bytes();
bool mmpl_xcd_dispatch_ok(bool may_probe);
hipError_t mmpl_launch_gemm(const GemmArgs& g, hipStream_t s);

constexpr int MMPL_MAX_PAGES = 24;
struct AttnArgs {
  const bf16_t* q; int ldq;
  bf16_t* o; int ldo;
  const bf16_t* k_pages[MMPL_MAX_PAGES];
  const bf16_t* v_pages[MMPL_MAX_PAGES];
  int ldk, ldv;
  int n_pages, page_rows;
  int page_rows_each[MMPL_MAX_PAGES];
  unsigned char page_group[MMPL_MAX_PAGES];
  int Lq, H;
  float scale;
  int cross;
  float* split_ws; size_t split_ws_bytes;
  int variant;
  int q_prescaled;
  int last_row_copies;
  unsigned long long* redo_stats;
  unsigned char* history;
  short* history_mem;
};
__device__ __forceinline__ bool mmpl_attn_item(int H, int n_qb, int xcd, int local, int& head, int& qb) {
  if ((H & 7) == 0) {
    head = xcd + 8 * (local / n_qb);
    qb = local % n_qb;
    return head < H;
  }
  const int total = n_qb * H, per = (total + 7) >> 3, item = xcd * per + local;
  if (local >= per || item >= total) return false;
  head = item / n_qb;
  qb = item % n_qb;
  return true;
}
enum { ATTN_AUTO = 0, ATTN_LOCKSTEP = 1, ATTN_W64 = 3 };
int mmpl_attention_self_variant();
int mmpl_attention_w64_smem();
const void* mmpl_attention_w64_symbol(int split);
void mmpl_launch_attention_w64(const AttnArgs& a, int blocks, int local_base, int sp, bool split, hipStream_t s);
size_t mmpl_attention_split_ws_bytes();
inline size_t mmpl_attention_history_state_bytes(int Lq, int H) { return ((size_t)H * ((Lq + 255) / 256) * 4 + 255) & ~(size_t)255; }
inline size_t mmpl_attention_history_bytes(int Lq, int H) { return mmpl_attention_history_state_bytes(Lq, H) + (size_t)H * ((Lq + 255) / 256) * 4 * 128 * sizeof(short); }
hipError_t mmpl_launch_attention(const AttnArgs& a, hipStream_t s);

struct LnArgs {
  const bf16_t* x; int ldx;
  bf16_t* y; int ldy;
  int rows, d;
  float eps;
  const bf16_t* scale; const bf16_t* shift; int mod_frame_stride; int rows_per_frame;
  const bf16_t* w; const bf16_t* b;
};
hipError_t mmpl_launch_layernorm(const LnArgs& a, hipStream_t s);

struct QkNormArgs {
  bf16_t* q; int ldq;
  const bf16_t* k; int ldk;
  const bf16_t* v; int ldv;
  const bf16_t* wq; const bf16_t* wk;
  int rows, d;
  float eps;
  float q_scale;
  int rope;
  const float* cos_tab; const float* sin_tab;
  int frame_ids[8];
  bf16_t* k_dst[8]; bf16_t* v_dst[8];
  int rows_per_frame, grid_w;
};
hipError_t mmpl_launch_qknorm(const QkNormArgs& a, hipStream_t s);

hipError_t mmpl_launch_rmsnorm(bf16_t* x, int ldx, const bf16_t* w, int rows, int d, float eps, hipStream_t s, float out_scale = 0.f);

hipError_t mmpl_launch_modulation(const bf16_t* mod, size_t mod_layer_stride, const bf16_t* e, int e_frame_stride, int bcast,
                                  bf16_t* emod, int n_layers, int n_frames, int nmod, int d, hipStream_t s);
hipError_t mmpl_launch_patchify(const bf16_t* x, bf16_t* a, int lda, int F, int C, int h, int w, hipStream_t s);
hipError_t mmpl_launch_add(bf16_t* a, const bf16_t* b, size_t n, hipStream_t s);
hipError_t mmpl_launch_unpatchify(const bf16_t* y, int ldy, bf16_t* out, int F, int C, int h, int w, hipStream_t s);
hipError_t mmpl_launch_zero_ints(int* p, int n, hipStream_t s);
struct PageList { const void* p[MMPL_MAX_PAGES]; int n; };
hipError_t mmpl_launch_share_check_zero(unsigned long long* chk, int which, hipStream_t s);
hipError_t mmpl_launch_pages_fingerprint(const PageList& pl, size_t bytes_per_page, unsigned long long* chk, int which, hipStream_t s);
hipError_t mmpl_launch_share_check_compare(unsigned long long* chk, hipStream_t s);
hipError_t mmpl_launch_rows_equal_last(const bf16_t* x, int ld, int rows, int d, int* flags, hipStream_t s);
hipError_t mmpl_launch_sinusoid(const float* t, bf16_t* out, int F, int freq_dim, hipStream_t s);
hipError_t mmpl_launch_silu(const bf16_t* x, bf16_t* y, size_t n, hipStream_t s);

struct UniPCArgs {
  const bf16_t* flow_c; const bf16_t* flow_u;
  float guidance;
  bf16_t* x;
  bf16_t* m0; bf16_t* m1; bf16_t* last_sample;
  size_t n;
  float sigma_cur;
  int use_corrector, corr_order; float c_c1, c_c2, c_c3, c_inv_rk, c_rho0, c_rho_last;
  int pred_order; float p_c1, p_c2, p_c3, p_inv_rk;
};
hipError_t mmpl_launch_unipc(const UniPCArgs& a, hipStream_t s);
struct UniPCStepDev {
  float guidance, sigma_cur; int use_corrector, corr_order; float c_c1, c_c2, c_c3, c_inv_rk, c_rho0, c_rho_last;
  int pred_order; float p_c1, p_c2, p_c3, p_inv_rk;
};
hipError_t mmpl_launch_unipc_table(const UniPCArgs& a, const UniPCStepDev* table, int* step, float* t_out, const float* t_tab,
                                   int n_t, int n_steps, hipStream_t s);
```

### mmpl_amd/csrc/mmpl_config.h

```cpp
#pragma once

struct MmplRuntimeConfig {
  bool attn_v1, attn_nosplit, attn_no_merge, cross_w64;
  bool gemm_v1, gemm_v2, gemm_no_splitk, gemm_no_subtile;
  int gemm_group;
  int gemm_pf;
  int gemm_v8;
  bool vae_no_fuse_norm;
  int ln_pipeline_min_rows;
  bool check_share;
};
const MmplRuntimeConfig& mmpl_config();
```

Measured before the change: 0.06380.

## Fuse cross-attention Q RMSNorm into GEMM epilogue and attention Q load

The cross-attention Q projection GEMM epilogue now writes per-row, per-64-column sum-of-squares partials. A tiny kernel reduces these into reciprocal RMS factors, and the LDS cross-attention kernel applies the factor and the gain when it loads Q. This replaces the separate RMSNorm pass that read and rewrote the whole Q buffer. It adds epilogue shuffles, a small extra launch and a second template instantiation, and it only applies when the v6 GEMM path and the LDS cross-attention path are taken.

```diff
diff --git a/include/mmpl_hip.h b/include/mmpl_hip.h
--- a/include/mmpl_hip.h
+++ b/include/mmpl_hip.h
@@ -71,6 +71,14 @@
 int mmpl_gemm_scratch(const void* A, int lda, const void* W, int ldw, const void* bias, void* C, int ldc, int M, int N, int K,
                       int epi, const void* res, int ldres, const void* gate, int gate_frame_stride, int rows_per_frame,
                       void* scratch, size_t scratch_bytes, mmpl_stream_t stream);
+
+int mmpl_gemm_rowsq(const void* A, int lda, const void* W, int ldw, const void* bias, void* C, int ldc, int M, int N, int K,
+                    void* scratch, size_t scratch_bytes, int mode, float* rowsq, int* wrote, mmpl_stream_t stream);
+int mmpl_rowsq_rr(const float* rowsq, int n_strips, int rows, int d, float eps, float* rr, mmpl_stream_t stream);
+int mmpl_rmsnorm(void* x, int ldx, const void* w, int rows, int d, float eps, mmpl_stream_t stream);
+int mmpl_attn_cross_qnorm(const void* q, int ldq, void* o, int ldo, const void* k, const void* v, int ldk, int ldv, int n_keys,
+                          int last_row_copies, int Lq, int num_heads, float softmax_scale, const float* q_rr, const void* q_gain,
+                          mmpl_stream_t stream);
 
 int mmpl_layernorm(const void* x, int ldx, void* y, int ldy, int rows, int d, float eps, const void* scale,
                    const void* shift, int mod_frame_stride, int rows_per_frame, const void* w, const void* b,
diff --git a/mmpl_amd/_lib.py b/mmpl_amd/_lib.py
--- a/mmpl_amd/_lib.py
+++ b/mmpl_amd/_lib.py
@@ -9,7 +9,7 @@
 SYMBOLS = [
     "mmpl_dit_num_weights", "mmpl_dit_weight_name", "mmpl_dit_create", "mmpl_dit_destroy", "mmpl_dit_bind_weights",
     "mmpl_dit_workspace_bytes", "mmpl_dit_context_workspace_bytes", "mmpl_dit_precompute_context", "mmpl_dit_forward", "mmpl_dit_attn_history_bytes", "mmpl_dit_share_check_failures", "mmpl_dit_set_attn_stats", "mmpl_dit_set_image_kv", "mmpl_clip_visual", "mmpl_clip_visual_workspace_bytes",
-    "mmpl_attn_fwd", "mmpl_attn_fwd_ws", "mmpl_attn_fwd_variant", "mmpl_attn_fwd_history", "mmpl_attn_history_bytes", "mmpl_attn_workspace_bytes", "mmpl_gemm", "mmpl_gemm_tickets", "mmpl_gemm_scratch", "mmpl_gemm_scratch_bytes", "mmpl_device_xcd_round_robin", "mmpl_probe_mfma_tflops", "mmpl_layernorm", "mmpl_qknorm_rope", "mmpl_cfg_unipc_step", "mmpl_cfg_unipc_step_table", "mmpl_fewstep_update",
+    "mmpl_attn_fwd", "mmpl_attn_fwd_ws", "mmpl_attn_fwd_variant", "mmpl_attn_fwd_history", "mmpl_attn_history_bytes", "mmpl_attn_workspace_bytes", "mmpl_gemm", "mmpl_gemm_tickets", "mmpl_gemm_scratch", "mmpl_gemm_scratch_bytes", "mmpl_device_xcd_round_robin", "mmpl_probe_mfma_tflops", "mmpl_layernorm", "mmpl_qknorm_rope", "mmpl_gemm_rowsq", "mmpl_rowsq_rr", "mmpl_rmsnorm", "mmpl_attn_cross_qnorm", "mmpl_cfg_unipc_step", "mmpl_cfg_unipc_step_table", "mmpl_fewstep_update",
     "mmpl_vae_num_weights", "mmpl_vae_weight_name", "mmpl_vae_create", "mmpl_vae_destroy", "mmpl_vae_bind_weights",
     "mmpl_vae_workspace_bytes", "mmpl_vae_decode", "mmpl_vae_encode",
     "mmpl_vae_stream_create", "mmpl_vae_stream_destroy", "mmpl_vae_stream_reset", "mmpl_vae_stream_decode",
@@ -88,6 +88,10 @@
     lib.mmpl_device_xcd_round_robin.argtypes = []
     lib.mmpl_probe_mfma_tflops.argtypes = [ci, C.c_double, C.POINTER(C.c_double)]
     lib.mmpl_gemm_scratch_bytes.restype = sz
+    lib.mmpl_gemm_rowsq.argtypes = [vp, ci, vp, ci, vp, vp, ci, ci, ci, ci, vp, sz, ci, vp, C.POINTER(ci), vp]
+    lib.mmpl_rowsq_rr.argtypes = [vp, ci, ci, ci, cf, vp, vp]
+    lib.mmpl_rmsnorm.argtypes = [vp, ci, vp, ci, ci, cf, vp]
+    lib.mmpl_attn_cross_qnorm.argtypes = [vp, ci, vp, ci, vp, vp, ci, ci, ci, ci, ci, ci, cf, vp, vp, vp]
     lib.mmpl_layernorm.argtypes = [vp, ci, vp, ci, ci, ci, cf, vp, vp, ci, ci, vp, vp, vp]
     lib.mmpl_qknorm_rope.argtypes = [vp, vp, ci, vp, ci, vp, ci, vp, vp, ci, C.POINTER(ci), C.POINTER(vp), C.POINTER(vp), vp]
     lib.mmpl_cfg_unipc_step.argtypes = [vp, vp, vp, vp, vp, vp, sz, C.POINTER(MmplUniPCStep), vp]
diff --git a/mmpl_amd/csrc/api.hip b/mmpl_amd/csrc/api.hip
--- a/mmpl_amd/csrc/api.hip
+++ b/mmpl_amd/csrc/api.hip
@@ -451,10 +451,25 @@
       ProfScope ps(K_LAYERNORM, 0, s);
       HIP_TRY(mmpl_launch_layernorm(a, s), "norm3");
     }
-    TRY(gemm(w.xn, d, h->Lw(l, L_CQ_W), d, h->Lw(l, L_CQ_B), w.big, d, Lq, d, d, EPI_BIAS, nullptr, 0, nullptr, 0, 1, s, tc, w.splitk));
+    const bool cross_lds = !cross_w64 && (ctx_n >= 0 ? ctx_n + 1 : T) <= MMPL_CROSS_LDS_MAX_KEYS;
+    float* const rowsq = (float*)w.ksc;
+    float* const q_rr = rowsq + (((size_t)Lq * (d / 64) + 63) & ~(size_t)63);
+    bool fused_qnorm = false;
+    {
+      GemmArgs g{w.xn, d, h->Lw(l, L_CQ_W), d, h->Lw(l, L_CQ_B), w.big, d, Lq, d, d, EPI_BIAS, nullptr, 0, nullptr, 0, 1, 1.0f, 0, 0, 0, 0, 0};
+      g.tile_counter = tc;
+      g.splitk_ws = w.splitk; g.splitk_cnt = tc + 64;
+      g.rowsq = rowsq;
+      fused_qnorm = !mmpl_config().no_fused_cross_qnorm && cross_lds && !h->img_k && mmpl_gemm_writes_rowsq(g) &&
+                    reinterpret_cast<uintptr_t>(h->Lw(l, L_CNQ)) % 16 == 0;
+      if (!fused_qnorm) g.rowsq = nullptr;
+      ProfScope ps(K_GEMM, 2.0 * Lq * (double)d * d, s);
+      HIP_TRY(mmpl_launch_gemm(g, s), "cross q gemm");
+    }
     {
       ProfScope ps(K_QKNORM, 0, s);
-      HIP_TRY(mmpl_launch_rmsnorm(w.big, d, h->Lw(l, L_CNQ), Lq, d, c.eps, s, cross_w64 ? scale * 1.4426950408889634f : 0.f), "cross q norm");
+      if (fused_qnorm) HIP_TRY(mmpl_launch_rowsq_rr(rowsq, d / 64, Lq, d, c.eps, q_rr, s), "cross q norm (row factors)");
+      else HIP_TRY(mmpl_launch_rmsnorm(w.big, d, h->Lw(l, L_CNQ), Lq, d, c.eps, s, cross_w64 ? scale * 1.4426950408889634f : 0.f), "cross q norm");
     }
     {
       AttnArgs a = {};
@@ -463,6 +478,7 @@
       a.cross = 1;
       if (cross_w64) { a.variant = ATTN_W64; a.q_prescaled = true; }
       else if (ctx_n >= 0) { a.page_rows = ctx_n + 1; a.last_row_copies = T - ctx_n; }
+      if (fused_qnorm) { a.q_rr = q_rr; a.q_gain = h->Lw(l, L_CNQ); }
       a.k_pages[0] = (const bf16_t*)cross_k + (size_t)l * T * d;
       a.v_pages[0] = (const bf16_t*)cross_v + (size_t)l * T * d;
       ProfScope ps(K_ATTN_CROSS, 4.0 * Lq * (double)T * d, s);
@@ -609,6 +625,46 @@
               (float*)((char*)scratch + 2048));
 }
 
+int mmpl_gemm_rowsq(const void* A, int lda, const void* W, int ldw, const void* bias, void* C, int ldc, int M, int N, int K,
+                    void* scratch, size_t scratch_bytes, int mode, float* rowsq, int* wrote, mmpl_stream_t stream) {
+  if (mode < 0 || mode > 2 || !rowsq || !wrote) return fail("mmpl_gemm_rowsq", "bad argument");
+  if (mode > 0 && (!scratch || scratch_bytes < mmpl_gemm_scratch_bytes() || reinterpret_cast<uintptr_t>(scratch) % 256))
+    return fail("mmpl_gemm_rowsq", "scratch missing, misaligned or smaller than mmpl_gemm_scratch_bytes()");
+  GemmArgs g{(const bf16_t*)A, lda, (const bf16_t*)W, ldw, (const bf16_t*)bias, (bf16_t*)C, ldc, M, N, K, EPI_BIAS, nullptr, 0, nullptr, 0, 1,
+             1.0f, 0, 0, 0, 0, 0};
+  if (mode >= 1) g.tile_counter = (int*)scratch;
+  if (mode == 2) { g.splitk_ws = (float*)((char*)scratch + 2048); g.splitk_cnt = (int*)scratch + 64; }
+  g.rowsq = rowsq;
+  *wrote = mmpl_gemm_writes_rowsq(g) ? 1 : 0;
+  HIP_TRY(mmpl_launch_gemm(g, (hipStream_t)stream), "mmpl_gemm_rowsq");
+  return 0;
+}
+
+int mmpl_rowsq_rr(const float* rowsq, int n_strips, int rows, int d, float eps, float* rr, mmpl_stream_t stream) {
+  if (!rowsq || !rr || n_strips < 1 || d < 1) return fail("mmpl_rowsq_rr", "bad argument");
+  HIP_TRY(mmpl_launch_rowsq_rr(rowsq, n_strips, rows, d, eps, rr, (hipStream_t)stream), "mmpl_rowsq_rr");
+  return 0;
+}
+
+int mmpl_rmsnorm(void* x, int ldx, const void* w, int rows, int d, float eps, mmpl_stream_t stream) {
+  HIP_TRY(mmpl_launch_rmsnorm((bf16_t*)x, ldx, (const bf16_t*)w, rows, d, eps, (hipStream_t)stream), "mmpl_rmsnorm");
+  return 0;
+}
+
+int mmpl_attn_cross_qnorm(const void* q, int ldq, void* o, int ldo, const void* k, const void* v, int ldk, int ldv, int n_keys,
+                          int last_row_copies, int Lq, int num_heads, float softmax_scale, const float* q_rr, const void* q_gain,
+                          mmpl_stream_t stream) {
+  if (n_keys < 1 || n_keys > MMPL_CROSS_LDS_MAX_KEYS) return fail("mmpl_attn_cross_qnorm", "n_keys out of range");
+  AttnArgs a = {};
+  a.cross = 1;
+  a.q = (const bf16_t*)q; a.ldq = ldq; a.o = (bf16_t*)o; a.ldo = ldo; a.ldk = ldk; a.ldv = ldv; a.n_pages = 1;
+  a.page_rows = n_keys; a.last_row_copies = last_row_copies; a.Lq = Lq; a.H = num_heads; a.scale = softmax_scale;
+  a.k_pages[0] = (const bf16_t*)k; a.v_pages[0] = (const bf16_t*)v;
+  a.q_rr = q_rr; a.q_gain = (const bf16_t*)q_gain;
+  HIP_TRY(mmpl_launch_attention(a, (hipStream_t)stream), "mmpl_attn_cross_qnorm");
+  return 0;
+}
+
 int mmpl_layernorm(const void* x, int ldx, void* y, int ldy, int rows, int d, float eps, const void* scale,
                    const void* shift, int mod_frame_stride, int rows_per_frame, const void* w, const void* b,
                    mmpl_stream_t stream) {
diff --git a/mmpl_amd/csrc/attention.hip b/mmpl_amd/csrc/attention.hip
--- a/mmpl_amd/csrc/attention.hip
+++ b/mmpl_amd/csrc/attention.hip
@@ -246,8 +246,9 @@
 
 constexpr int O_PITCH_X = 264;
 constexpr int SMEM_X = 2 * BUF + NW * QW * O_PITCH_X;
-
-template <int NT>
+constexpr int SMEM_X_QN = SMEM_X + 256;
+
+template <int NT, bool QN>
 __global__ __launch_bounds__(512, 2) void attn_cross_kernel(AttnArgs a, int qb_per_block, int blocks_per_head) {
   extern __shared__ __attribute__((aligned(16))) char smem[];
   const int tid = threadIdx.x, lane = tid & 63, wave = __builtin_amdgcn_readfirstlane(tid >> 6);
@@ -272,8 +273,30 @@
 #pragma unroll
     for (int c = 0; c < 8; ++c) f[c] = *reinterpret_cast<const bf16x8*>(qp + 16 * c);
   };
+  [[maybe_unused]] auto load_rr = [&](int qblock) { return a.q_rr[min(qblock * QB + wave * QW + l31, a.Lq - 1)]; };
+  [[maybe_unused]] const char* const gains = smem + SMEM_X + 16 * hi;
+  [[maybe_unused]] auto norm_q = [&](bf16x8 (&f)[8], float rr) {
+#pragma unroll
+    for (int c = 0; c < 8; ++c) {
+      union { bf16x8 v; uint32_t u[4]; } x, w;
+      x.v = f[c];
+      w.v = *reinterpret_cast<const bf16x8*>(gains + 32 * c);
+#pragma unroll
+      for (int j = 0; j < 4; ++j) {
+        const float lo = rbf(__uint_as_float(x.u[j] << 16) * rr) * __uint_as_float(w.u[j] << 16);
+        const float hi2 = rbf(__uint_as_float(x.u[j] & 0xffff0000u) * rr) * __uint_as_float(w.u[j] & 0xffff0000u);
+        x.u[j] = pack2bf(lo, hi2);
+      }
+      f[c] = x.v;
+    }
+  };
   bf16x8 qf[8], qn[8];
+  [[maybe_unused]] float rr_cur = 0.f, rr_nxt = 0.f;
   load_q(qf, qb);
+  if constexpr (QN) {
+    rr_cur = load_rr(qb);
+    if (tid < 16) *reinterpret_cast<u32x4*>(smem + SMEM_X + 16 * tid) = *reinterpret_cast<const u32x4*>(a.q_gain + head * 128 + 8 * tid);
+  }
   {
     const int srow = tid >> 4, schunk = tid & 15;
     const bf16_t* kp = a.k_pages[0] + head * 128 + schunk * 8;
@@ -297,10 +320,14 @@
   const int v_off = (4 * hi + (i16 >> 2)) * V_STRIDE + (16 * g16 + 4 * (i16 & 3)) * 2;
   char* ob = smem + 2 * BUF + wave * (QW * O_PITCH_X);
   const int orow = lane >> 4, ochunk = lane & 15;
+  if constexpr (QN) norm_q(qf, rr_cur);
 
   for (;; ++qb) {
     const bool more = qb + 1 < qb_end;
-    if (more) load_q(qn, qb + 1);
+    if (more) {
+      load_q(qn, qb + 1);
+      if constexpr (QN) rr_nxt = load_rr(qb + 1);
+    }
     asm volatile("" ::: "memory");
     AttnState st;
 #pragma unroll
@@ -336,6 +363,7 @@
       qf[i] = qn[i];
       asm volatile("" : "+v"(qf[i]));
     }
+    if constexpr (QN) norm_q(qf, rr_nxt);
   }
 }
 
@@ -432,17 +460,33 @@
   if (a.q_prescaled && variant != ATTN_W64) return hipErrorInvalidValue;
   if (a.last_row_copies > 1 && (variant != ATTN_LOCKSTEP || a.n_pages != 1)) return hipErrorInvalidValue;
   const int n_qb = (a.Lq + QB - 1) / QB;
-  if (variant == ATTN_LOCKSTEP && a.cross && a.n_pages == 1 && a.page_rows <= 2 * KVB) {
+  static_assert(MMPL_CROSS_LDS_MAX_KEYS == 2 * KVB, "attn_cross_kernel holds two KV tiles");
+  const bool cross_lds = variant == ATTN_LOCKSTEP && a.cross && a.n_pages == 1 && a.page_rows <= MMPL_CROSS_LDS_MAX_KEYS;
+  if ((a.q_rr != nullptr) != (a.q_gain != nullptr) || (a.q_rr && (!cross_lds || ((uintptr_t)a.q_gain & 15)))) return hipErrorInvalidValue;
+  if (cross_lds && a.q_rr) {
     const int nt = (a.page_rows + KVB - 1) / KVB;
-    const void* f = nt == 1 ? reinterpret_cast<const void*>(attn_cross_kernel<1>) : reinterpret_cast<const void*>(attn_cross_kernel<2>);
+    const void* f = nt == 1 ? reinterpret_cast<const void*>(attn_cross_kernel<1, true>) : reinterpret_cast<const void*>(attn_cross_kernel<2, true>);
+    if (hipError_t e = mmpl_dyn_smem_once(f, SMEM_X_QN); e != hipSuccess) return e;
+    const int cus = 8 * mmpl_cus_per_xcd();
+    int bph = cus / a.H < 1 ? 1 : cus / a.H;
+    if (bph > n_qb) bph = n_qb;
+    const int qpb = (n_qb + bph - 1) / bph;
+    bph = (n_qb + qpb - 1) / qpb;
+    if (nt == 1) hipLaunchKernelGGL((attn_cross_kernel<1, true>), dim3(bph * a.H), dim3(512), SMEM_X_QN, s, a, qpb, bph);
+    else hipLaunchKernelGGL((attn_cross_kernel<2, true>), dim3(bph * a.H), dim3(512), SMEM_X_QN, s, a, qpb, bph);
+    return hipGetLastError();
+  }
+  if (cross_lds) {
+    const int nt = (a.page_rows + KVB - 1) / KVB;
+    const void* f = nt == 1 ? reinterpret_cast<const void*>(attn_cross_kernel<1, false>) : reinterpret_cast<const void*>(attn_cross_kernel<2, false>);
     if (hipError_t e = mmpl_dyn_smem_once(f, SMEM_X); e != hipSuccess) return e;
     const int cus = 8 * mmpl_cus_per_xcd();
     int bph = cus / a.H < 1 ? 1 : cus / a.H;
     if (bph > n_qb) bph = n_qb;
     const int qpb = (n_qb + bph - 1) / bph;
     bph = (n_qb + qpb - 1) / qpb;
-    if (nt == 1) hipLaunchKernelGGL(attn_cross_kernel<1>, dim3(bph * a.H), dim3(512), SMEM_X, s, a, qpb, bph);
-    else hipLaunchKernelGGL(attn_cross_kernel<2>, dim3(bph * a.H), dim3(512), SMEM_X, s, a, qpb, bph);
+    if (nt == 1) hipLaunchKernelGGL((attn_cross_kernel<1, false>), dim3(bph * a.H), dim3(512), SMEM_X, s, a, qpb, bph);
+    else hipLaunchKernelGGL((attn_cross_kernel<2, false>), dim3(bph * a.H), dim3(512), SMEM_X, s, a, qpb, bph);
     return hipGetLastError();
   }
   if (variant == ATTN_LOCKSTEP) {
diff --git a/mmpl_amd/csrc/device_state.hip b/mmpl_amd/csrc/device_state.hip
--- a/mmpl_amd/csrc/device_state.hip
+++ b/mmpl_amd/csrc/device_state.hip
@@ -87,6 +87,7 @@
     c.vae_no_fuse_norm = flag("MMPL_VAE_NO_FUSE_NORM");
     c.ln_pipeline_min_rows = num("MMPL_LN_PIPELINE_MIN_ROWS", 16384);
     c.check_share = flag("MMPL_CHECK_SHARE");
+    c.no_fused_cross_qnorm = flag("MMPL_NO_FUSED_CROSS_QNORM");
     return c;
   }();
   return cfg;
diff --git a/mmpl_amd/csrc/elementwise.hip b/mmpl_amd/csrc/elementwise.hip
--- a/mmpl_amd/csrc/elementwise.hip
+++ b/mmpl_amd/csrc/elementwise.hip
@@ -464,6 +464,27 @@
   return mmpl_launch_qknorm(a, s);
 }
 
+__global__ __launch_bounds__(256) void rowsq_rr_kernel(const float* rowsq, int n_strips, int rows, float d, float eps, float* rr) {
+  const int row = blockIdx.x * 256 + threadIdx.x;
+  if (row >= rows) return;
+  const float* p = rowsq + (size_t)row * n_strips;
+  float sq = 0.f;
+  int i = 0;
+  if ((n_strips & 3) == 0) {
+    for (; i < n_strips; i += 4) {
+      const f32x4 v = *reinterpret_cast<const f32x4*>(p + i);
+      sq = (((sq + v[0]) + v[1]) + v[2]) + v[3];
+    }
+  }
+  for (; i < n_strips; ++i) sq += p[i];
+  rr[row] = rsqrtf(sq / d + eps);
+}
+hipError_t mmpl_launch_rowsq_rr(const float* rowsq, int n_strips, int rows, int d, float eps, float* rr, hipStream_t s) {
+  if (rows <= 0) return hipSuccess;
+  hipLaunchKernelGGL(rowsq_rr_kernel, dim3((rows + 255) / 256), dim3(256), 0, s, rowsq, n_strips, rows, (float)d, eps, rr);
+  return hipGetLastError();
+}
+
 hipError_t mmpl_launch_modulation(const bf16_t* mod, size_t mod_layer_stride, const bf16_t* e, int e_frame_stride, int bcast,
                                   bf16_t* emod, int n_layers, int n_frames, int nmod, int d, hipStream_t s) {
   const size_t n = (size_t)n_layers * n_frames * nmod * d;
diff --git a/mmpl_amd/csrc/gemm.hip b/mmpl_amd/csrc/gemm.hip
--- a/mmpl_amd/csrc/gemm.hip
+++ b/mmpl_amd/csrc/gemm.hip
@@ -93,6 +93,29 @@
         *reinterpret_cast<uint2*>(g.v_dst[fr] + (size_t)(m - fr * g.rows_per_frame) * g.v_ld + (n - g.v_col0)) = o;
       } else {
         *reinterpret_cast<uint2*>(g.C + (size_t)m * g.ldc + n) = o;
+      }
+    }
+  }
+  if (EPI == EPI_BIAS) {
+    if (g.rowsq) {
+#pragma unroll
+      for (int i = 0; i < 4; ++i) {
+        const int m = mw + 16 * i + frow;
+        float s[4];
+#pragma unroll
+        for (int j = 0; j < 4; ++j) {
+          const uint2 bb = bias4[j];
+          const float b[4] = {bf2f(bb.x & 0xffff), bf2f(bb.x >> 16), bf2f(bb.y & 0xffff), bf2f(bb.y >> 16)};
+          float q[4];
+#pragma unroll
+          for (int r = 0; r < 4; ++r) { const float v = rbf(acc[i][j][r] + b[r]); q[r] = v * v; }
+          const float first = ((q[0] + q[1]) + q[2]) + q[3];
+          const float from = __shfl_xor(first, 16, 64);
+          s[j] = (((from + q[0]) + q[1]) + q[2]) + q[3];
+          s[j] += __shfl_xor(s[j], 32, 64);
+        }
+        const float tot = (s[0] + s[1]) + (s[2] + s[3]);
+        if (fchunk == 1 && m < g.M && nw < g.N) g.rowsq[(size_t)m * (g.N >> 6) + (nw >> 6)] = tot;
       }
     }
   }
@@ -438,6 +461,21 @@
   for (int u = 0; u < 16; ++u) {
     const int row = 8 * u + erow, m = mw + row;
     const uint4 yv = *reinterpret_cast<const uint4*>(stg + row * 128 + ((ec ^ (row & 7)) << 4));
+    if (EPI == EPI_BIAS) {
+      if (g.rowsq) {
+        const uint32_t yw[4] = {yv.x, yv.y, yv.z, yv.w};
+        float sq = 0.f;
+#pragma unroll
+        for (int e = 0; e < 8; ++e) {
+          const float y = __uint_as_float((e & 1) ? (yw[e >> 1] & 0xffff0000u) : (yw[e >> 1] << 16));
+          sq += y * y;
+        }
+        sq += __shfl_xor(sq, 1, 64);
+        sq += __shfl_xor(sq, 2, 64);
+        sq += __shfl_xor(sq, 4, 64);
+        if (ec == 0 && m < g.M && nw < g.N) g.rowsq[(size_t)m * (g.N >> 6) + (nw >> 6)] = sq;
+      }
+    }
     if (m >= g.M || !n_ok) continue;
     uint4 ov = yv;
     if (HAS_RES) {
@@ -1041,6 +1079,26 @@
   }
 }
 
+bool staged_epilogue_ok(const GemmArgs& g) {
+  auto al = [](const void* p, uintptr_t a) { return p == nullptr || reinterpret_cast<uintptr_t>(p) % a == 0; };
+  bool ptrs_ok = al(g.C, 16) && al(g.bias, 8);
+  if (g.epi == EPI_GATE_RES || g.epi == EPI_RES) ptrs_ok = ptrs_ok && al(g.res, 16);
+  if (g.epi == EPI_GATE_RES) ptrs_ok = ptrs_ok && al(g.gate, 16);
+  if (g.epi == EPI_BIAS_VPAGES)
+    for (int i = 0; i < 8; ++i) ptrs_ok = ptrs_ok && al(g.v_dst[i], 16);
+  return ptrs_ok && g.N % 8 == 0 && g.ldc % 8 == 0 &&
+         (g.epi != EPI_GATE_RES || (g.gate_frame_stride % 8 == 0 && g.rows_per_frame >= 128)) &&
+         ((g.epi != EPI_GATE_RES && g.epi != EPI_RES) || g.ldres % 8 == 0) &&
+         (g.epi != EPI_BIAS_VPAGES || (g.v_col0 % 8 == 0 && g.v_ld % 8 == 0));
+}
+bool takes_v6(const GemmArgs& g) {
+  const bool big = g.batch <= 1 && g.M >= 1024 && g.N >= 256 && g.K >= 128 && !mmpl_config().gemm_v1 && !mmpl_config().gemm_v2;
+  return big && (long long)g.M * g.lda < (1ll << 31) && (long long)g.N * g.ldw < (1ll << 31);
+}
+bool rowsq_ok(const GemmArgs& g) {
+  return g.rowsq != nullptr && g.epi == EPI_BIAS && g.N % 64 == 0 && takes_v6(g) && staged_epilogue_ok(g);
+}
+
 template <int EPI>
 hipError_t launch_v6(const GemmArgs& g, hipStream_t s) {
   constexpr int smem = 2 * STAGE4 + 1024;
@@ -1057,16 +1115,8 @@
   const int env_group = rc.gemm_group;
   const int tiles_m_ = (g.M + BM3 - 1) / BM3;
   g2.group = env_group > 0 ? env_group : ((tiles_m_ >= 96 && g.N < 8192 && g.K < 8192) ? 8 : 4);
-  auto al = [](const void* p, uintptr_t a) { return p == nullptr || reinterpret_cast<uintptr_t>(p) % a == 0; };
-  bool ptrs_ok = al(g.C, 16) && al(g.bias, 8);
-  if (g.epi == EPI_GATE_RES || g.epi == EPI_RES) ptrs_ok = ptrs_ok && al(g.res, 16);
-  if (g.epi == EPI_GATE_RES) ptrs_ok = ptrs_ok && al(g.gate, 16);
-  if (g.epi == EPI_BIAS_VPAGES)
-    for (int i = 0; i < 8; ++i) ptrs_ok = ptrs_ok && al(g.v_dst[i], 16);
-  g2.staged_epilogue = ptrs_ok && g.N % 8 == 0 && g.ldc % 8 == 0 &&
-                       (g.epi != EPI_GATE_RES || (g.gate_frame_stride % 8 == 0 && g.rows_per_frame >= 128)) &&
-                       ((g.epi != EPI_GATE_RES && g.epi != EPI_RES) || g.ldres % 8 == 0) &&
-                       (g.epi != EPI_BIAS_VPAGES || (g.v_col0 % 8 == 0 && g.v_ld % 8 == 0));
+  g2.staged_epilogue = staged_epilogue_ok(g);
+  if (!rowsq_ok(g)) g2.rowsq = nullptr;
   g2.pf_dist = rc.gemm_pf;
   g2.sync_sweeps = 1;
   const int per = mmpl_cus_per_xcd(), n_cu = 8 * per;
@@ -1129,10 +1179,11 @@
 }
 
 template <int EPI>
-hipError_t launch(const GemmArgs& g, hipStream_t s) {
-  const bool env_v1 = mmpl_config().gemm_v1, env_v2 = mmpl_config().gemm_v2;
-  const bool big = g.batch <= 1 && g.M >= 1024 && g.N >= 256 && g.K >= 128 && !env_v1 && !env_v2;
-  if (big && (long long)g.M * g.lda < (1ll << 31) && (long long)g.N * g.ldw < (1ll << 31)) return launch_v6<EPI>(g, s);
+hipError_t launch(const GemmArgs& g_in, hipStream_t s) {
+  const bool env_v1 = mmpl_config().gemm_v1;
+  if (takes_v6(g_in)) return launch_v6<EPI>(g_in, s);
+  GemmArgs g = g_in;
+  g.rowsq = nullptr;
   if (g.batch <= 1 && g.M >= 1024 && g.N >= 128 && g.K >= 128 && !env_v1) return launch_v2<EPI>(g, s);
   constexpr int smem = 4 * TILE_BYTES;
   if (hipError_t e = mmpl_dyn_smem_once(reinterpret_cast<const void*>(gemm_bf16_kernel<EPI>), smem); e != hipSuccess) return e;
@@ -1142,6 +1193,8 @@
 }
 
 }
+
+bool mmpl_gemm_writes_rowsq(const GemmArgs& g) { return g.M > 0 && g.N > 0 && rowsq_ok(g); }
 
 size_t mmpl_gemm_splitk_ws_bytes() { return (size_t)256 * BM3 * BN3 * sizeof(float); }
 
diff --git a/mmpl_amd/csrc/kernels.h b/mmpl_amd/csrc/kernels.h
--- a/mmpl_amd/csrc/kernels.h
+++ b/mmpl_amd/csrc/kernels.h
@@ -30,12 +30,15 @@
   int sync_sweeps;
   float* splitk_ws; int* splitk_cnt;
   int splitk_s, splitk_tb, splitk_per;
+  float* rowsq;
 };
 size_t mmpl_gemm_splitk_ws_bytes();
+bool mmpl_gemm_writes_rowsq(const GemmArgs& g);
 bool mmpl_xcd_dispatch_ok(bool may_probe);
 hipError_t mmpl_launch_gemm(const GemmArgs& g, hipStream_t s);
 
 constexpr int MMPL_MAX_PAGES = 24;
+constexpr int MMPL_CROSS_LDS_MAX_KEYS = 128;
 struct AttnArgs {
   const bf16_t* q; int ldq;
   bf16_t* o; int ldo;
@@ -55,6 +58,7 @@
   unsigned long long* redo_stats;
   unsigned char* history;
   short* history_mem;
+  const float* q_rr; const bf16_t* q_gain;
 };
 __device__ __forceinline__ bool mmpl_attn_item(int H, int n_qb, int xcd, int local, int& head, int& qb) {
   if ((H & 7) == 0) {
@@ -106,6 +110,8 @@
 
 hipError_t mmpl_launch_rmsnorm(bf16_t* x, int ldx, const bf16_t* w, int rows, int d, float eps, hipStream_t s, float out_scale = 0.f);
 
+hipError_t mmpl_launch_rowsq_rr(const float* rowsq, int n_strips, int rows, int d, float eps, float* rr, hipStream_t s);
+
 hipError_t mmpl_launch_modulation(const bf16_t* mod, size_t mod_layer_stride, const bf16_t* e, int e_frame_stride, int bcast,
                                   bf16_t* emod, int n_layers, int n_frames, int nmod, int d, hipStream_t s);
 hipError_t mmpl_launch_patchify(const bf16_t* x, bf16_t* a, int lda, int F, int C, int h, int w, hipStream_t s);
diff --git a/mmpl_amd/csrc/mmpl_config.h b/mmpl_amd/csrc/mmpl_config.h
--- a/mmpl_amd/csrc/mmpl_config.h
+++ b/mmpl_amd/csrc/mmpl_config.h
@@ -9,5 +9,6 @@
   bool vae_no_fuse_norm;
   int ln_pipeline_min_rows;
   bool check_share;
+  bool no_fused_cross_qnorm;
 };
 const MmplRuntimeConfig& mmpl_config();
```

Result: no change. 0.06400, median of 6 (+0.3%).
